# ecmwf/anemoi-models

Measured on AMD Instinct MI355X. Metric: mesh-node updates/sec (fwd step), higher is better.
Workload: dtype bf16

## Files before the change

### anemoi_models_amd/_lib.py

```python

from __future__ import annotations

import ctypes
import os
from ctypes import c_char_p
from ctypes import c_float
from ctypes import c_int
from ctypes import c_int64
from ctypes import c_uint32
from ctypes import c_void_p

import torch

_PKG_DIR = os.path.dirname(os.path.abspath(__file__))
LIB_PATH = os.path.join(_PKG_DIR, "lib", "libanemoi_amd.so")

ANEMOI_OK = 0
ANEMOI_ERR_INVALID = 1
ANEMOI_ERR_UNSUPPORTED = 2
ANEMOI_ERR_LAUNCH = 3

F32 = 0
BF16 = 1

ACT_NONE, ACT_GELU, ACT_SILU, ACT_RELU = 0, 1, 2, 3
ACT_CODES = {"Identity": ACT_NONE, "GELU": ACT_GELU, "SiLU": ACT_SILU, "ReLU": ACT_RELU}

ABI_VERSION = 41


class GtBlockArgs(ctypes.Structure):

    _fields_ = [
        ("struct_bytes", c_int64), ("n_dst", c_int64),
        ("dtype", ctypes.c_int32), ("C", ctypes.c_int32), ("H", ctypes.c_int32), ("up", ctypes.c_int32),
        ("hidden", ctypes.c_int32), ("act", ctypes.c_int32), ("k_proj", ctypes.c_int32), ("n_in", ctypes.c_int32),
        ("eps_mlp", c_float), ("eps_out", c_float),
        ("x", c_void_p), ("ldx", c_int64), ("x_stats", c_void_p),
        ("w_in", c_void_p), ("b_in", c_void_p), ("cs_in", c_void_p),
        ("sq", c_void_p), ("ld_sq", c_int64),
        ("q", c_void_p), ("k", c_void_p), ("v", c_void_p), ("x_r", c_void_p), ("u", c_void_p),
        ("ldq", c_int64), ("ldkv", c_int64), ("ldr", c_int64), ("ldu", c_int64),
        ("edge_attr", c_void_p), ("rowptr", c_void_p), ("col", c_void_p),
        ("att", c_void_p), ("ld_att", c_int64),
        ("w_proj", c_void_p), ("b_proj", c_void_p), ("res", c_void_p), ("ld_res", c_int64), ("y", c_void_p),
        ("y_stats", c_void_p),
        ("w_fc1", c_void_p), ("b_fc1", c_void_p), ("cs_fc1", c_void_p), ("h", c_void_p),
        ("w_fc2", c_void_p), ("b_fc2", c_void_p), ("out", c_void_p), ("out_stats", c_void_p),
        ("stats_ws", c_void_p), ("stats_ws_bytes", c_int64),
        ("run_ptr", c_void_p), ("run_perm", c_void_p), ("n_runs", c_int64),
        ("sched", c_void_p), ("sched_slots", ctypes.c_int32), ("sched_steps", ctypes.c_int32), ("n_src", c_int64),
        ("run_dst", c_void_p), ("n_edges", c_int64),
        ("tile_hdr", c_void_p), ("tile_dst", c_void_p), ("tile_src", c_void_p), ("tile_slot", c_void_p), ("tile_xcd", c_void_p),
        ("tile_max_per_xcd", ctypes.c_int32), ("tile_src_cap", ctypes.c_int32), ("tile_edge_cap", ctypes.c_int32),
        ("tile_pad", ctypes.c_int32),
    ]

class TfmBlockArgs(ctypes.Structure):

    _fields_ = [
        ("struct_bytes", c_int64), ("rows", c_int64),
        ("dtype", ctypes.c_int32), ("B", ctypes.c_int32), ("S", ctypes.c_int32), ("C", ctypes.c_int32), ("H", ctypes.c_int32),
        ("hidden", ctypes.c_int32), ("act", ctypes.c_int32), ("window", ctypes.c_int32),
        ("eps1", c_float), ("eps2", c_float),
        ("dropout_p", c_float), ("dropout_seed", c_uint32), ("dropout_seed_dev", c_void_p),
        ("dropout_h0", ctypes.c_int32), ("dropout_h_total", ctypes.c_int32),
        ("x", c_void_p), ("ldx", c_int64),
        ("ln1_w", c_void_p), ("ln1_b", c_void_p), ("ln2_w", c_void_p), ("ln2_b", c_void_p),
        ("w_qkv", c_void_p), ("b_qkv", c_void_p), ("w_proj", c_void_p), ("b_proj", c_void_p),
        ("w_fc1", c_void_p), ("b_fc1", c_void_p), ("w_fc2", c_void_p), ("b_fc2", c_void_p),
        ("h_ln", c_void_p), ("qkv", c_void_p), ("att", c_void_p), ("y", c_void_p), ("h", c_void_p),
        ("mhsa_ws", c_void_p), ("out", c_void_p),
    ]


SIGNATURES = {
    "anemoi_abi_version": (c_int, []),
    "anemoi_build_info": (ctypes.c_char_p, []),
    "anemoi_last_error": (c_char_p, []),
    "anemoi_layer_norm": (c_int, [c_int, c_void_p, c_int64, c_void_p, c_void_p, c_void_p, c_int64, c_int64, c_int,
                                  c_float, c_void_p]),
    "anemoi_layer_norm_residual": (c_int, [c_int, c_void_p, c_int64, c_void_p, c_void_p, c_void_p, c_int64, c_void_p, c_int64,
                                           c_int64, c_int, c_float, c_void_p]),
    "anemoi_layer_norm_stats": (c_int, [c_int, c_void_p, c_int64, c_void_p, c_void_p, c_void_p, c_int64, c_void_p, c_int64,
                                        c_int, c_float, c_void_p]),
    "anemoi_linear": (c_int, [c_int, c_int, c_void_p, c_int64, c_void_p, c_void_p, c_void_p, c_int64, c_void_p,
                              c_int64, c_int64, c_int, c_int, c_int, c_void_p]),
    "anemoi_linear_stats": (c_int, [c_int, c_void_p, c_int64, c_void_p, c_void_p, c_void_p, c_void_p, c_void_p, c_int64,
                                    c_void_p, c_int64, c_int64, c_int, c_int, c_void_p, c_int64, c_float, c_void_p,
                                    c_void_p]),
    "anemoi_row_stats": (c_int, [c_int, c_void_p, c_int64, c_void_p, c_int64, c_int, c_float, c_void_p]),
    "anemoi_linear_ln": (c_int, [c_int, c_int, c_void_p, c_int64, c_void_p, c_void_p, c_void_p, c_void_p, c_void_p,
                                 c_int64, c_void_p, c_int64, c_int64, c_int, c_int, c_int, c_void_p]),
    "anemoi_edge_attr_csr": (c_int, [c_void_p, c_int, c_void_p, c_int, c_int64, c_void_p, c_void_p, c_int, c_int,
                                     c_int64, c_void_p]),
    "anemoi_gt_edge_attention_folded": (c_int, [c_int, c_void_p, c_int64, c_void_p, c_void_p, c_int64, c_void_p,
                                                c_int64, c_void_p, c_int64, c_void_p, c_int, c_void_p, c_void_p,
                                                c_void_p, c_int64, c_void_p, c_int64, c_int, c_int, c_void_p]),
    "anemoi_gt_edge_attention_folded_runs": (c_int, [c_int, c_void_p, c_int64, c_void_p, c_void_p, c_int64, c_void_p,
                                                     c_int64, c_void_p, c_int64, c_void_p, c_int, c_void_p, c_void_p,
                                                     c_void_p, c_void_p, c_int64, c_void_p, c_int64, c_void_p, c_int64, c_int,
                                                     c_int, c_void_p]),
    "anemoi_gt_edge_attention_folded_groups": (c_int, [c_int, c_void_p, c_int64, c_void_p, c_void_p, c_int64, c_void_p,
                                                       c_int64, c_void_p, c_int64, c_void_p, c_int, c_void_p, c_void_p,
                                                       c_void_p, c_void_p, c_void_p, c_int64, c_int64, c_void_p, c_int64,
                                                       c_void_p, c_int64, c_int, c_int, c_void_p]),
    "anemoi_edge_schedule_shape": (c_int, [c_int, c_int64, c_int, c_void_p, c_void_p]),
    "anemoi_gt_edge_attention_folded_sched": (c_int, [c_int, c_void_p, c_int64, c_void_p, c_void_p, c_int64, c_void_p,
                                                      c_int64, c_void_p, c_int64, c_void_p, c_int, c_void_p, c_void_p,
                                                      c_void_p, c_int, c_int, c_int64, c_int64, c_void_p, c_int64, c_void_p,
                                                      c_int64, c_int, c_int, c_void_p]),
    "anemoi_gt_edge_attention_folded_tiles": (c_int, [c_int, c_void_p, c_int64, c_void_p, c_void_p, c_int64, c_void_p,
                                                      c_int64, c_void_p, c_int64, c_void_p, c_int, c_void_p, c_void_p,
                                                      c_void_p, c_void_p, c_void_p, c_void_p, c_void_p, c_int, c_int, c_int,
                                                      c_int64, c_int64, c_void_p, c_int64, c_void_p, c_int64, c_int, c_int,
                                                      c_void_p]),
    "anemoi_linear_dual": (c_int, [c_int, c_void_p, c_int64, c_void_p, c_void_p, c_void_p, c_int64, c_void_p, c_int64,
                                   c_int64, c_int, c_int, c_int, c_void_p]),
    "anemoi_linear_actgrad": (c_int, [c_int, c_void_p, c_int64, c_void_p, c_void_p, c_int64, c_void_p, c_int64, c_int64,
                                      c_int, c_int, c_int, c_void_p]),
    "anemoi_gt_conv": (c_int, [c_int, c_void_p, c_int64, c_void_p, c_void_p, c_int64, c_void_p, c_int64, c_void_p, c_int64,
                               c_void_p, c_void_p, c_void_p, c_int64, c_void_p, c_int64, c_int, c_int, c_float, c_uint32,
                               c_void_p, c_void_p]),
    "anemoi_gt_conv_backward_dst": (c_int, [c_int, c_void_p, c_int64, c_void_p, c_void_p, c_int64, c_void_p, c_int64,
                                            c_void_p, c_int64, c_void_p, c_void_p, c_void_p, c_void_p, c_void_p, c_void_p,
                                            c_void_p, c_int64, c_int64, c_int, c_int, c_float, c_uint32, c_void_p,
                                            c_void_p]),
    "anemoi_gt_conv_backward_src": (c_int, [c_int, c_void_p, c_int64, c_void_p, c_int64, c_void_p, c_void_p, c_void_p,
                                            c_void_p, c_void_p, c_void_p, c_void_p, c_void_p, c_int64, c_void_p, c_int64,
                                            c_int64, c_int, c_int, c_float, c_uint32, c_void_p, c_void_p]),
    "anemoi_gt_edge_attention": (c_int, [c_int, c_void_p, c_int64, c_void_p, c_void_p, c_int64, c_void_p, c_int64,
                                         c_void_p, c_int, c_int, c_void_p, c_void_p, c_void_p, c_void_p, c_void_p,
                                         c_int64, c_int64, c_int, c_int, c_void_p]),
    "anemoi_gather_add_act": (c_int, [c_int, c_void_p, c_int64, c_void_p, c_int64, c_void_p, c_int64, c_void_p, c_void_p,
                                      c_void_p, c_int64, c_int64, c_int, c_int, c_void_p]),
    "anemoi_segment_sum": (c_int, [c_int, c_void_p, c_int64, c_void_p, c_void_p, c_int64, c_int64, c_int, c_void_p]),
    "anemoi_segment_sum_cat": (c_int, [c_int, c_void_p, c_int64, c_void_p, c_void_p, c_int64, c_void_p, c_int64, c_int64,
                                       c_int, c_void_p]),
    "anemoi_mhsa_workspace_bytes": (c_int64, [c_int, c_int, c_int, c_int, c_int]),
    "anemoi_mhsa": (c_int, [c_int, c_void_p, c_int64, c_void_p, c_int64, c_void_p, c_void_p, c_int, c_int, c_int, c_int,
                            c_int, c_float, c_uint32, c_void_p, c_int, c_int, c_void_p]),
    "anemoi_mhsa_backward_workspace_bytes": (c_int64, [c_int, c_int, c_int, c_int, c_int]),
    "anemoi_mhsa_backward": (c_int, [c_int, c_void_p, c_int64, c_void_p, c_int64, c_void_p, c_int64, c_void_p, c_void_p,
                                     c_void_p, c_int64, c_void_p, c_int, c_int, c_int, c_int, c_int, c_float, c_uint32,
                                     c_void_p, c_int, c_int, c_void_p]),
    "anemoi_assemble_nodes": (c_int, [c_int, c_void_p, c_int, c_int, c_int, c_int64, c_int, c_void_p, c_int,
                                      c_void_p, c_int, c_void_p, c_int64, c_void_p, c_void_p, c_void_p]),
    "anemoi_finalize_output": (c_int, [c_void_p, c_int, c_void_p, c_int, c_int, c_int, c_int64, c_int, c_void_p,
                                       c_void_p, c_void_p, c_void_p, c_void_p, c_void_p]),
    "anemoi_assemble_node_rows": (c_int, [c_int, c_void_p, c_int, c_int64, c_int, c_void_p, c_int, c_void_p, c_int,
                                          c_void_p, c_int64, c_void_p, c_int64, c_void_p, c_void_p, c_void_p]),
    "anemoi_finalize_output_rows": (c_int, [c_void_p, c_int, c_void_p, c_int, c_int64, c_int, c_void_p, c_void_p, c_int64,
                                            c_void_p, c_void_p, c_void_p, c_void_p, c_void_p]),
    "anemoi_bound_output": (c_int, [c_void_p, c_int, c_int64, c_int, c_void_p, c_void_p, c_void_p, c_void_p, c_int,
                                    c_void_p, c_void_p, c_void_p, c_void_p]),
    "anemoi_prognostic_residual": (c_int, [c_void_p, c_int, c_void_p, c_int, c_int, c_int, c_int64, c_int, c_void_p,
                                           c_void_p, c_int, c_void_p]),
    "anemoi_advance_input": (c_int, [c_void_p, c_int, c_int, c_int, c_int64, c_int, c_void_p, c_int, c_void_p, c_int,
                                     c_void_p, c_void_p]),
    "anemoi_transpose": (c_int, [c_int, c_void_p, c_int64, c_void_p, c_int64, c_int64, c_int, c_void_p]),
    "anemoi_transpose_colsum_rows": (c_int64, [c_int64, c_int64]),
    "anemoi_transpose_chunked": (c_int, [c_int, c_void_p, c_int64, c_void_p, c_int64, c_int64, c_int, c_int64, c_void_p,
                                         c_void_p]),
    "anemoi_weight_grad_tn": (c_int, [c_void_p, c_int64, c_void_p, c_int64, c_void_p, c_int64, c_void_p, c_int64, c_int64,
                                      c_int, c_int, c_int, c_void_p]),
    "anemoi_linear_batched": (c_int, [c_int, c_int, c_void_p, c_int64, c_int64, c_void_p, c_int64, c_void_p, c_int64,
                                      c_int64, c_int, c_int64, c_int, c_int, c_void_p]),
    "anemoi_col_sum_workspace_floats": (c_int64, [c_int64, c_int]),
    "anemoi_col_sum": (c_int, [c_int, c_void_p, c_int64, c_int64, c_int, c_void_p, c_void_p, c_int64, c_void_p]),
    "anemoi_row_dot": (c_int, [c_int, c_void_p, c_int64, c_void_p, c_int64, c_void_p, c_void_p, c_int64, c_int, c_void_p]),
    "anemoi_row_scale": (c_int, [c_int, c_void_p, c_int64, c_void_p, c_float, c_void_p, c_int64, c_int64, c_int, c_void_p]),
    "anemoi_act_forward": (c_int, [c_int, c_int, c_void_p, c_int64, c_void_p, c_int64, c_void_p, c_int64, c_int64, c_int,
                                   c_void_p]),
    "anemoi_act_backward": (c_int, [c_int, c_int, c_void_p, c_int64, c_void_p, c_int64, c_void_p, c_int64, c_int64, c_int,
                                    c_void_p]),
    "anemoi_layer_norm_backward_workspace_floats": (c_int64, [c_int64, c_int]),
    "anemoi_layer_norm_backward": (c_int, [c_int, c_void_p, c_int64, c_void_p, c_void_p, c_void_p, c_int64, c_void_p,
                                           c_int64, c_void_p, c_int64, c_int64, c_int, c_void_p, c_void_p, c_void_p,
                                           c_int64, c_void_p]),
    "anemoi_gt_edge_attention_folded_backward_dst": (c_int, [c_int, c_void_p, c_int64, c_void_p, c_void_p, c_int64,
                                                             c_void_p, c_int64, c_void_p, c_int64, c_void_p, c_int64,
                                                             c_void_p, c_void_p, c_int, c_void_p, c_void_p, c_void_p,
                                                             c_void_p, c_void_p, c_void_p, c_int64, c_void_p, c_int64,
                                                             c_void_p, c_int64, c_int64, c_int, c_int, c_void_p]),
    "anemoi_gt_edge_attention_folded_backward_src": (c_int, [c_int, c_void_p, c_int64, c_void_p, c_int64, c_void_p,
                                                             c_void_p, c_void_p, c_void_p, c_void_p, c_void_p, c_void_p,
                                                             c_void_p, c_int64, c_int64, c_int, c_int, c_void_p]),
    "anemoi_gt_edge_attr_grad": (c_int, [c_int, c_void_p, c_void_p, c_void_p, c_void_p, c_int64, c_void_p, c_int64,
                                         c_void_p, c_void_p, c_int64, c_int, c_int, c_int, c_void_p]),
    "anemoi_convert_pad": (c_int, [c_int, c_void_p, c_int64, c_int, c_void_p, c_int64, c_int64, c_int, c_void_p]),
    "anemoi_add": (c_int, [c_int, c_void_p, c_int64, c_void_p, c_int64, c_void_p, c_int64, c_int64, c_int, c_void_p]),
    "anemoi_gt_block_tail": (c_int, [ctypes.POINTER(GtBlockArgs), c_void_p]),
    "anemoi_gt_processor_block_forward": (c_int, [ctypes.POINTER(GtBlockArgs), c_void_p]),
    "anemoi_transformer_block_forward": (c_int, [ctypes.POINTER(TfmBlockArgs), c_void_p]),
}

_lib = None


class KernelLibraryMissing(RuntimeError):
    pass


def load(build_if_missing: bool = False) -> ctypes.CDLL:
    global _lib
    if _lib is not None:
        return _lib
    if not os.path.exists(LIB_PATH):
        if build_if_missing:
            from ._build import build

            build()
        else:
            raise KernelLibraryMissing(
                f"{LIB_PATH} not found: the HIP kernel library has not been built "
                "(run `python -c 'import __graft_entry__ as g; g.build()'`). There is no CPU fallback."
            )
    lib = ctypes.CDLL(LIB_PATH)
    for name, (restype, argtypes) in SIGNATURES.items():
        fn = getattr(lib, name)
        fn.restype = restype
        fn.argtypes = argtypes
    got = lib.anemoi_abi_version()
    if got != ABI_VERSION:
        raise RuntimeError(f"libanemoi_amd.so ABI version {got} != expected {ABI_VERSION}; rebuild the library")
    _lib = lib
    return lib


def check(status: int, what: str) -> None:
    if status == ANEMOI_OK:
        return
    msg = load().anemoi_last_error()
    msg = msg.decode() if msg else what
    if status == ANEMOI_ERR_INVALID:
        raise ValueError(msg)
    if status == ANEMOI_ERR_UNSUPPORTED:
        raise NotImplementedError(msg)
    raise RuntimeError(msg)
```

### anemoi_models_amd/csrc/blocks.hip

```cpp
#include "common.hpp"

using namespace anemoi;

namespace {

int check_args(const anemoi_gt_block_args* a, const char* who, bool with_input) {
  ANEMOI_REQUIRE(a != nullptr, ANEMOI_ERR_INVALID, "%s: null argument block", who);
  ANEMOI_REQUIRE(a->struct_bytes == (int64_t)sizeof(anemoi_gt_block_args), ANEMOI_ERR_INVALID,
                 "%s: argument block of %lld bytes, this library expects %lld (header / binding out of sync)", who,
                 (long long)a->struct_bytes, (long long)sizeof(anemoi_gt_block_args));
  ANEMOI_REQUIRE(a->dtype == ANEMOI_BF16, ANEMOI_ERR_UNSUPPORTED,
                 "%s: the LayerNorm-folded block route is bf16 only (dtype %d)", who, a->dtype);
  ANEMOI_REQUIRE(a->n_dst >= 0 && a->C > 0 && a->H > 0 && a->C % a->H == 0 && a->up > 0 && a->hidden > 0,
                 ANEMOI_ERR_INVALID, "%s: bad shape (n_dst %lld, C %d, H %d, up %d, hidden %d)", who, (long long)a->n_dst,
                 a->C, a->H, a->up, a->hidden);
  ANEMOI_REQUIRE(a->k_proj >= a->C + a->H * a->up && a->ld_att >= a->k_proj, ANEMOI_ERR_INVALID,
                 "%s: projection K %d / ld_att %lld too small for C + H * up = %d", who, a->k_proj, (long long)a->ld_att,
                 a->C + a->H * a->up);
  ANEMOI_REQUIRE(a->edge_attr && a->rowptr && a->col && a->att && a->w_proj && a->y && a->y_stats && a->w_fc1 && a->cs_fc1 &&
                     a->h && a->w_fc2 && a->out && a->stats_ws,
                 ANEMOI_ERR_INVALID, "%s: null pointer", who);
  ANEMOI_REQUIRE(a->stats_ws_bytes >= a->n_dst * (int64_t)(a->C / 128 > 1 ? a->C / 128 : 1) * 8, ANEMOI_ERR_INVALID,
                 "%s: statistics workspace of %lld bytes too small", who, (long long)a->stats_ws_bytes);
  if (with_input) {
    ANEMOI_REQUIRE(a->x && a->x_stats && a->w_in && a->cs_in && a->sq, ANEMOI_ERR_INVALID, "%s: null pointer (input product)",
                   who);
    ANEMOI_REQUIRE(a->n_in >= 4 * a->C + a->H * a->up && a->ld_sq >= a->n_in && a->ldx >= a->C, ANEMOI_ERR_INVALID,
                   "%s: input product of %d columns (ld %lld) cannot hold x_r | q | k | v | u = %d", who, a->n_in,
                   (long long)a->ld_sq, 4 * a->C + a->H * a->up);
  } else {
    ANEMOI_REQUIRE(a->q && a->k && a->v && a->x_r && a->u && a->res, ANEMOI_ERR_INVALID,
                   "%s: null pointer (edge phase operands / residual)", who);
  }
  return ANEMOI_OK;
}

int run_tail(const anemoi_gt_block_args* a, anemoi_stream_t stream) {
  int st;
  if (a->tile_hdr != nullptr && a->run_ptr == nullptr)
    st = anemoi_gt_edge_attention_folded_tiles(a->dtype, a->q, a->ldq, a->k, a->v, a->ldkv, a->x_r, a->ldr, a->u, a->ldu,
                                               a->edge_attr, a->up, a->rowptr, a->col, a->tile_hdr, a->tile_dst, a->tile_src,
                                               a->tile_slot, a->tile_xcd, a->tile_max_per_xcd, a->tile_src_cap,
                                               a->tile_edge_cap, a->n_src, a->n_edges, a->att, a->ld_att, nullptr, a->n_dst,
                                               a->C, a->H, stream);
  else if (a->sched != nullptr && a->run_ptr == nullptr)
    st = anemoi_gt_edge_attention_folded_sched(a->dtype, a->q, a->ldq, a->k, a->v, a->ldkv, a->x_r, a->ldr, a->u, a->ldu,
                                               a->edge_attr, a->up, a->rowptr, a->col, a->sched, a->sched_slots, a->sched_steps,
                                               a->n_src, a->n_edges, a->att, a->ld_att, nullptr, a->n_dst, a->C, a->H, stream);
  else if (a->run_ptr != nullptr && a->run_dst != nullptr)
    st = anemoi_gt_edge_attention_folded_groups(a->dtype, a->q, a->ldq, a->k, a->v, a->ldkv, a->x_r, a->ldr, a->u, a->ldu,
                                                a->edge_attr, a->up, a->rowptr, a->col, a->run_ptr, a->run_dst, a->run_perm,
                                                a->n_runs, a->n_src, a->att, a->ld_att, nullptr, a->n_dst, a->C, a->H, stream);
  else
    st = anemoi_gt_edge_attention_folded_runs(a->dtype, a->q, a->ldq, a->k, a->v, a->ldkv, a->x_r, a->ldr, a->u, a->ldu,
                                              a->edge_attr, a->up, a->rowptr, a->col, a->run_ptr, a->run_perm, a->n_runs,
                                              a->att, a->ld_att, nullptr, a->n_dst, a->C, a->H, stream);
  if (st != ANEMOI_OK) return st;
  st = anemoi_linear_stats(a->dtype, a->att, a->ld_att, a->w_proj, a->b_proj, nullptr, nullptr, a->res, a->ld_res, a->y,
                           a->C, a->n_dst, a->C, a->k_proj, a->stats_ws, a->stats_ws_bytes, a->eps_mlp, a->y_stats, stream);
  if (st != ANEMOI_OK) return st;
  st = anemoi_linear_ln(a->dtype, a->dtype, a->y, a->C, a->w_fc1, a->b_fc1, a->cs_fc1, a->y_stats, nullptr, 0, a->h,
                        a->hidden, a->n_dst, a->hidden, a->C, a->act, stream);
  if (st != ANEMOI_OK) return st;
  if (a->out_stats != nullptr)
    return anemoi_linear_stats(a->dtype, a->h, a->hidden, a->w_fc2, a->b_fc2, nullptr, nullptr, a->y, a->C, a->out, a->C,
                               a->n_dst, a->C, a->hidden, a->stats_ws, a->stats_ws_bytes, a->eps_out, a->out_stats, stream);
  return anemoi_linear(a->dtype, a->dtype, a->h, a->hidden, a->w_fc2, a->b_fc2, a->y, a->C, a->out, a->C, a->n_dst, a->C,
                       a->hidden, ANEMOI_ACT_NONE, stream);
}

}

extern "C" int anemoi_gt_block_tail(const anemoi_gt_block_args* args, anemoi_stream_t stream) {
  const int st = check_args(args, "anemoi_gt_block_tail", false);
  if (st != ANEMOI_OK) return st;
  if (args->n_dst == 0) return ANEMOI_OK;
  return run_tail(args, stream);
}

extern "C" int anemoi_gt_processor_block_forward(const anemoi_gt_block_args* args, anemoi_stream_t stream) {
  int st = check_args(args, "anemoi_gt_processor_block_forward", true);
  if (st != ANEMOI_OK) return st;
  if (args->n_dst == 0) return ANEMOI_OK;
  st = anemoi_linear_ln(args->dtype, args->dtype, args->x, args->ldx, args->w_in, args->b_in, args->cs_in, args->x_stats,
                        nullptr, 0, args->sq, args->ld_sq, args->n_dst, args->n_in, args->C, ANEMOI_ACT_NONE, stream);
  if (st != ANEMOI_OK) return st;
  anemoi_gt_block_args a = *args;
  const char* sq = static_cast<const char*>(args->sq);
  const int64_t c2 = (int64_t)args->C * 2;
  a.x_r = sq;
  a.q = sq + c2;
  a.k = sq + 2 * c2;
  a.v = sq + 3 * c2;
  a.u = sq + 4 * c2;
  a.ldq = a.ldkv = a.ldr = a.ldu = args->ld_sq;
  a.res = args->x;
  a.ld_res = args->ldx;
  return run_tail(&a, stream);
}

extern "C" int anemoi_transformer_block_forward(const anemoi_tfm_block_args* a, anemoi_stream_t stream) {
  const char* who = "anemoi_transformer_block_forward";
  ANEMOI_REQUIRE(a != nullptr, ANEMOI_ERR_INVALID, "%s: null argument block", who);
  ANEMOI_REQUIRE(a->struct_bytes == (int64_t)sizeof(anemoi_tfm_block_args), ANEMOI_ERR_INVALID,
                 "%s: argument block of %lld bytes, this library expects %lld (header / binding out of sync)", who,
                 (long long)a->struct_bytes, (long long)sizeof(anemoi_tfm_block_args));
  ANEMOI_REQUIRE(a->dtype == ANEMOI_F32 || a->dtype == ANEMOI_BF16, ANEMOI_ERR_UNSUPPORTED, "%s: dtype %d", who, a->dtype);
  ANEMOI_REQUIRE(a->rows >= 0 && a->B > 0 && a->S >= 0 && a->rows == (int64_t)a->B * a->S && a->C > 0 && a->H > 0 &&
                     a->C % a->H == 0 && a->hidden > 0,
                 ANEMOI_ERR_INVALID, "%s: bad shape (rows %lld, B %d, S %d, C %d, H %d, hidden %d)", who, (long long)a->rows,
                 a->B, a->S, a->C, a->H, a->hidden);
  ANEMOI_REQUIRE(a->x && a->ln1_w && a->ln1_b && a->ln2_w && a->ln2_b && a->w_qkv && a->w_proj && a->w_fc1 && a->w_fc2 &&
                     a->h_ln && a->qkv && a->att && a->y && a->h && a->out,
                 ANEMOI_ERR_INVALID, "%s: null pointer", who);
  ANEMOI_REQUIRE(a->ldx >= a->C && a->out != a->x, ANEMOI_ERR_INVALID, "%s: ldx too small, or out aliases x", who);
  if (a->rows == 0) return ANEMOI_OK;
  const int C = a->C;
  int st = anemoi_layer_norm(a->dtype, a->x, a->ldx, a->ln1_w, a->ln1_b, a->h_ln, C, a->rows, C, a->eps1, stream);
  if (st != ANEMOI_OK) return st;
  st = anemoi_linear(a->dtype, a->dtype, a->h_ln, C, a->w_qkv, a->b_qkv, nullptr, 0, a->qkv, 3 * (int64_t)C, a->rows, 3 * C, C,
                     ANEMOI_ACT_NONE, stream);
  if (st != ANEMOI_OK) return st;
  st = anemoi_mhsa(a->dtype, a->qkv, 3 * (int64_t)C, a->att, C, a->mhsa_ws, nullptr, a->B, a->S, a->H, C / a->H, a->window,
                   a->dropout_p, a->dropout_seed, a->dropout_seed_dev, a->dropout_h0, a->dropout_h_total, stream);
  if (st != ANEMOI_OK) return st;
  st = anemoi_linear(a->dtype, a->dtype, a->att, C, a->w_proj, a->b_proj, a->x, a->ldx, a->y, C, a->rows, C, C, ANEMOI_ACT_NONE,
                     stream);
  if (st != ANEMOI_OK) return st;
  st = anemoi_layer_norm(a->dtype, a->y, C, a->ln2_w, a->ln2_b, a->h_ln, C, a->rows, C, a->eps2, stream);
  if (st != ANEMOI_OK) return st;
  st = anemoi_linear(a->dtype, a->dtype, a->h_ln, C, a->w_fc1, a->b_fc1, nullptr, 0, a->h, a->hidden, a->rows, a->hidden, C,
                     a->act, stream);
  if (st != ANEMOI_OK) return st;
  return anemoi_linear(a->dtype, a->dtype, a->h, a->hidden, a->w_fc2, a->b_fc2, a->y, C, a->out, C, a->rows, C, a->hidden,
                       ANEMOI_ACT_NONE, stream);
}
```

### anemoi_models_amd/csrc/elementwise.hip

```cpp
#include <cstdlib>

#include "common.hpp"

namespace anemoi {

template <typename T>
__device__ __forceinline__ float round_to(float v);
template <>
__device__ __forceinline__ float round_to<float>(float v) { return v; }
template <>
__device__ __forceinline__ float round_to<bf16_t>(float v) { return bf16_to_f32(f32_to_bf16(v)); }

template <typename T, int VEC, int ITEMS>
__global__ __launch_bounds__(256) void layer_norm_kernel(const T* __restrict__ x, int64_t ldx,
                                                         const float* __restrict__ gamma,
                                                         const float* __restrict__ beta, T* __restrict__ y,
                                                         int64_t ldy, int64_t rows, int C, float eps,
                                                         float2* __restrict__ stats, const T* __restrict__ res = nullptr,
                                                         int64_t ldr = 0) {
  const int lane = threadIdx.x & 63;
  const int64_t row = (int64_t)blockIdx.x * 4 + (threadIdx.x >> 6);
  if (row >= rows) return;
  const T* xr = x + row * ldx;
  float v[ITEMS][VEC];
// ... 497 lines not shown
      const int m = op_mul[i];
      if (m >= 0) v *= yr[m];
      yr[c] = v;
    }
    for (int j = 0; j < n_fin; ++j) {
      const int c = fin_col[j];
      yr[c] = (yr[c] - fin_add[j]) / fin_mul[j];
    }
  }
}

static bool force_idx64() {
  static const bool v = [] {
    const char* e = getenv("ANEMOI_AMD_IDX64");
    return e != nullptr && atoi(e) != 0;
  }();
  return v;
}

static inline unsigned flat_grid(int64_t total) {
  int64_t blocks = (total + 255) / 256;
  if (blocks > 256 * 16) blocks = 256 * 16;
  if (blocks < 1) blocks = 1;
  return (unsigned)blocks;
}

}

using namespace anemoi;

extern "C" {

int anemoi_layer_norm(int dtype, const void* x, int64_t ldx, const float* gamma, const float* beta, void* y,
                      int64_t ldy, int64_t rows, int C, float eps, anemoi_stream_t stream) {
  ANEMOI_REQUIRE(x && y && gamma && beta, ANEMOI_ERR_INVALID, "anemoi_layer_norm: null pointer");
  ANEMOI_REQUIRE(C > 0 && rows >= 0 && ldx >= C && ldy >= C, ANEMOI_ERR_INVALID,
                 "anemoi_layer_norm: bad shape rows=%lld C=%d ldx=%lld ldy=%lld", (long long)rows, C, (long long)ldx,
                 (long long)ldy);
  if (rows == 0) return ANEMOI_OK;
  if (dtype == ANEMOI_F32) return layer_norm_launch<float>(x, ldx, gamma, beta, y, ldy, rows, C, eps, as_stream(stream));
  if (dtype == ANEMOI_BF16) return layer_norm_launch<bf16_t>(x, ldx, gamma, beta, y, ldy, rows, C, eps, as_stream(stream));
  return fail(ANEMOI_ERR_UNSUPPORTED, "anemoi_layer_norm: dtype %d", dtype);
}

int anemoi_layer_norm_residual(int dtype, const void* x, int64_t ldx, const float* gamma, const float* beta,
                               const void* residual, int64_t ldr, void* y, int64_t ldy, int64_t rows, int C, float eps,
                               anemoi_stream_t stream) {
  ANEMOI_REQUIRE(x && y && gamma && beta && residual, ANEMOI_ERR_INVALID, "anemoi_layer_norm_residual: null pointer");
  ANEMOI_REQUIRE(C > 0 && rows >= 0 && ldx >= C && ldy >= C && ldr >= C, ANEMOI_ERR_INVALID,
                 "anemoi_layer_norm_residual: bad shape rows=%lld C=%d ldx=%lld ldr=%lld ldy=%lld", (long long)rows, C,
                 (long long)ldx, (long long)ldr, (long long)ldy);
  if (rows == 0) return ANEMOI_OK;
  if (dtype == ANEMOI_F32)
    return layer_norm_launch<float>(x, ldx, gamma, beta, y, ldy, rows, C, eps, as_stream(stream), nullptr, residual, ldr);
  if (dtype == ANEMOI_BF16)
    return layer_norm_launch<bf16_t>(x, ldx, gamma, beta, y, ldy, rows, C, eps, as_stream(stream), nullptr, residual, ldr);
  return fail(ANEMOI_ERR_UNSUPPORTED, "anemoi_layer_norm_residual: dtype %d", dtype);
}

int anemoi_layer_norm_stats(int dtype, const void* x, int64_t ldx, const float* gamma, const float* beta, void* y,
                            int64_t ldy, float* stats, int64_t rows, int C, float eps, anemoi_stream_t stream) {
  ANEMOI_REQUIRE(x && y && gamma && beta && stats, ANEMOI_ERR_INVALID, "anemoi_layer_norm_stats: null pointer");
  ANEMOI_REQUIRE(C > 0 && rows >= 0 && ldx >= C && ldy >= C && (uintptr_t)stats % 8 == 0, ANEMOI_ERR_INVALID,
                 "anemoi_layer_norm_stats: bad shape rows=%lld C=%d ldx=%lld ldy=%lld (stats 8-byte aligned)",
                 (long long)rows, C, (long long)ldx, (long long)ldy);
  if (rows == 0) return ANEMOI_OK;
  float2* sp = reinterpret_cast<float2*>(stats);
  if (dtype == ANEMOI_F32)
    return layer_norm_launch<float>(x, ldx, gamma, beta, y, ldy, rows, C, eps, as_stream(stream), sp);
  if (dtype == ANEMOI_BF16)
    return layer_norm_launch<bf16_t>(x, ldx, gamma, beta, y, ldy, rows, C, eps, as_stream(stream), sp);
  return fail(ANEMOI_ERR_UNSUPPORTED, "anemoi_layer_norm_stats: dtype %d", dtype);
}

int anemoi_row_stats(int dtype, const void* x, int64_t ldx, float* stats, int64_t rows, int C, float eps,
                     anemoi_stream_t stream) {
  ANEMOI_REQUIRE(x && stats, ANEMOI_ERR_INVALID, "anemoi_row_stats: null pointer");
  ANEMOI_REQUIRE(C > 0 && rows >= 0 && ldx >= C, ANEMOI_ERR_INVALID, "anemoi_row_stats: bad shape rows=%lld C=%d ldx=%lld",
                 (long long)rows, C, (long long)ldx);
  ANEMOI_REQUIRE((uintptr_t)stats % 8 == 0, ANEMOI_ERR_INVALID, "anemoi_row_stats: stats must be 8-byte aligned");
  if (rows == 0) return ANEMOI_OK;
  if (dtype == ANEMOI_F32) return row_stats_launch<float>(x, ldx, stats, rows, C, eps, as_stream(stream));
  if (dtype == ANEMOI_BF16) return row_stats_launch<bf16_t>(x, ldx, stats, rows, C, eps, as_stream(stream));
  return fail(ANEMOI_ERR_UNSUPPORTED, "anemoi_row_stats: dtype %d", dtype);
}

static int assemble_nodes_impl(int dtype, const float* x, int B, int T, int Ens, int64_t G, int V, const float* latlons,
                               int n_ll, const float* trainable, int n_tr, void* out, int64_t ldo, const float* in_mul,
                               const float* in_add, const int64_t* rows, int64_t n_rows, anemoi_stream_t stream) {
  ANEMOI_REQUIRE((in_mul == nullptr) == (in_add == nullptr), ANEMOI_ERR_INVALID,
                 "anemoi_assemble_nodes: in_mul and in_add come together");
  ANEMOI_REQUIRE(out && B > 0 && Ens > 0 && G >= 0 && T >= 0 && V >= 0 && n_ll >= 0 && n_tr >= 0, ANEMOI_ERR_INVALID,
                 "anemoi_assemble_nodes: bad argument");
  ANEMOI_REQUIRE((x != nullptr) || T * V == 0, ANEMOI_ERR_INVALID, "anemoi_assemble_nodes: x is null");
  ANEMOI_REQUIRE((latlons != nullptr) || n_ll == 0, ANEMOI_ERR_INVALID, "anemoi_assemble_nodes: latlons is null");
  ANEMOI_REQUIRE((trainable != nullptr) || n_tr == 0, ANEMOI_ERR_INVALID, "anemoi_assemble_nodes: trainable is null");
  ANEMOI_REQUIRE(ldo >= (int64_t)T * V + n_ll + n_tr, ANEMOI_ERR_INVALID, "anemoi_assemble_nodes: ldo too small");
  const int64_t total = (rows != nullptr ? n_rows : (int64_t)B * Ens * G) * ldo;
  if (total == 0) return ANEMOI_OK;
  hipStream_t st = as_stream(stream);
  if (ldo % 8 == 0 && ldo < ((int64_t)1 << 31) && (uintptr_t)out % 16 == 0 && (dtype == ANEMOI_F32 || dtype == ANEMOI_BF16)) {
    const int ldo8 = (int)(ldo / 8);
#define ANEMOI_ASM8(TT, I32)                                                                                          \
  hipLaunchKernelGGL((assemble_nodes8_kernel<TT, I32>), dim3(flat_grid(total / 8)), dim3(256), 0, st, x, B, T, Ens, G, V, \
                     latlons, n_ll, trainable, n_tr, static_cast<TT*>(out), ldo8, in_mul, in_add, rows, n_rows)
    const bool idx32 = !force_idx64() && total / 8 < ((int64_t)1 << 31) - ((int64_t)1 << 24);
    if (dtype == ANEMOI_F32) {
      if (idx32) ANEMOI_ASM8(float, true);
      else ANEMOI_ASM8(float, false);
    } else {
      if (idx32) ANEMOI_ASM8(bf16_t, true);
      else ANEMOI_ASM8(bf16_t, false);
    }
#undef ANEMOI_ASM8
    return check_launch("anemoi_assemble_nodes");
  }
  if (dtype == ANEMOI_F32)
    hipLaunchKernelGGL((assemble_nodes_kernel<float>), dim3(flat_grid(total)), dim3(256), 0, st, x, B, T, Ens, G, V,
                       latlons, n_ll, trainable, n_tr, static_cast<float*>(out), ldo, in_mul, in_add, rows, n_rows);
  else if (dtype == ANEMOI_BF16)
    hipLaunchKernelGGL((assemble_nodes_kernel<bf16_t>), dim3(flat_grid(total)), dim3(256), 0, st, x, B, T, Ens, G, V,
                       latlons, n_ll, trainable, n_tr, static_cast<bf16_t*>(out), ldo, in_mul, in_add, rows, n_rows);
  else
    return fail(ANEMOI_ERR_UNSUPPORTED, "anemoi_assemble_nodes: dtype %d", dtype);
  return check_launch("anemoi_assemble_nodes");
}

int anemoi_assemble_nodes(int dtype, const float* x, int B, int T, int Ens, int64_t G, int V, const float* latlons,
                          int n_ll, const float* trainable, int n_tr, void* out, int64_t ldo, const float* in_mul,
                          const float* in_add, anemoi_stream_t stream) {
  return assemble_nodes_impl(dtype, x, B, T, Ens, G, V, latlons, n_ll, trainable, n_tr, out, ldo, in_mul, in_add, nullptr, 0,
                             stream);
}

int anemoi_assemble_node_rows(int dtype, const float* x, int T, int64_t G, int V, const float* latlons, int n_ll,
                              const float* trainable, int n_tr, const int64_t* rows, int64_t n_rows, void* out,
                              int64_t ldo, const float* in_mul, const float* in_add, anemoi_stream_t stream) {
  ANEMOI_REQUIRE(n_rows >= 0 && (rows != nullptr || n_rows == 0), ANEMOI_ERR_INVALID,
                 "anemoi_assemble_node_rows: null row list");
  if (n_rows == 0) return ANEMOI_OK;
  return assemble_nodes_impl(dtype, x, 1, T, 1, G, V, latlons, n_ll, trainable, n_tr, out, ldo, in_mul, in_add, rows, n_rows,
                             stream);
}

int anemoi_edge_attr_csr(const float* a0, int d0, const float* a1, int d1, int64_t rows0, const int32_t* perm,
                         float* out, int ld_out, int one_col, int64_t n_edges, anemoi_stream_t stream) {
  ANEMOI_REQUIRE(a0 && perm && out && d0 > 0 && d1 >= 0 && rows0 > 0 && n_edges >= 0, ANEMOI_ERR_INVALID,
                 "anemoi_edge_attr_csr: bad argument");
  ANEMOI_REQUIRE((a1 != nullptr) || d1 == 0, ANEMOI_ERR_INVALID, "anemoi_edge_attr_csr: a1 is null but d1 > 0");
  ANEMOI_REQUIRE(ld_out >= d0 + d1, ANEMOI_ERR_INVALID, "anemoi_edge_attr_csr: ld_out %d < %d", ld_out, d0 + d1);
  ANEMOI_REQUIRE(one_col < ld_out && (one_col < 0 || one_col >= d0 + d1), ANEMOI_ERR_INVALID,
                 "anemoi_edge_attr_csr: one_col %d must be a padding column", one_col);
  if (n_edges == 0) return ANEMOI_OK;
  hipLaunchKernelGGL(edge_attr_csr_kernel, dim3(flat_grid(n_edges * ld_out)), dim3(256), 0, as_stream(stream), a0, d0,
                     a1, d1, rows0, perm, out, ld_out, one_col, n_edges);
  return check_launch("anemoi_edge_attr_csr");
}

int anemoi_convert_pad(int src_dtype, const void* src, int64_t ld_src, int dst_dtype, void* dst, int64_t ld_dst,
                       int64_t rows, int cols, anemoi_stream_t stream) {
  ANEMOI_REQUIRE(src && dst && rows >= 0 && cols >= 0 && ld_src >= cols && ld_dst >= cols, ANEMOI_ERR_INVALID,
                 "anemoi_convert_pad: bad argument");
  if (rows == 0 || ld_dst == 0) return ANEMOI_OK;
  hipStream_t st = as_stream(stream);
  dim3 grid(flat_grid(rows * ld_dst)), block(256);
#define CP(S, D)                                                                                           \
  hipLaunchKernelGGL((convert_pad_kernel<S, D>), grid, block, 0, st, static_cast<const S*>(src), ld_src, \
                     static_cast<D*>(dst), ld_dst, rows, cols)
  if (src_dtype == ANEMOI_F32 && dst_dtype == ANEMOI_F32) CP(float, float);
  else if (src_dtype == ANEMOI_F32 && dst_dtype == ANEMOI_BF16) CP(float, bf16_t);
  else if (src_dtype == ANEMOI_BF16 && dst_dtype == ANEMOI_F32) CP(bf16_t, float);
  else if (src_dtype == ANEMOI_BF16 && dst_dtype == ANEMOI_BF16) CP(bf16_t, bf16_t);
  else return fail(ANEMOI_ERR_UNSUPPORTED, "anemoi_convert_pad: dtypes %d -> %d", src_dtype, dst_dtype);
#undef CP
  return check_launch("anemoi_convert_pad");
}

int anemoi_row_scale(int dtype, const void* x, int64_t ldx, const float* s, float alpha, void* out, int64_t ldo,
                     int64_t rows, int cols, anemoi_stream_t stream) {
  ANEMOI_REQUIRE(x && s && out && rows >= 0 && cols >= 0 && ldx >= cols && ldo >= cols, ANEMOI_ERR_INVALID,
                 "anemoi_row_scale: bad argument");
  if (rows * cols == 0) return ANEMOI_OK;
  hipStream_t st = as_stream(stream);
  const int vec = dtype == ANEMOI_F32 ? 4 : 8;
  dim3 grid(flat_grid(rows * ((cols + vec - 1) / vec))), block(256);
  if (dtype == ANEMOI_F32)
    hipLaunchKernelGGL((row_scale_kernel<float>), grid, block, 0, st, static_cast<const float*>(x), ldx, s, alpha,
                       static_cast<float*>(out), ldo, rows, cols);
  else if (dtype == ANEMOI_BF16)
    hipLaunchKernelGGL((row_scale_kernel<bf16_t>), grid, block, 0, st, static_cast<const bf16_t*>(x), ldx, s, alpha,
                       static_cast<bf16_t*>(out), ldo, rows, cols);
  else
    return fail(ANEMOI_ERR_UNSUPPORTED, "anemoi_row_scale: dtype %d", dtype);
  return check_launch("anemoi_row_scale");
}

int anemoi_row_dot(int dtype, const void* a, int64_t lda, const void* b, int64_t ldb, const float* shift, float* out,
                   int64_t rows, int cols, anemoi_stream_t stream) {
  ANEMOI_REQUIRE(a && b && out && rows >= 0 && cols >= 0 && lda >= cols && ldb >= cols, ANEMOI_ERR_INVALID,
                 "anemoi_row_dot: bad argument");
  if (rows == 0) return ANEMOI_OK;
  hipStream_t st = as_stream(stream);
  dim3 grid((unsigned)((rows + 3) / 4)), block(256);
  ANEMOI_REQUIRE((rows + 3) / 4 < ((int64_t)1 << 31), ANEMOI_ERR_UNSUPPORTED, "anemoi_row_dot: grid too large");
  if (dtype == ANEMOI_F32)
    hipLaunchKernelGGL((row_dot_kernel<float>), grid, block, 0, st, static_cast<const float*>(a), lda,
                       static_cast<const float*>(b), ldb, shift, out, rows, cols);
  else if (dtype == ANEMOI_BF16)
    hipLaunchKernelGGL((row_dot_kernel<bf16_t>), grid, block, 0, st, static_cast<const bf16_t*>(a), lda,
                       static_cast<const bf16_t*>(b), ldb, shift, out, rows, cols);
  else
    return fail(ANEMOI_ERR_UNSUPPORTED, "anemoi_row_dot: dtype %d", dtype);
  return check_launch("anemoi_row_dot");
}

int anemoi_add(int dtype, const void* a, int64_t lda, const void* b, int64_t ldb, void* y, int64_t ldy, int64_t rows,
               int cols, anemoi_stream_t stream) {
  ANEMOI_REQUIRE(a && b && y && rows >= 0 && cols >= 0, ANEMOI_ERR_INVALID, "anemoi_add: bad argument");
  if (rows * cols == 0) return ANEMOI_OK;
  hipStream_t st = as_stream(stream);
  dim3 grid(flat_grid(rows * cols)), block(256);
  if (dtype == ANEMOI_F32)
    hipLaunchKernelGGL((add_kernel<float>), grid, block, 0, st, static_cast<const float*>(a), lda,
                       static_cast<const float*>(b), ldb, static_cast<float*>(y), ldy, rows, cols);
  else if (dtype == ANEMOI_BF16)
    hipLaunchKernelGGL((add_kernel<bf16_t>), grid, block, 0, st, static_cast<const bf16_t*>(a), lda,
                       static_cast<const bf16_t*>(b), ldb, static_cast<bf16_t*>(y), ldy, rows, cols);
  else
    return fail(ANEMOI_ERR_UNSUPPORTED, "anemoi_add: dtype %d", dtype);
  return check_launch("anemoi_add");
}

int anemoi_prognostic_residual(float* y, int V_out, const float* x, int B, int T, int Ens, int64_t G, int V_in,
                               const int32_t* out_idx, const int32_t* in_idx, int n_prog, anemoi_stream_t stream) {
  ANEMOI_REQUIRE(y && x && B > 0 && T > 0 && Ens > 0 && G >= 0 && n_prog >= 0, ANEMOI_ERR_INVALID,
                 "anemoi_prognostic_residual: bad argument");
  ANEMOI_REQUIRE(n_prog == 0 || (out_idx && in_idx), ANEMOI_ERR_INVALID, "anemoi_prognostic_residual: null index");
  const int64_t total = (int64_t)B * Ens * G * n_prog;
  if (total == 0) return ANEMOI_OK;
  hipLaunchKernelGGL(prognostic_residual_kernel, dim3(flat_grid(total)), dim3(256), 0, as_stream(stream), y, V_out, x,
                     B, T, Ens, G, V_in, out_idx, in_idx, n_prog);
  return check_launch("anemoi_prognostic_residual");
}

int anemoi_advance_input(float* x, int B, int T, int Ens, int64_t G, int V_in, const float* y, int V_out,
                         const float* forcing, int F, const int32_t* colmap, anemoi_stream_t stream) {
  ANEMOI_REQUIRE(x && y && colmap && B > 0 && T > 0 && Ens > 0 && G >= 0 && V_in > 0 && V_out > 0 && F >= 0,
                 ANEMOI_ERR_INVALID, "anemoi_advance_input: bad argument");
  const int64_t total = (int64_t)B * Ens * G * V_in;
  if (total == 0) return ANEMOI_OK;
  hipLaunchKernelGGL(advance_input_kernel, dim3(flat_grid(total)), dim3(256), 0, as_stream(stream), x, B, T, Ens, G,
                     V_in, y, V_out, forcing, F, colmap);
  return check_launch("anemoi_advance_input");
}

static int finalize_output_impl(float* y, int V_out, const float* x, int B, int T, int Ens, int64_t G, int V_in,
                                const int32_t* src, const float* in_mul, const float* in_add, const float* out_mul,
                                const float* out_add, const int64_t* rows, int64_t n_rows, anemoi_stream_t stream) {
  ANEMOI_REQUIRE(y && x && src && B > 0 && T > 0 && Ens > 0 && G >= 0 && V_in > 0 && V_out > 0, ANEMOI_ERR_INVALID,
                 "anemoi_finalize_output: bad argument");
  ANEMOI_REQUIRE((in_mul == nullptr) == (in_add == nullptr) && (out_mul == nullptr) == (out_add == nullptr),
                 ANEMOI_ERR_INVALID, "anemoi_finalize_output: mul and add come together");
  const int64_t total = (rows != nullptr ? n_rows : (int64_t)B * Ens * G) * V_out;
  if (total == 0) return ANEMOI_OK;
  if (!force_idx64() && total < ((int64_t)1 << 31) - ((int64_t)1 << 24))
    hipLaunchKernelGGL(finalize_output_kernel<true>, dim3(flat_grid(total)), dim3(256), 0, as_stream(stream), y, V_out, x, B,
                       T, Ens, G, V_in, src, in_mul, in_add, out_mul, out_add, rows, n_rows);
  else
    hipLaunchKernelGGL(finalize_output_kernel<false>, dim3(flat_grid(total)), dim3(256), 0, as_stream(stream), y, V_out, x, B,
                       T, Ens, G, V_in, src, in_mul, in_add, out_mul, out_add, rows, n_rows);
  return check_launch("anemoi_finalize_output");
}

int anemoi_finalize_output(float* y, int V_out, const float* x, int B, int T, int Ens, int64_t G, int V_in,
                           const int32_t* src, const float* in_mul, const float* in_add, const float* out_mul,
                           const float* out_add, anemoi_stream_t stream) {
  return finalize_output_impl(y, V_out, x, B, T, Ens, G, V_in, src, in_mul, in_add, out_mul, out_add, nullptr, 0, stream);
}

int anemoi_finalize_output_rows(float* y, int V_out, const float* x, int T, int64_t G, int V_in, const int32_t* src,
                                const int64_t* rows, int64_t n_rows, const float* in_mul, const float* in_add,
                                const float* out_mul, const float* out_add, anemoi_stream_t stream) {
  ANEMOI_REQUIRE(n_rows >= 0 && (rows != nullptr || n_rows == 0), ANEMOI_ERR_INVALID,
                 "anemoi_finalize_output_rows: null row list");
  if (n_rows == 0) return ANEMOI_OK;
  return finalize_output_impl(y, V_out, x, 1, T, 1, G, V_in, src, in_mul, in_add, out_mul, out_add, rows, n_rows, stream);
}

int anemoi_bound_output(float* y, int V_out, int64_t rows, int n_ops, const int32_t* op_col, const float* op_lo,
                        const float* op_hi, const int32_t* op_mul, int n_fin, const int32_t* fin_col,
                        const float* fin_mul, const float* fin_add, anemoi_stream_t stream) {
  ANEMOI_REQUIRE(y && V_out > 0 && rows >= 0 && n_ops >= 0 && n_fin >= 0, ANEMOI_ERR_INVALID,
                 "anemoi_bound_output: bad argument");
  ANEMOI_REQUIRE(n_ops == 0 || (op_col && op_lo && op_hi && op_mul), ANEMOI_ERR_INVALID,
                 "anemoi_bound_output: null op list");
  ANEMOI_REQUIRE(n_fin == 0 || (fin_col && fin_mul && fin_add), ANEMOI_ERR_INVALID,
                 "anemoi_bound_output: null de-normalisation list");
  if (rows == 0 || (n_ops == 0 && n_fin == 0)) return ANEMOI_OK;
  hipLaunchKernelGGL(bound_output_kernel, dim3(flat_grid(rows)), dim3(256), 0, as_stream(stream), y, V_out, rows, n_ops,
                     op_col, op_lo, op_hi, op_mul, n_fin, fin_col, fin_mul, fin_add);
  return check_launch("anemoi_bound_output");
}

int anemoi_abi_version(void) { return 41; }

#ifndef ANEMOI_HIPCC_VERSION
#define ANEMOI_HIPCC_VERSION "unknown (built without anemoi_models_amd/_build.py)"
#endif
const char* anemoi_build_info(void) { return "gfx950; " ANEMOI_HIPCC_VERSION; }

const char* anemoi_last_error(void) { return err_buf(); }

}
```

### anemoi_models_amd/layers/block.py

```python

from __future__ import annotations

import os
from abc import ABC
from abc import abstractmethod
from typing import Optional

import torch
from torch import Tensor
from torch import nn

from .. import ops
from .. import runtime
from .. import training
from ..runtime import EdgePlan
from .conv import GraphConv
from .conv import GraphTransformerConv
from .mlp import MLP
from .mlp import NativeSequential
from .mlp import activation_class
from .mlp import linear_native


def inference_num_chunks() -> int:
    return int(os.environ.get("ANEMOI_INFERENCE_NUM_CHUNKS", "1"))


def _group_size(group) -> int:
    return 1 if group is None else group.size()


def _as_compute(x: Tensor, dtype: torch.dtype) -> Tensor:
    x = x if x.dtype == dtype else x.to(dtype)
    return x if (x.dim() == 2 and x.stride(1) == 1) else x.contiguous()



def folded_edge_phase(q: Tensor, k: Tensor, v: Tensor, x_r: Optional[Tensor], u: Tensor, edge_attr_csr: Tensor, plan,
                      num_heads: int, up: int, ld_out: Optional[int] = None) -> Tensor:
    runs = edge_runs(plan, q.dtype)
    tiles = None if runs is not None else edge_tiles(plan, q, num_heads, up)
    return ops.gt_edge_attention_folded(q, k, v, x_r, u, edge_attr_csr, plan.rowptr, plan.col, num_heads, up,
                                        ld_out=ld_out, runs=runs, tiles=tiles,
                                        sched=None if runs is not None or tiles is not None else edge_schedule(plan, q))


TILES_DEFAULT = "0"


def edge_tiles(plan, q: Tensor, num_heads: int, up: int):
    if (q.dtype != torch.bfloat16 or not hasattr(plan, "tiles")
            or os.environ.get("ANEMOI_AMD_EDGE_TILES", TILES_DEFAULT) == "0"):
        return None
    return plan.tiles(q.dtype, q.shape[-1], num_heads, up)


def edge_schedule(plan, q: Tensor):
    if q.dtype != torch.bfloat16 or not hasattr(plan, "schedule") or os.environ.get("ANEMOI_AMD_EDGE_SCHED", "1") == "0":
        return None
    return plan.schedule(q.dtype, q.shape[-1])


def set_tile_args(a, tiles, n_src: int, n_edges: int) -> None:
    a.tile_hdr, a.tile_dst, a.tile_src = tiles.hdr.data_ptr(), tiles.dst.data_ptr(), tiles.src.data_ptr()
    a.tile_slot, a.tile_xcd = tiles.slot.data_ptr(), tiles.xcd.data_ptr()
    a.tile_max_per_xcd, a.tile_src_cap, a.tile_edge_cap = tiles.max_tiles_per_xcd, tiles.src_cap, tiles.edge_cap
    a.n_src, a.n_edges = n_src, n_edges


def edge_runs(plan, dtype):
    if dtype != torch.bfloat16 or not hasattr(plan, "runs3") or os.environ.get("ANEMOI_AMD_EDGE_RUNS", "1") == "0":
        return None
    return plan.runs3()


class EmbeddedRows:

    def __init__(self, x_aug: Tensor, one_col: int, emb: nn.Linear, h: Optional[Tensor], packed, tag: str) -> None:
        self.x_aug, self.one_col, self.emb, self.h, self._packed, self._tag = x_aug, one_col, emb, h, packed, tag

    @property
    def dtype(self) -> torch.dtype:
        return self.x_aug.dtype

    @property
    def device(self) -> torch.device:
        return self.x_aug.device

    @property
    def shape(self):
        return (self.x_aug.shape[0], self.emb.out_features)

    def stats(self, eps: float) -> Tensor:
        if self.h is not None:
            return ops.row_stats(self.h, eps)
        kp = self.x_aug.shape[1]
        t = self._packed.get((self._tag, "embstats", self.dtype, kp, self.one_col), [self.emb.weight, self.emb.bias],
                             lambda: runtime.embedding_stats_operator(self.emb.weight, self.emb.bias, kp, self.one_col,
                                                                      self.dtype))
        return ops.row_stats(ops.linear(self.x_aug, t, None, stats_eps=eps), eps)


class BaseBlock(nn.Module, ABC):

    @abstractmethod
    def forward(self, x, edge_attr, edge_index, shapes, batch_size, size=None, model_comm_group=None): ...


class GraphTransformerBaseBlock(BaseBlock, ABC):

    def __init__(
        self,
        in_channels: int,
        hidden_dim: int,
        out_channels: int,
        edge_dim: int,
        num_heads: int = 16,
        bias: bool = True,
        activation: str = "GELU",
        num_chunks: int = 1,
        update_src_nodes: bool = False,
        **kwargs,
    ) -> None:
        super().__init__(**kwargs)
        self.update_src_nodes = update_src_nodes
        self.out_channels_conv = out_channels // num_heads
        self.num_heads = num_heads
        self.num_chunks = num_chunks
        self.activation = activation
        self.edge_dim = edge_dim
        width = num_heads * self.out_channels_conv

        self.lin_key = nn.Linear(in_channels, width)
        self.lin_query = nn.Linear(in_channels, width)
        self.lin_value = nn.Linear(in_channels, width)
        self.lin_self = nn.Linear(in_channels, width, bias=bias)
        self.lin_edge = nn.Linear(edge_dim, width)
        self.conv = GraphTransformerConv(out_channels=self.out_channels_conv)
        self.projection = nn.Linear(out_channels, out_channels)

        act = activation_class(activation)
        self.node_dst_mlp = nn.Sequential(
            nn.LayerNorm(out_channels), nn.Linear(out_channels, hidden_dim), act(), nn.Linear(hidden_dim, out_channels)
        )
        self.layer_norm1 = nn.LayerNorm(in_channels)
        if self.update_src_nodes:
            self.node_src_mlp = nn.Sequential(
                nn.LayerNorm(out_channels), nn.Linear(out_channels, hidden_dim), act(),
                nn.Linear(hidden_dim, out_channels),
            )
        self._packed = runtime.PackedWeights()
        self._plans = runtime.PlanCache()
        self._dst_mlp: Optional[NativeSequential] = None
        self._src_mlp: Optional[NativeSequential] = None

    def shard_qkve_heads(self, query: Tensor, key: Tensor, value: Tensor, edges: Tensor, shapes: tuple, batch_size: int,
                         model_comm_group=None):
        h, d = self.num_heads, self.out_channels_conv
        if _group_size(model_comm_group) <= 1:
            return tuple(t.reshape(t.shape[0], h, d) for t in (query, key, value, edges))
        from ..distributed.transformer import shard_heads

        assert batch_size == 1, "Only batch size of 1 is supported when model is sharded across GPUs"
        shapes_src, shapes_dst, shapes_edges = shapes
        out = []
        for t, shp in ((query, shapes_dst), (key, shapes_src), (value, shapes_src), (edges, shapes_edges)):
            t = t.reshape(1, t.shape[0], h, d).permute(0, 2, 1, 3)
            t = shard_heads(t, shapes=shp, mgroup=model_comm_group)
            out.append(t[0].permute(1, 0, 2).contiguous())
        return tuple(out)

    def shard_output_seq(self, out: Tensor, shapes: tuple, batch_size: int, model_comm_group=None) -> Tensor:
        if _group_size(model_comm_group) <= 1:
            return out.reshape(out.shape[0], -1)
        from ..distributed.transformer import shard_sequence

        t = out.permute(1, 0, 2).unsqueeze(0)
        t = shard_sequence(t, shapes=shapes[1], mgroup=model_comm_group)
        return t[0].permute(1, 0, 2).reshape(t.shape[2], -1).contiguous()

    def _cat_linear(self, tag: str, layers, dtype):
        w = self._packed.get((tag, "w", dtype), [l.weight for l in layers],
                             lambda: runtime.pack_weight([l.weight for l in layers], dtype))
        b = self._packed.get((tag, "b"), [l.bias for l in layers],
                             lambda: runtime.pack_bias([l.bias for l in layers], [l.out_features for l in layers],
                                                       layers[0].weight.device))
        return w, b

    @staticmethod
    def _ln_begin(ln: nn.LayerNorm, x: Tensor):
        if isinstance(x, EmbeddedRows):
            return x, x.stats(ln.eps), ln
        if runtime.ln_fold_enabled(x.dtype):
            return x, ops.row_stats(x, ln.eps), ln
        return ops.layer_norm(x, runtime.f32c(ln.weight), runtime.f32c(ln.bias), ln.eps), None, None

    def _ln_linear(self, handle, tag: str, plain, rows, params, **kw) -> Tensor:
        xin, stats, ln = handle
        if isinstance(xin, EmbeddedRows):
            xa = xin.x_aug
            wf, bf, zero = self._packed.get(
                (tag, "embfold", xa.dtype, xa.shape[1], xin.one_col, xin._tag),
                list(params) + [ln.weight, ln.bias, xin.emb.weight, xin.emb.bias],
                lambda: runtime.fold_embedded_layer_norm(*rows(), ln.weight, ln.bias, xin.emb.weight, xin.emb.bias,
                                                         xa.shape[1], xin.one_col, xa.dtype))
            return ops.linear(xa, wf, bf, ln=(stats, zero), **kw)
        if stats is None:
            w, b = plain()
            return ops.linear(xin, w, b, **kw)
        wf, bf, cs = self._packed.get(
            (tag, "lnfold", xin.dtype), list(params) + [ln.weight, ln.bias],
            lambda: runtime.fold_layer_norm(*rows(), ln.weight, ln.bias, xin.dtype))
        return ops.linear(xin, wf, bf, ln=(stats, cs), **kw)

    def _cat_rows(self, layers):
        w = torch.cat([l.weight.detach().float() for l in layers], dim=0)
        b = runtime.pack_bias([l.bias for l in layers], [l.out_features for l in layers], w.device)
        return w, b

    def _folded_rows(self, lead_layers, up: int):
        w, b = self._cat_rows(lead_layers)
        wu, bu = self._query_fold(up)
        return torch.cat([w, wu], dim=0), torch.cat([b, bu], dim=0)

    def _edge_params(self):
        return runtime.f32c(self.lin_edge.weight), runtime.f32c(self.lin_edge.bias)

    def fold_width(self, dtype) -> Optional[int]:
        if os.environ.get("ANEMOI_AMD_EDGE_FOLD", "1") == "0":
            return None
        vec = 16 // torch.empty((), dtype=dtype).element_size()
        d, h = self.out_channels_conv, self.num_heads
        if d % vec != 0 or (d // vec) not in (1, 2, 4, 8, 16):
            return None
        up = ops.round_up(self.edge_dim + 1, 4)
        if up > 16 or (h * up) % vec != 0 or self.lin_self.in_features % vec != 0:
            return None
        return up

    def edge_layout(self, dtype):
        up = self.fold_width(dtype)
        return (ops.round_up(self.edge_dim, 4), -1) if up is None else (up, self.edge_dim)

    def _edge_fold(self, up: int) -> Tensor:
        h, d = self.num_heads, self.out_channels_conv
        we = torch.zeros((h * d, up), dtype=torch.float32, device=self.lin_edge.weight.device)
        we[:, : self.edge_dim] = self.lin_edge.weight.detach().float()
        we[:, self.edge_dim] = self.lin_edge.bias.detach().float()
        return we.view(h, d, up)

    def _query_fold(self, up: int):
        h, d = self.num_heads, self.out_channels_conv
        weh = self._edge_fold(up)
        wq = self.lin_query.weight.detach().float().view(h, d, -1)
        wu = torch.einsum("hda,hdc->hac", weh, wq).reshape(h * up, -1)
        bu = torch.einsum("hda,hd->ha", weh, self.lin_query.bias.detach().float().view(h, d)).reshape(h * up)
        return wu, bu

    def _projection_fold(self, up: int) -> Tensor:
        h, d = self.num_heads, self.out_channels_conv
        wp = self.projection.weight.detach().float()
        return torch.einsum("ohd,hda->oha", wp.view(wp.shape[0], h, d), self._edge_fold(up)).reshape(wp.shape[0],
                                                                                                       h * up)

    def _folded_in(self, tag: str, lead_layers, dtype, up: int):
        edge_q = [self.lin_edge.weight, self.lin_edge.bias, self.lin_query.weight, self.lin_query.bias]
        w_in = self._packed.get((tag, "w", dtype, up), [l.weight for l in lead_layers] + edge_q,
                                lambda: runtime.pack_weight([l.weight for l in lead_layers] + [self._query_fold(up)[0]],
                                                            dtype))
        b_in = self._packed.get((tag, "b", up), [l.bias for l in lead_layers] + edge_q,
                                lambda: torch.cat([runtime.pack_bias([l.bias for l in lead_layers],
                                                                     [l.out_features for l in lead_layers],
                                                                     self.lin_edge.weight.device),
                                                   self._query_fold(up)[1]]).contiguous())
        return w_in, b_in

    def _folded_out(self, dtype, up: int):
        edge_p = [self.lin_edge.weight, self.lin_edge.bias, self.projection.weight]
        w_out = self._packed.get(("projf", "w", dtype, up), edge_p,
                                 lambda: runtime.pack_weight_cols([self.projection.weight.detach().float(),
                                                                   self._projection_fold(up)], dtype))
        return w_out, runtime.f32c(self.projection.bias)

    def _fold_params(self, lead_layers):
        return ([l.weight for l in lead_layers] + [l.bias for l in lead_layers]
                + [self.lin_edge.weight, self.lin_edge.bias, self.lin_query.weight, self.lin_query.bias])

    def _mlp_ln_eps(self, which: str, dtype) -> Optional[float]:
        mlp = self.node_dst_mlp if which == "dst" else self.node_src_mlp
        first = mlp[0] if isinstance(mlp, nn.Sequential) else None
        return first.eps if isinstance(first, nn.LayerNorm) and runtime.ln_fold_enabled(dtype) else None

    def _next_ln_eps(self, dtype) -> Optional[float]:
        ln1 = getattr(self, "layer_norm1", None)
        return ln1.eps if isinstance(ln1, nn.LayerNorm) and runtime.ln_fold_enabled(dtype) else None

    def block_abi_operands(self, dtype: torch.dtype, lead_layers, tag: str):
        up = self.fold_width(dtype)
        if up is None or not runtime.ln_fold_enabled(dtype):
            return None
        if self._dst_mlp is None:
            self._dst_mlp = NativeSequential(self.node_dst_mlp)
        mlp = self._dst_mlp.folded_pair(dtype)
        if mlp is None:
            return None
        ln = self.layer_norm1
        w_in, b_in, cs_in = self._packed.get(
            (tag, "lnfold", dtype), list(self._fold_params(lead_layers)) + [ln.weight, ln.bias],
            lambda: runtime.fold_layer_norm(*self._folded_rows(lead_layers, up), ln.weight, ln.bias, dtype))
        w_proj, b_proj = self._folded_out(dtype, up)
        eps_mlp, act, w1, b1, cs1, w2, b2 = mlp
        return dict(up=up, w_in=w_in, b_in=b_in, cs_in=cs_in, w_proj=w_proj, b_proj=b_proj, eps_mlp=eps_mlp, act=act, w_fc1=w1,
                    b_fc1=b1, cs_fc1=cs1, w_fc2=w2, b_fc2=b2, eps_ln1=ln.eps)

    def _block_tail(self, q: Tensor, k: Tensor, v: Tensor, x_r: Tensor, u: Tensor, edge_attr_csr: Tensor, plan, res: Tensor,
                    up: int, out_stats_eps: Optional[float]) -> Optional[Tensor]:
        import ctypes

        from .. import _lib

        dtype = q.dtype
        if (ops.PROFILE is not None or dtype != torch.bfloat16 or not q.is_cuda or plan.num_edges == 0 or q.shape[0] == 0
                or not self.block_abi or self._mlp_ln_eps("dst", dtype) is None):
            return None
        if self._dst_mlp is None:
            self._dst_mlp = NativeSequential(self.node_dst_mlp)
        mlp = self._dst_mlp.folded_pair(dtype)
        if mlp is None or not (res.dim() == 2 and res.stride(1) == 1):
            return None
        eps_mlp, act, w1, b1, cs1, w2, b2 = mlp
        wp, bp = self._folded_out(dtype, up)
        n, c, h = q.shape[0], q.shape[1], self.num_heads
        dev = q.device
        att = torch.empty((n, wp.shape[1]), dtype=dtype, device=dev)
        if wp.shape[1] > c + h * up:
            att[:, c + h * up:].zero_()
        y, hid, out = (torch.empty((n, w), dtype=dtype, device=dev) for w in (c, w1.shape[0], c))
        stats = torch.empty((2 if out_stats_eps is not None else 1, n, 2), dtype=torch.float32, device=dev)
        ws = torch.empty((n * max(c // 128, 1), 2), dtype=torch.float32, device=dev)
        a = _lib.GtBlockArgs()
        a.struct_bytes, a.n_dst, a.dtype = ctypes.sizeof(_lib.GtBlockArgs), n, ops.dtype_code(dtype)
        a.C, a.H, a.up, a.hidden, a.act, a.k_proj = c, h, up, w1.shape[0], _lib.ACT_CODES[act], wp.shape[1]
        a.eps_mlp, a.eps_out = eps_mlp, (out_stats_eps if out_stats_eps is not None else 0.0)
        a.q, a.k, a.v, a.x_r, a.u = q.data_ptr(), k.data_ptr(), v.data_ptr(), x_r.data_ptr(), u.data_ptr()
        a.ldq, a.ldkv, a.ldr, a.ldu = ops._ld(q), ops._ld(k), ops._ld(x_r), ops._ld(u)
        a.edge_attr, a.rowptr, a.col = edge_attr_csr.data_ptr(), plan.rowptr.data_ptr(), plan.col.data_ptr()
        runs = edge_runs(plan, dtype)
        if runs is not None:
            a.run_ptr, a.run_perm, a.n_runs = runs[0].data_ptr(), runs[1].data_ptr(), runs[0].shape[0] - 1
            if len(runs) == 3:
                a.run_dst, a.n_src = runs[2].data_ptr(), k.shape[0]
        else:
            tiles = edge_tiles(plan, q, h, up)
            if tiles is not None:
                set_tile_args(a, tiles, k.shape[0], edge_attr_csr.shape[0])
            sched = None if tiles is not None else edge_schedule(plan, q)
            if sched is not None:
                a.sched, a.sched_slots, a.sched_steps, a.n_src = sched.data_ptr(), sched.shape[1], sched.shape[2], k.shape[0]
                a.n_edges = edge_attr_csr.shape[0]
        a.att, a.ld_att = att.data_ptr(), wp.shape[1]
        a.w_proj, a.b_proj = wp.data_ptr(), ops._ptr(bp)
        a.res, a.ld_res, a.y, a.y_stats = res.data_ptr(), ops._ld(res), y.data_ptr(), stats[0].data_ptr()
        a.w_fc1, a.b_fc1, a.cs_fc1, a.h = w1.data_ptr(), ops._ptr(b1), cs1.data_ptr(), hid.data_ptr()
        a.w_fc2, a.b_fc2, a.out = w2.data_ptr(), ops._ptr(b2), out.data_ptr()
        a.out_stats = stats[1].data_ptr() if out_stats_eps is not None else None
        a.stats_ws, a.stats_ws_bytes = ws.data_ptr(), ws.numel() * 4
        _lib.check(_lib.load().anemoi_gt_block_tail(ctypes.byref(a), ops._stream()), "anemoi_gt_block_tail")
        if out_stats_eps is not None:
            ops._carry_stats(out, out_stats_eps, stats[1])
        return out

    block_abi = True

    def _node_mlp(self, y: Tensor, which: str, num_chunks: int, out_stats_eps: Optional[float] = None) -> Tensor:
        if which == "dst":
            if self._dst_mlp is None:
                self._dst_mlp = NativeSequential(self.node_dst_mlp)
            run = self._dst_mlp
        else:
            if self._src_mlp is None:
                self._src_mlp = NativeSequential(self.node_src_mlp)
            run = self._src_mlp
        if num_chunks <= 1:
            return run(y, residual=y, out_stats_eps=out_stats_eps)
        return torch.cat([run(c, residual=c) for c in y.tensor_split(num_chunks, dim=0) if c.shape[0] > 0], dim=0)

    def _check_channels(self, dtype) -> None:
        mult = ops.k_multiple(dtype)
        width = self.num_heads * self.out_channels_conv
        if width % mult != 0:
            raise NotImplementedError(
                f"hidden width {width} must be a multiple of {mult} for {dtype} on the MI355X path"
            )

    def _edge_inputs(self, edge_attr: Tensor, edge_index: Tensor, n_src: int, n_dst: int, dtype):
        if edge_attr.shape[1] != self.edge_dim:
            raise ValueError(f"edge_attr has {edge_attr.shape[1]} features, lin_edge expects {self.edge_dim}")
        if edge_attr.shape[0] != edge_index.shape[1]:
            raise ValueError(f"edge_attr has {edge_attr.shape[0]} rows for {edge_index.shape[1]} edges")
        plan = self._plans.get(edge_index, n_src, n_dst)
        return plan, ops.edge_attr_csr(edge_attr, None, plan.perm, *self.edge_layout(dtype))

    @abstractmethod
    def forward(self, x, edge_attr, edge_index, shapes, batch_size, model_comm_group=None, size=None): ...


class GraphTransformerProcessorBlock(GraphTransformerBaseBlock):

    def native(self, x: Tensor, edge_attr_csr: Tensor, plan: EdgePlan, halo=None) -> Tensor:
        dtype = x.dtype
        self._check_channels(dtype)
        c = self.num_heads * self.out_channels_conv
        xh = self._ln_begin(self.layer_norm1, x)
        up = self.fold_width(dtype)
        if halo is not None:
            if up is None:
                raise NotImplementedError("node-partitioned blocks need the folded edge kernel")
            n_own = x.shape[0]
            kv_layers, sq_layers = [self.lin_key, self.lin_value], [self.lin_self, self.lin_query]
            kv = torch.empty((n_own + halo.n_recv, 2 * c), dtype=dtype, device=x.device)
            self._ln_linear(xh, "kv", lambda: self._cat_linear("kv", kv_layers, dtype),
                            lambda: self._cat_rows(kv_layers), [l.weight for l in kv_layers] + [l.bias for l in kv_layers],
                            out=kv[:n_own])
            pending = halo.start(kv, n_own)
            wpf, bp = self._folded_out(dtype, up)
            sq = self._ln_linear(xh, "squ", lambda: self._folded_in("squ", sq_layers, dtype, up),
                                 lambda: self._folded_rows(sq_layers, up),
                                 self._fold_params(sq_layers))
            halo.finish(pending)
            done = self._block_tail(sq[:, c:2 * c], kv[:, :c], kv[:, c:], sq[:, :c], sq[:, 2 * c:], edge_attr_csr, plan, x, up,
                                    self._next_ln_eps(dtype))
            if done is not None:
                return done
            att = folded_edge_phase(sq[:, c:2 * c], kv[:, :c], kv[:, c:], sq[:, :c], sq[:, 2 * c:], edge_attr_csr, plan,
                                    self.num_heads, up, ld_out=wpf.shape[1])
            y = ops.linear(att, wpf, bp, residual=x, stats_eps=self._mlp_ln_eps("dst", dtype))
            return self._node_mlp(y, "dst", 1, out_stats_eps=self._next_ln_eps(dtype))
        all4 = [self.lin_self, self.lin_query, self.lin_key, self.lin_value]
        if up is not None:
            wpf, bp = self._folded_out(dtype, up)
            sq = self._ln_linear(xh, "sqkvu", lambda: self._folded_in("sqkvu", all4, dtype, up),
                                 lambda: self._folded_rows(all4, up),
                                 self._fold_params(all4))
            done = self._block_tail(sq[:, c:2 * c], sq[:, 2 * c:3 * c], sq[:, 3 * c:4 * c], sq[:, :c], sq[:, 4 * c:],
                                    edge_attr_csr, plan, x, up, self._next_ln_eps(dtype))
            if done is not None:
                return done
            att = folded_edge_phase(sq[:, c:2 * c], sq[:, 2 * c:3 * c], sq[:, 3 * c:4 * c], sq[:, :c], sq[:, 4 * c:],
                                    edge_attr_csr, plan, self.num_heads, up, ld_out=wpf.shape[1])
            y = ops.linear(att, wpf, bp, residual=x, stats_eps=self._mlp_ln_eps("dst", dtype))
            return self._node_mlp(y, "dst", 1, out_stats_eps=self._next_ln_eps(dtype))
        wp, bp = self._cat_linear("proj", [self.projection], dtype)
        we, be = self._edge_params()
        sqkv = self._ln_linear(xh, "sqkv", lambda: self._cat_linear("sqkv", all4, dtype), lambda: self._cat_rows(all4),
                               [l.weight for l in all4] + [l.bias for l in all4])
        att = self.conv.fused(sqkv[:, c:2 * c], sqkv[:, 2 * c:3 * c], sqkv[:, 3 * c:], sqkv[:, :c], edge_attr_csr,
                              self.edge_dim, we, be, plan, self.num_heads)
        y = ops.linear(att, wp, bp, residual=x, stats_eps=self._mlp_ln_eps("dst", dtype))
        return self._node_mlp(y, "dst", 1, out_stats_eps=self._next_ln_eps(dtype))

    def _sharded(self, x: Tensor, edge_attr: Tensor, edge_index: Tensor, shapes: tuple, batch_size: int, model_comm_group,
                 size=None) -> Tensor:
        from .. import autograd

        dtype = runtime.compute_dtype(x)
        x = _as_compute(x, dtype)
        ln = self.layer_norm1
        h = autograd.layer_norm(x, ln.weight, ln.bias, ln.eps)
        x_r, q, k, v = (autograd.linear(h, lin.weight, lin.bias) for lin in (self.lin_self, self.lin_query, self.lin_key,
                                                                              self.lin_value))
        e = autograd.linear(_as_compute(edge_attr, dtype), self.lin_edge.weight, self.lin_edge.bias)
        q, k, v, e = self.shard_qkve_heads(q, k, v, e, shapes, batch_size, model_comm_group)
        out = self.conv(q, k, v, e, edge_index, size=size)
        out = self.shard_output_seq(out, shapes, batch_size, model_comm_group)
        out = autograd.linear(out + x_r, self.projection.weight, self.projection.bias, "Identity", x)
        return training.sequential(self.node_dst_mlp, out, residual=out)

    def forward(
        self,
        x: Tensor,
        edge_attr: Tensor,
        edge_index: Tensor,
        shapes: tuple,
        batch_size: int,
        model_comm_group=None,
        size=None,
    ):
        if _group_size(model_comm_group) > 1:
            assert batch_size == 1, "Only batch size of 1 is supported when model is sharded across GPUs"
            return self._sharded(x, edge_attr, edge_index, shapes, batch_size, model_comm_group, size), edge_attr
        if training.wants_grad(self, x, edge_attr):
            return training.gt_processor_block(self, x, edge_attr, edge_index, size)
        dtype = runtime.compute_dtype(x)
        n = x.shape[0]
        if size is not None and tuple(size) != (n, n):
            raise ValueError(f"Encountered tensor with size {n} in dimension 0, but expected size {tuple(size)}")
        plan, ea = self._edge_inputs(edge_attr, edge_index, n, n, dtype)
        return self.native(_as_compute(x, dtype), ea, plan), edge_attr


class GraphTransformerMapperBlock(GraphTransformerBaseBlock):

    def __init__(
        self,
        in_channels: int,
        hidden_dim: int,
        out_channels: int,
        edge_dim: int,
        num_heads: int = 16,
        bias: bool = True,
        activation: str = "GELU",
        num_chunks: int = 1,
        update_src_nodes: bool = False,
        **kwargs,
    ) -> None:
        super().__init__(
            in_channels=in_channels, hidden_dim=hidden_dim, out_channels=out_channels, edge_dim=edge_dim,
            num_heads=num_heads, bias=bias, activation=activation, num_chunks=num_chunks,
            update_src_nodes=update_src_nodes, **kwargs,
        )
        self.layer_norm2 = nn.LayerNorm(in_channels)

    def native(self, x_src: Tensor, x_dst: Tensor, edge_attr_csr: Tensor, plan: EdgePlan, num_chunks: int = 1,
               halo=None, out_stats_eps: Optional[float] = None):
        dtype = x_dst.dtype
        self._check_channels(dtype)
        c = self.num_heads * self.out_channels_conv
        h_dst = x_dst.h if isinstance(x_dst, EmbeddedRows) else x_dst
        if isinstance(x_src, EmbeddedRows) and x_src.h is None and self.update_src_nodes:
            raise ValueError("update_src_nodes needs the embedded source rows")
        kv_layers, sq_layers = [self.lin_key, self.lin_value], [self.lin_self, self.lin_query]
        kv_args = ("kv", lambda: self._cat_linear("kv", kv_layers, dtype), lambda: self._cat_rows(kv_layers),
                   [l.weight for l in kv_layers] + [l.bias for l in kv_layers])
        xs = self._ln_begin(self.layer_norm1, x_src)
        if halo is None:
            kv = self._ln_linear(xs, *kv_args)
        else:
            n_own = x_src.shape[0]
            kv = torch.empty((n_own + halo.n_recv, 2 * c), dtype=dtype, device=x_src.device)
            self._ln_linear(xs, *kv_args, out=kv[:n_own])
            pending = halo.start(kv, n_own)
        del xs
        xd = self._ln_begin(self.layer_norm2, x_dst)
        up = self.fold_width(dtype)
        if up is not None:
            wp, bp = self._folded_out(dtype, up)
            sq = self._ln_linear(xd, "squ", lambda: self._folded_in("squ", sq_layers, dtype, up),
                                 lambda: self._folded_rows(sq_layers, up),
                                 self._fold_params(sq_layers))
            del xd
            if halo is not None:
                halo.finish(pending)
            if num_chunks <= 1 and not self.update_src_nodes:
                done = self._block_tail(sq[:, c:2 * c], kv[:, :c], kv[:, c:], sq[:, :c], sq[:, 2 * c:], edge_attr_csr, plan,
                                        h_dst, up, out_stats_eps)
                if done is not None:
                    return (x_src.h if isinstance(x_src, EmbeddedRows) else x_src), done
            att = folded_edge_phase(sq[:, c:2 * c], kv[:, :c], kv[:, c:], sq[:, :c], sq[:, 2 * c:], edge_attr_csr, plan,
                                    self.num_heads, up, ld_out=wp.shape[1])
        else:
            if halo is not None:
                raise NotImplementedError("node-partitioned blocks need the folded edge kernel")
            wp, bp = self._cat_linear("proj", [self.projection], dtype)
            we, be = self._edge_params()
            sq = self._ln_linear(xd, "sq", lambda: self._cat_linear("sq", sq_layers, dtype),
                                 lambda: self._cat_rows(sq_layers),
                                 [l.weight for l in sq_layers] + [l.bias for l in sq_layers])
            del xd
            att = self.conv.fused(sq[:, c:], kv[:, :c], kv[:, c:], sq[:, :c], edge_attr_csr, self.edge_dim, we, be,
                                  plan, self.num_heads)
        del sq, kv
        y = ops.linear(att, wp, bp, residual=h_dst,
                       stats_eps=self._mlp_ln_eps("dst", dtype) if num_chunks <= 1 else None)
        del att
        new_dst = self._node_mlp(y, "dst", num_chunks, out_stats_eps=out_stats_eps)
        if isinstance(x_src, EmbeddedRows):
            x_src = x_src.h
        new_src = self._node_mlp(x_src, "src", num_chunks) if self.update_src_nodes else x_src
        return new_src, new_dst

    def _sharded(self, x, edge_attr: Tensor, edge_index: Tensor, shapes: tuple, batch_size: int, model_comm_group, size=None):
        from .. import autograd

        x_src, x_dst = x
        dtype = runtime.compute_dtype(x_dst)
        x_src, x_dst = _as_compute(x_src, dtype), _as_compute(x_dst, dtype)
        ln1, ln2 = self.layer_norm1, self.layer_norm2
        hs = autograd.layer_norm(x_src, ln1.weight, ln1.bias, ln1.eps)
        hd = autograd.layer_norm(x_dst, ln2.weight, ln2.bias, ln2.eps)
        x_r = autograd.linear(hd, self.lin_self.weight, self.lin_self.bias)
        q = autograd.linear(hd, self.lin_query.weight, self.lin_query.bias)
        k = autograd.linear(hs, self.lin_key.weight, self.lin_key.bias)
        v = autograd.linear(hs, self.lin_value.weight, self.lin_value.bias)
        e = autograd.linear(_as_compute(edge_attr, dtype), self.lin_edge.weight, self.lin_edge.bias)
        q, k, v, e = self.shard_qkve_heads(q, k, v, e, shapes, batch_size, model_comm_group)
        out = self.conv(q, k, v, e, edge_index, size=size)
        out = self.shard_output_seq(out, shapes, batch_size, model_comm_group)
        out = autograd.linear(out + x_r, self.projection.weight, self.projection.bias, "Identity", x_dst)
        new_src = training.sequential(self.node_src_mlp, x_src, residual=x_src) if self.update_src_nodes else x_src
        return new_src, training.sequential(self.node_dst_mlp, out, residual=out)

    def forward(
        self,
        x,
        edge_attr: Tensor,
        edge_index: Tensor,
        shapes: tuple,
        batch_size: int,
        model_comm_group=None,
        size=None,
    ):
        if _group_size(model_comm_group) > 1:
            assert batch_size == 1, "Only batch size of 1 is supported when model is sharded across GPUs"
            return self._sharded(x, edge_attr, edge_index, shapes, batch_size, model_comm_group, size), edge_attr
        if training.wants_grad(self, x[0], x[1], edge_attr):
            return training.gt_mapper_block(self, x, edge_attr, edge_index, size)
        x_src, x_dst = x
        dtype = runtime.compute_dtype(x_dst)
        n_src, n_dst = x_src.shape[0], x_dst.shape[0]
        if size is not None and tuple(size) != (n_src, n_dst):
            raise ValueError(f"Encountered tensors with sizes {(n_src, n_dst)}, but expected size {tuple(size)}")
        plan, ea = self._edge_inputs(edge_attr, edge_index, n_src, n_dst, dtype)
        num_chunks = self.num_chunks if self.training else inference_num_chunks()
        new_src, new_dst = self.native(_as_compute(x_src, dtype), _as_compute(x_dst, dtype), ea, plan, num_chunks)
        return (new_src if self.update_src_nodes else x[0], new_dst), edge_attr


class GraphConvBaseBlock(BaseBlock, ABC):
    def __init__(
        self,
        in_channels: int,
        out_channels: int,
        mlp_extra_layers: int = 0,
        activation: str = "SiLU",
        update_src_nodes: bool = True,
        num_chunks: int = 1,
        **kwargs,
    ) -> None:
        super().__init__(**kwargs)
        self.update_src_nodes = update_src_nodes
        self.num_chunks = num_chunks
        self.node_mlp = MLP(2 * in_channels, out_channels, out_channels, n_extra_layers=mlp_extra_layers,
                            activation=activation)
        self.conv = GraphConv(in_channels=in_channels, out_channels=out_channels, mlp_extra_layers=mlp_extra_layers,
                              activation=activation)
        self._packed = runtime.PackedWeights()
        self._plans = runtime.PlanCache()

    @abstractmethod
    def forward(self, x, edge_attr: Tensor, edge_index: Tensor, shapes: tuple, model_comm_group=None, size=None):
        """``(new nodes, new edge state)`` -- reference layers/block.py:157-167."""

    @staticmethod
    def _check_width(width: int, dtype) -> None:
        mult = ops.k_multiple(dtype)
        if width % mult != 0:
            raise NotImplementedError(f"hidden width {width} must be a multiple of {mult} for {dtype} on the MI355X path")


class GraphConvProcessorBlock(GraphConvBaseBlock):

    def native(self, x: Tensor, e_csr: Tensor, plan: EdgePlan, halo=None):
        dtype = x.dtype
        c = x.shape[1]
        self._check_width(c, dtype)
        edge_mlp, node_mlp = self.conv.edge_mlp.native(), self.node_mlp.native()
        lin1 = edge_mlp.steps[0][1]
        act1 = edge_mlp.steps[0][2]
        if lin1.in_features != 3 * c or e_csr.shape[1] != c:
            raise ValueError(f"GNN block expects node / edge width {lin1.in_features // 3}, got {c} / {e_csr.shape[1]}")
        if e_csr.shape[0] == 0 and halo is None:
            xcat = torch.zeros((x.shape[0], 2 * c), dtype=dtype, device=x.device)
            xcat[:, :c].copy_(x)
            return node_mlp(xcat, residual=x), e_csr
        w_nodes = self._packed.get(("w1_nodes", dtype), [lin1.weight],
                                   lambda: runtime.pack_weight([lin1.weight[:, :c], lin1.weight[:, c:2 * c]], dtype))
        w_edges = self._packed.get(("w1_edges", dtype), [lin1.weight],
                                   lambda: runtime.pack_weight([lin1.weight[:, 2 * c:]], dtype))
        b1 = None if lin1.bias is None else runtime.f32c(lin1.bias)
        if halo is None:
            p = ops.linear(x, w_nodes, None)
            p_dst, p_src = p[:, :c], p[:, c:]
            t = ops.linear(e_csr, w_edges, b1)
        else:
            n_own = x.shape[0]
            p_src = torch.empty((n_own + halo.n_recv, c), dtype=dtype, device=x.device)
            ops.linear(x, w_nodes[c:], None, out=p_src[:n_own])
            pending = halo.start(p_src, n_own)
            p_dst = ops.linear(x, w_nodes[:c], None)
            t = ops.linear(e_csr, w_edges, b1)
            halo.finish(pending)
            p = None
        h = ops.gather_add_act(t, p_dst, p_src, plan.dst, plan.col, act=act1, out=t)
        e_new = edge_mlp(h, residual=e_csr, start=1)
        del h, t, p, p_dst, p_src
        xcat = ops.segment_sum(e_new, plan.rowptr, cat_with=x)
        return node_mlp(xcat, residual=x), e_new

    def _sharded(self, x, edge_attr, edge_index, shapes, model_comm_group, size=None):
        from ..distributed.graph import shard_tensor, sync_tensor

        dtype = runtime.compute_dtype(x)
        x = _as_compute(x, dtype)
        x_in = sync_tensor(x, 0, shapes[1], model_comm_group)
        out, edges_new = self.conv(x_in, _as_compute(edge_attr, dtype), edge_index, size=size)
        out = shard_tensor(out, 0, shapes[1], model_comm_group, gather_in_backward=False)
        return training.mlp(self.node_mlp, torch.cat([x, out], dim=1), residual=x), edges_new

    def forward(self, x, edge_attr, edge_index, shapes, model_comm_group=None, size=None):
        if _group_size(model_comm_group) > 1:
            return self._sharded(x, edge_attr, edge_index, shapes, model_comm_group, size)
        if training.wants_grad(self, x, edge_attr):
            return training.gnn_processor_block(self, x, edge_attr, edge_index, size)
        dtype = runtime.compute_dtype(x)
        n = x.shape[0]
        plan = self._plans.get(edge_index, n, n)
        perm = plan.perm.long()
        e_csr = _as_compute(edge_attr, dtype).index_select(0, perm)
        x_new, e_new = self.native(_as_compute(x, dtype), e_csr, plan)
        edges_new = torch.empty_like(e_new)
        edges_new[perm] = e_new
        return x_new, edges_new


class GraphConvMapperBlock(GraphConvBaseBlock):

    def native(self, x_src: Tensor, x_dst: Tensor, e_csr: Tensor, plan: EdgePlan, halo=None):
        dtype = x_dst.dtype
        c = x_dst.shape[1]
        self._check_width(c, dtype)
        edge_mlp, node_mlp = self.conv.edge_mlp.native(), self.node_mlp.native()
        lin1, act1 = edge_mlp.steps[0][1], edge_mlp.steps[0][2]
        if e_csr.shape[0] == 0 and halo is None:
            def lone(x, second):
                xcat = torch.zeros((x.shape[0], 2 * c), dtype=dtype, device=x.device)
                xcat[:, :c].copy_(x)
                if second is not None:
                    xcat[:, c:].copy_(second)
                return node_mlp(xcat, residual=x)

            return (lone(x_src, x_src) if self.update_src_nodes else x_src, lone(x_dst, None)), e_csr
        w_dst = self._packed.get(("w1_dst", dtype), [lin1.weight], lambda: runtime.pack_weight([lin1.weight[:, :c]], dtype))
        w_src = self._packed.get(("w1_src", dtype), [lin1.weight],
                                 lambda: runtime.pack_weight([lin1.weight[:, c:2 * c]], dtype))
        w_edges = self._packed.get(("w1_edges", dtype), [lin1.weight],
                                   lambda: runtime.pack_weight([lin1.weight[:, 2 * c:]], dtype))
        if halo is None:
            p_src = ops.linear(x_src, w_src, None)
            pending = None
        else:
            n_own = x_src.shape[0]
            p_src = torch.empty((n_own + halo.n_recv, c), dtype=dtype, device=x_dst.device)
            ops.linear(x_src, w_src, None, out=p_src[:n_own])
            pending = halo.start(p_src, n_own)
        p_dst = ops.linear(x_dst, w_dst, None)
        t = ops.linear(e_csr, w_edges, None if lin1.bias is None else runtime.f32c(lin1.bias))
        if pending is not None:
            halo.finish(pending)
        h = ops.gather_add_act(t, p_dst, p_src, plan.dst, plan.col, act=act1, out=t)
        e_new = edge_mlp(h, residual=e_csr, start=1)
        del h, t, p_dst, p_src

        def update(x, agg):
            if agg is not None:
                return node_mlp(ops.segment_sum(agg, plan.rowptr, cat_with=x), residual=x)
            xcat = torch.empty((x.shape[0], 2 * c), dtype=dtype, device=x.device)
            xcat[:, :c].copy_(x)
            xcat[:, c:].copy_(x)
            return node_mlp(xcat, residual=x)

        new_dst = update(x_dst, e_new)
        new_src = update(x_src, None) if self.update_src_nodes else x_src
        return (new_src, new_dst), e_new

    def _sharded(self, x, edge_attr, edge_index, shapes, model_comm_group, size=None):
        from ..distributed.graph import shard_tensor, sync_tensor

        dtype = runtime.compute_dtype(x[1])
        x_src, x_dst = _as_compute(x[0], dtype), _as_compute(x[1], dtype)
        x_in = (sync_tensor(x_src, 0, shapes[0], model_comm_group), sync_tensor(x_dst, 0, shapes[1], model_comm_group))
        out, edges_new = self.conv(x_in, _as_compute(edge_attr, dtype), edge_index, size=size)
        out = shard_tensor(out, 0, shapes[1], model_comm_group, gather_in_backward=False)
        new_dst = training.mlp(self.node_mlp, torch.cat([x_dst, out], dim=1), residual=x_dst)
        new_src = x_src if not self.update_src_nodes else training.mlp(self.node_mlp, torch.cat([x_src, x_src], dim=1),
                                                                      residual=x_src)
        return (new_src, new_dst), edges_new

    def forward(self, x, edge_attr, edge_index, shapes, model_comm_group=None, size=None):
        if _group_size(model_comm_group) > 1:
            return self._sharded(x, edge_attr, edge_index, shapes, model_comm_group, size)
        if training.wants_grad(self, x[0], x[1], edge_attr):
            return training.gnn_mapper_block(self, x, edge_attr, edge_index, size)
        x_src, x_dst = x
        dtype = runtime.compute_dtype(x_dst)
        n_src, n_dst = x_src.shape[0], x_dst.shape[0]
        if size is not None and tuple(size) != (n_src, n_dst):
            raise ValueError(f"Encountered tensors with sizes {(n_src, n_dst)}, but expected size {tuple(size)}")
        plan = self._plans.get(edge_index, n_src, n_dst)
        perm = plan.perm.long()
        e_csr = _as_compute(edge_attr, dtype).index_select(0, perm)
        nodes, e_new = self.native(_as_compute(x_src, dtype), _as_compute(x_dst, dtype), e_csr, plan)
        edges_new = torch.empty_like(e_new)
        edges_new[perm] = e_new
        return nodes, edges_new


class TransformerProcessorBlock(BaseBlock):
    def __init__(self, num_channels: int, hidden_dim: int, num_heads: int, activation: str, window_size: int,
                 dropout_p: float = 0.0):
        super().__init__()
        from .attention import MultiHeadSelfAttention

        act = activation_class(activation)
        self.layer_norm1 = nn.LayerNorm(num_channels)
        self.attention = MultiHeadSelfAttention(num_heads=num_heads, embed_dim=num_channels, window_size=window_size,
                                                bias=False, is_causal=False, dropout_p=dropout_p)
        self.mlp = nn.Sequential(nn.Linear(num_channels, hidden_dim), act(), nn.Linear(hidden_dim, num_channels))
        self.layer_norm2 = nn.LayerNorm(num_channels)

        self._mlp: Optional[NativeSequential] = None

    def native(self, x: Tensor, batch_size: int, head_exchange=None) -> Tensor:
        ln1, ln2 = self.layer_norm1, self.layer_norm2
        att = self.attention
        if head_exchange is None:
            done = self._block_abi(x, batch_size)
            if done is not None:
                return done
        h = ops.layer_norm(x, runtime.f32c(ln1.weight), runtime.f32c(ln1.bias), ln1.eps)
        qkv = linear_native(att._packed, "lin_qkv", att.lin_qkv, h)
        drop_p, drop_seed, drop_dev = att.dropout(None if head_exchange is None else head_exchange.group)
        if head_exchange is not None:
            window = att.attention_window()
            qkv_heads = head_exchange.rows_to_heads(qkv, att.num_heads)
            if window >= 0:
                qkv_heads = qkv_heads.index_select(0, head_exchange.to_external)
            a_heads = ops.mhsa(qkv_heads, batch_size, head_exchange.local_heads(att.num_heads), window, dropout_p=drop_p,
                               dropout_seed=drop_seed, head_offset=head_exchange._head_bounds(att.num_heads)[head_exchange.rank],
                               heads_total=att.num_heads, seed_dev=drop_dev)
            if window >= 0:
                a_heads = a_heads.index_select(0, head_exchange.to_internal)
            a = head_exchange.heads_to_rows(a_heads, att.num_heads)
        else:
            a = ops.mhsa(qkv, batch_size, att.num_heads, att.attention_window(), dropout_p=drop_p, dropout_seed=drop_seed,
                         seed_dev=drop_dev)
        x = linear_native(att._packed, "projection", att.projection, a, residual=x)
        if self._mlp is None:
            self._mlp = NativeSequential(self.mlp)
        h = ops.layer_norm(x, runtime.f32c(ln2.weight), runtime.f32c(ln2.bias), ln2.eps)
        return self._mlp(h, residual=x)

    block_abi = True

    def _block_abi(self, x: Tensor, batch_size: int) -> Optional[Tensor]:
        import ctypes

        from .. import _lib

        dtype, att = x.dtype, self.attention
        c, rows = x.shape[1], x.shape[0]
        mult = ops.k_multiple(dtype)
        if (not self.block_abi or ops.PROFILE is not None or not x.is_cuda or rows == 0 or x.stride(1) != 1
                or c != att.embed_dim or c % mult != 0 or rows % batch_size != 0):
            return None
        if self._mlp is None:
            self._mlp = NativeSequential(self.mlp)
        steps = self._mlp.steps
        if [k for k, _, _ in steps] != ["linear", "linear"] or steps[0][2] not in _lib.ACT_CODES or steps[1][2] != "Identity":
            return None
        fc1, fc2 = steps[0][1], steps[1][1]
        hidden = fc1.out_features
        if hidden % mult != 0 or fc1.in_features != c or fc2.out_features != c:
            return None

        def packed(cache, tag, lin):
            w = cache.get((tag, "w", dtype), [lin.weight], lambda: runtime.pack_weight([lin.weight], dtype))
            return w, (None if lin.bias is None else runtime.f32c(lin.bias))

        w_qkv, b_qkv = packed(att._packed, "lin_qkv", att.lin_qkv)
        w_proj, b_proj = packed(att._packed, "projection", att.projection)
        w1 = self._mlp.cache.get(("w", 0, dtype), [fc1.weight], lambda: runtime.pack_weight([fc1.weight], dtype))
        w2 = self._mlp.cache.get(("w", 1, dtype), [fc2.weight], lambda: runtime.pack_weight([fc2.weight], dtype))
# ... 53 lines not shown
```

### anemoi_models_amd/ops.py

```python

from __future__ import annotations

from typing import Optional

import torch
from torch import Tensor

from . import _lib

_DT = {torch.float32: _lib.F32, torch.bfloat16: _lib.BF16}

PROFILE: Optional[list] = None


class _Timed:
    __slots__ = ("name", "work", "start")

    def __init__(self, name: str, **work) -> None:
        self.name, self.work, self.start = name, work, None

    def __enter__(self):
        if PROFILE is not None:
            self.start = torch.cuda.Event(enable_timing=True)
            self.start.record(torch.cuda.current_stream())
        return self

    def __exit__(self, *exc):
        if self.start is not None:
            end = torch.cuda.Event(enable_timing=True)
            end.record(torch.cuda.current_stream())
            PROFILE.append((self.name, self.start, end, self.work))
        return False


def dtype_code(dtype: torch.dtype) -> int:
    try:
        return _DT[dtype]
    except KeyError:
        raise NotImplementedError(f"compute dtype {dtype} is not supported (float32 or bfloat16)") from None


def k_multiple(dtype: torch.dtype) -> int:
    return 128 // torch.empty((), dtype=dtype).element_size()


def round_up(n: int, m: int) -> int:
    return (n + m - 1) // m * m


def _dev(*tensors: Optional[Tensor]) -> None:
    for t in tensors:
        if t is not None and not t.is_cuda:
            raise RuntimeError(
                "anemoi_models_amd kernels run on an MI355X only: got a CPU tensor (there is no CPU fallback)"
            )


_raw_stream = getattr(torch._C, "_cuda_getCurrentRawStream", None)


def _stream() -> int:
    if _raw_stream is not None:
        return _raw_stream(torch.cuda.current_device())
    return torch.cuda.current_stream().cuda_stream


def _rows(t: Tensor) -> Tensor:
    if t.dim() != 2 or (t.shape[1] > 1 and t.stride(1) != 1):
        raise ValueError(f"expected a row-major 2-D tensor (unit inner stride), got shape {tuple(t.shape)} "
                         f"strides {t.stride()}")
    return t


def _ld(t: Tensor) -> int:
    return t.stride(0) if t.shape[0] > 1 else max(t.stride(0), t.shape[1])


def _ptr(t: Optional[Tensor]) -> Optional[int]:
    return None if t is None else t.data_ptr()


def layer_norm(x: Tensor, weight: Tensor, bias: Tensor, eps: float = 1e-5, out: Optional[Tensor] = None,
               residual: Optional[Tensor] = None) -> Tensor:
    _dev(x, weight, bias, out, residual)
    _rows(x)
    if out is None:
        out = torch.empty((x.shape[0], x.shape[1]), dtype=x.dtype, device=x.device)
    if residual is not None:
        if residual.dtype != x.dtype or residual.shape != x.shape:
            raise ValueError("layer_norm: the residual must have the shape and dtype of x")
        with _Timed("layer_norm", bytes=3 * x.shape[0] * x.shape[1] * x.element_size()):
            st = _lib.load().anemoi_layer_norm_residual(dtype_code(x.dtype), x.data_ptr(), _ld(x), weight.data_ptr(),
                                                        bias.data_ptr(), residual.data_ptr(), _ld(_rows(residual)),
                                                        out.data_ptr(), _ld(_rows(out)), x.shape[0], x.shape[1], eps, _stream())
        _lib.check(st, "anemoi_layer_norm_residual")
        return out
    with _Timed("layer_norm", bytes=2 * x.shape[0] * x.shape[1] * x.element_size()):
        st = _lib.load().anemoi_layer_norm(dtype_code(x.dtype), x.data_ptr(), _ld(x), weight.data_ptr(),
                                           bias.data_ptr(), out.data_ptr(), _ld(_rows(out)), x.shape[0], x.shape[1],
                                           eps, _stream())
    _lib.check(st, "anemoi_layer_norm")
    return out


def layer_norm_with_stats(x: Tensor, weight: Tensor, bias: Tensor, eps: float = 1e-5):
    _dev(x, weight, bias)
    _rows(x)
    out = torch.empty((x.shape[0], x.shape[1]), dtype=x.dtype, device=x.device)
    stats = torch.empty((x.shape[0], 2), dtype=torch.float32, device=x.device)
    st = _lib.load().anemoi_layer_norm_stats(dtype_code(x.dtype), x.data_ptr(), _ld(x), weight.data_ptr(), bias.data_ptr(),
                                             out.data_ptr(), _ld(out), stats.data_ptr(), x.shape[0], x.shape[1], eps,
                                             _stream())
    _lib.check(st, "anemoi_layer_norm_stats")
    return out, stats


def _carry_stats(y: Tensor, eps: float, stats: Tensor) -> None:
    y._anemoi_row_stats = (eps, stats, y.data_ptr(), y._version)


def _carried_stats(x: Tensor, eps: float) -> Optional[Tensor]:
    rec = getattr(x, "_anemoi_row_stats", None)
    if rec is None:
        return None
    r_eps, stats, ptr, version = rec
    if r_eps != eps or stats.shape[0] != x.shape[0] or ptr != x.data_ptr() or version != x._version:
        return None
    return stats


def row_stats(x: Tensor, eps: float = 1e-5) -> Tensor:
    _dev(x)
    _rows(x)
    carried = _carried_stats(x, eps)
    if carried is not None:
        return carried
    out = torch.empty((x.shape[0], 2), dtype=torch.float32, device=x.device)
    with _Timed("row_stats", bytes=x.shape[0] * x.shape[1] * x.element_size()):
        st = _lib.load().anemoi_row_stats(dtype_code(x.dtype), x.data_ptr(), _ld(x), out.data_ptr(), x.shape[0],
                                          x.shape[1], eps, _stream())
    _lib.check(st, "anemoi_row_stats")
    return out


def linear(x: Tensor, w: Tensor, bias: Optional[Tensor] = None, *, act: str = "Identity",
           residual: Optional[Tensor] = None, out: Optional[Tensor] = None, out_dtype: Optional[torch.dtype] = None,
           n_out: Optional[int] = None, ln=None, stats_eps: Optional[float] = None) -> Tensor:
    _dev(x, w, bias, residual, out)
    _rows(x)
    if w.dtype != x.dtype or not w.is_contiguous():
        raise ValueError("linear: weight must be contiguous and in the activation dtype")
    n = w.shape[0] if n_out is None else n_out
    k = w.shape[1]
    if x.shape[1] != k:
        raise ValueError(f"linear: x has {x.shape[1]} columns, weight expects {k}")
    if out is None:
        out = torch.empty((x.shape[0], n), dtype=out_dtype or x.dtype, device=x.device)
    if act not in _lib.ACT_CODES:
        raise RuntimeError(f"activation {act} is not supported by the fused Linear kernel")
    if x.shape[0] == 0:
        return out
    alg = (x.shape[0] * k + n * k) * x.element_size() + x.shape[0] * n * (out.element_size() + (
        0 if residual is None else residual.element_size()))
    fuse_stats = stats_eps is not None and act == "Identity" and out.dtype == x.dtype and _rows(out).shape[1] == n
    with _Timed("linear", flops=2 * x.shape[0] * n * k, bytes=alg, m=x.shape[0], n=n, k=k):
        if fuse_stats:
            stats_in = colsum = None
            if ln is not None:
                stats_in, colsum = ln
                _dev(stats_in, colsum)
            m_rows = x.shape[0]
            ws = torch.empty((m_rows * max(n // 128, 1), 2), dtype=torch.float32, device=x.device)
            stats_out = torch.empty((m_rows, 2), dtype=torch.float32, device=x.device)
            st = _lib.load().anemoi_linear_stats(
                dtype_code(x.dtype), x.data_ptr(), _ld(x), w.data_ptr(), _ptr(bias), _ptr(colsum), _ptr(stats_in),
                _ptr(residual), 0 if residual is None else _ld(_rows(residual)), out.data_ptr(), _ld(_rows(out)), m_rows,
                n, k, ws.data_ptr(), ws.numel() * 4, stats_eps, stats_out.data_ptr(), _stream())
            _carry_stats(out, stats_eps, stats_out)
        elif ln is None:
            st = _lib.load().anemoi_linear(
                dtype_code(x.dtype), dtype_code(out.dtype), x.data_ptr(), _ld(x), w.data_ptr(), _ptr(bias),
                _ptr(residual), 0 if residual is None else _ld(_rows(residual)), out.data_ptr(), _ld(_rows(out)),
                x.shape[0], n, k, _lib.ACT_CODES[act], _stream())
        else:
            stats, colsum = ln
            _dev(stats, colsum)
            if stats.shape != (x.shape[0], 2) or stats.dtype != torch.float32 or not stats.is_contiguous():
                raise ValueError("linear: ln stats must be the contiguous [M, 2] f32 result of row_stats(x)")
            if colsum.numel() < n or colsum.dtype != torch.float32 or not colsum.is_contiguous():
                raise ValueError("linear: ln colsum must be a contiguous f32 vector with one entry per output column")
            st = _lib.load().anemoi_linear_ln(
                dtype_code(x.dtype), dtype_code(out.dtype), x.data_ptr(), _ld(x), w.data_ptr(), _ptr(bias),
                colsum.data_ptr(), stats.data_ptr(), _ptr(residual),
                0 if residual is None else _ld(_rows(residual)), out.data_ptr(), _ld(_rows(out)), x.shape[0], n, k,
                _lib.ACT_CODES[act], _stream())
    _lib.check(st, "anemoi_linear" if ln is None else "anemoi_linear_ln")
    return out


def edge_attr_csr(a0: Tensor, a1: Optional[Tensor], perm: Tensor, ld_out: Optional[int] = None,
                  one_col: int = -1) -> Tensor:
    _dev(a0, a1, perm)
    d0 = a0.shape[1]
    d1 = 0 if a1 is None else a1.shape[1]
    ld = round_up(d0 + d1, 4) if ld_out is None else ld_out
    a0 = a0.contiguous().float()
    a1 = None if a1 is None else a1.contiguous().float()
    out = torch.empty((perm.shape[0], ld), dtype=torch.float32, device=a0.device)
    if perm.shape[0] == 0:
        return out
    st = _lib.load().anemoi_edge_attr_csr(a0.data_ptr(), d0, _ptr(a1), d1, a0.shape[0], perm.data_ptr(),
                                          out.data_ptr(), ld, one_col, perm.shape[0], _stream())
    _lib.check(st, "anemoi_edge_attr_csr")
    return out


def gt_edge_attention(q: Tensor, k: Tensor, v: Tensor, x_r: Optional[Tensor], edge_attr: Tensor, edge_dim: int,
                      w_edge: Tensor, b_edge: Tensor, rowptr: Tensor, col: Tensor, num_heads: int,
                      out: Optional[Tensor] = None) -> Tensor:
    _dev(q, k, v, x_r, edge_attr, w_edge, b_edge, rowptr, col, out)
    n_dst, c = _rows(q).shape
    if _ld(_rows(k)) != _ld(_rows(v)):
        raise ValueError("gt_edge_attention: k and v must share their leading dimension")
    if out is None:
        out = torch.empty((n_dst, c), dtype=q.dtype, device=q.device)
    if rowptr.dtype != torch.int32 or col.dtype != torch.int32 or rowptr.shape[0] != n_dst + 1:
        raise ValueError("gt_edge_attention: rowptr/col must be int32 with rowptr of length n_dst + 1")
    if col.shape[0] == 0:
        col = torch.zeros(1, dtype=torch.int32, device=q.device)
        edge_attr = torch.zeros((1, max(4, round_up(edge_dim, 4))), dtype=torch.float32, device=q.device)
    alg_bytes = (2 * n_dst + 2 * k.shape[0]) * c * q.element_size() + col.shape[0] * 52 + (n_dst + 1) * 4
    with _Timed("gt_edge_attention", bytes=alg_bytes, n_dst=n_dst, n_src=k.shape[0], edges=col.shape[0]):
        st = _lib.load().anemoi_gt_edge_attention(
            dtype_code(q.dtype), q.data_ptr(), _ld(q), k.data_ptr(), v.data_ptr(), _ld(k), _ptr(x_r),
            0 if x_r is None else _ld(_rows(x_r)), edge_attr.data_ptr(),
            edge_attr.stride(0) if edge_attr.shape[0] > 1 else edge_attr.shape[1], edge_dim, w_edge.data_ptr(),
            b_edge.data_ptr(), rowptr.data_ptr(), col.data_ptr(), out.data_ptr(), _ld(_rows(out)), n_dst, c,
            num_heads, _stream())
    _lib.check(st, "anemoi_gt_edge_attention")
    return out


def gt_edge_attention_folded(q: Tensor, k: Tensor, v: Tensor, x_r: Optional[Tensor], u: Tensor, edge_attr: Tensor,
                             rowptr: Tensor, col: Tensor, num_heads: int, up: int, out: Optional[Tensor] = None,
                             ld_out: Optional[int] = None, lse: Optional[Tensor] = None, runs=None, sched=None,
                             tiles=None) -> Tensor:
    _dev(q, k, v, x_r, u, edge_attr, rowptr, col, out, lse)
    if lse is not None and (lse.dtype != torch.float32 or not lse.is_contiguous()
                            or tuple(lse.shape) != (_rows(q).shape[0], num_heads)):
        raise ValueError("gt_edge_attention_folded: lse must be a contiguous f32 [n_dst, H] tensor")
    n_dst, c = _rows(q).shape
    if _ld(_rows(k)) != _ld(_rows(v)):
        raise ValueError("gt_edge_attention_folded: k and v must share their leading dimension")
    width = c + num_heads * up
    ld = width if ld_out is None else ld_out
    if out is None:
        out = torch.empty((n_dst, ld), dtype=q.dtype, device=q.device)
        if ld > width:
            out[:, width:].zero_()
    if rowptr.dtype != torch.int32 or col.dtype != torch.int32 or rowptr.shape[0] != n_dst + 1:
        raise ValueError("gt_edge_attention_folded: rowptr/col must be int32 with rowptr of length n_dst + 1")
    if edge_attr.shape[0] != col.shape[0] or (col.shape[0] > 0 and (edge_attr.shape[1] != up or
                                                                      not edge_attr.is_contiguous())):
        raise ValueError("gt_edge_attention_folded: edge_attr must be contiguous [E, up]")
    if col.shape[0] == 0:
        col = torch.zeros(1, dtype=torch.int32, device=q.device)
        edge_attr = torch.zeros((1, up), dtype=torch.float32, device=q.device)
    alg_bytes = (2 * n_dst + 2 * k.shape[0]) * c * q.element_size() + col.shape[0] * 52 + (n_dst + 1) * 4
    fused_bytes = alg_bytes + n_dst * ((0 if x_r is None else c) + 2 * num_heads * up) * q.element_size()
    with _Timed("gt_edge_attention", bytes=alg_bytes, fused_bytes=fused_bytes, n_dst=n_dst, n_src=k.shape[0], edges=col.shape[0]):
        if runs is not None and len(runs) == 3:
            grp_ptr, grp_perm, grp_dst = runs
            _dev(grp_ptr, grp_perm, grp_dst)
            if (grp_ptr.dtype != torch.int32 or grp_perm.dtype != torch.int32 or grp_dst.dtype != torch.int32
                    or grp_perm.shape[0] != n_dst or grp_dst.shape[0] != n_dst):
                raise ValueError("gt_edge_attention_folded: runs = (int32 grp_ptr [n_groups + 1], int32 grp_perm [n_dst], "
                                 "int32 grp_dst [n_dst])")
            st = _lib.load().anemoi_gt_edge_attention_folded_groups(
                dtype_code(q.dtype), q.data_ptr(), _ld(q), k.data_ptr(), v.data_ptr(), _ld(_rows(k)), _ptr(x_r),
                0 if x_r is None else _ld(_rows(x_r)), u.data_ptr(), _ld(_rows(u)), edge_attr.data_ptr(), up,
                rowptr.data_ptr(), col.data_ptr(), grp_ptr.data_ptr(), grp_dst.data_ptr(), grp_perm.data_ptr(),
                grp_ptr.shape[0] - 1, _rows(k).shape[0], out.data_ptr(), _ld(_rows(out)), _ptr(lse), n_dst, c, num_heads,
                _stream())
        elif runs is not None:
            run_ptr, perm = runs
            _dev(run_ptr, perm)
            if run_ptr.dtype != torch.int32 or perm.dtype != torch.int32 or perm.shape[0] != run_ptr.shape[0] - 1:
                raise ValueError("gt_edge_attention_folded: runs = (int32 run_ptr [n_runs + 1], int32 perm [n_runs])")
            st = _lib.load().anemoi_gt_edge_attention_folded_runs(
                dtype_code(q.dtype), q.data_ptr(), _ld(q), k.data_ptr(), v.data_ptr(), _ld(_rows(k)), _ptr(x_r),
                0 if x_r is None else _ld(_rows(x_r)), u.data_ptr(), _ld(_rows(u)), edge_attr.data_ptr(), up,
                rowptr.data_ptr(), col.data_ptr(), run_ptr.data_ptr(), perm.data_ptr(), run_ptr.shape[0] - 1,
                out.data_ptr(), _ld(_rows(out)), _ptr(lse), n_dst, c, num_heads, _stream())
        elif tiles is not None:
            _dev(tiles.hdr, tiles.dst, tiles.src, tiles.slot, tiles.xcd)
            st = _lib.load().anemoi_gt_edge_attention_folded_tiles(
                dtype_code(q.dtype), q.data_ptr(), _ld(q), k.data_ptr(), v.data_ptr(), _ld(_rows(k)), _ptr(x_r),
                0 if x_r is None else _ld(_rows(x_r)), u.data_ptr(), _ld(_rows(u)), edge_attr.data_ptr(), up,
                rowptr.data_ptr(), col.data_ptr(), tiles.hdr.data_ptr(), tiles.dst.data_ptr(), tiles.src.data_ptr(),
                tiles.slot.data_ptr(), tiles.xcd.data_ptr(), tiles.max_tiles_per_xcd, tiles.src_cap, tiles.edge_cap,
                _rows(k).shape[0], col.shape[0], out.data_ptr(), _ld(_rows(out)), _ptr(lse), n_dst, c, num_heads, _stream())
        elif sched is not None:
            _dev(sched)
            if sched.dtype != torch.int32 or sched.dim() != 3 or sched.shape[0] != 8 or not sched.is_contiguous():
                raise ValueError("gt_edge_attention_folded: sched = contiguous int32 [8, slots, steps]")
            st = _lib.load().anemoi_gt_edge_attention_folded_sched(
                dtype_code(q.dtype), q.data_ptr(), _ld(q), k.data_ptr(), v.data_ptr(), _ld(_rows(k)), _ptr(x_r),
                0 if x_r is None else _ld(_rows(x_r)), u.data_ptr(), _ld(_rows(u)), edge_attr.data_ptr(), up,
                rowptr.data_ptr(), col.data_ptr(), sched.data_ptr(), sched.shape[1], sched.shape[2], _rows(k).shape[0],
                col.shape[0], out.data_ptr(), _ld(_rows(out)), _ptr(lse), n_dst, c, num_heads, _stream())
        else:
            st = _lib.load().anemoi_gt_edge_attention_folded(
                dtype_code(q.dtype), q.data_ptr(), _ld(q), k.data_ptr(), v.data_ptr(), _ld(_rows(k)), _ptr(x_r),
                0 if x_r is None else _ld(_rows(x_r)), u.data_ptr(), _ld(_rows(u)), edge_attr.data_ptr(), up,
                rowptr.data_ptr(), col.data_ptr(), out.data_ptr(), _ld(_rows(out)), _ptr(lse), n_dst, c, num_heads, _stream())
    _lib.check(st, "anemoi_gt_edge_attention_folded")
    return out


def gt_conv(q: Tensor, k: Tensor, v: Tensor, edges_csr: Tensor, rowptr: Tensor, col: Tensor, num_heads: int,
            x_r: Optional[Tensor] = None, lse: Optional[Tensor] = None, dropout_p: float = 0.0, dropout_seed: int = 0,
            seed_dev: Optional[Tensor] = None) -> Tensor:
    if not 0.0 <= dropout_p <= 1.0:
        raise ValueError(f"dropout probability has to be between 0 and 1, but got {dropout_p}")
    _dev(q, k, v, edges_csr, rowptr, col, x_r, lse)
    n_dst, c = _rows(q).shape
    if _ld(_rows(k)) != _ld(_rows(v)):
        raise ValueError("gt_conv: k and v must share their leading dimension")
    if rowptr.dtype != torch.int32 or col.dtype != torch.int32 or rowptr.shape[0] != n_dst + 1:
        raise ValueError("gt_conv: rowptr/col must be int32 with rowptr of length n_dst + 1")
    if edges_csr.shape[0] != col.shape[0] or edges_csr.dtype != q.dtype:
        raise ValueError("gt_conv: edges must be [E, C] in the activation dtype")
    out = torch.empty((n_dst, c), dtype=q.dtype, device=q.device)
    if col.shape[0] == 0:
        if lse is not None:
            lse.fill_(float("-inf"))
        return out.zero_() if x_r is None else out.copy_(x_r)
    alg_bytes = (2 * n_dst + 2 * k.shape[0] + col.shape[0]) * c * q.element_size() + col.shape[0] * 4 + (n_dst + 1) * 4
    with _Timed("gt_conv", bytes=alg_bytes, n_dst=n_dst, n_src=k.shape[0], edges=col.shape[0]):
        st = _lib.load().anemoi_gt_conv(dtype_code(q.dtype), q.data_ptr(), _ld(q), k.data_ptr(), v.data_ptr(), _ld(_rows(k)),
                                        edges_csr.data_ptr(), _ld(_rows(edges_csr)), _ptr(x_r),
                                        0 if x_r is None else _ld(_rows(x_r)), rowptr.data_ptr(), col.data_ptr(),
                                        out.data_ptr(), _ld(out), _ptr(lse), n_dst, c, num_heads, float(dropout_p),
                                        int(dropout_seed) & 0xFFFFFFFF, _seed_dev_ptr(seed_dev, q), _stream())
    _lib.check(st, "anemoi_gt_conv")
    return out


def gather_add_act(t: Tensor, p_dst: Tensor, p_src: Tensor, dst: Tensor, src: Tensor, act: str = "Identity",
                   out: Optional[Tensor] = None) -> Tensor:
    _dev(t, p_dst, p_src, dst, src, out)
    e, c = _rows(t).shape
    if out is None:
        out = torch.empty((e, c), dtype=t.dtype, device=t.device)
    if e == 0:
        return out
    if dst.dtype != torch.int32 or src.dtype != torch.int32 or dst.shape[0] != e or src.shape[0] != e:
        raise ValueError("gather_add_act: dst / src must be int32 [E]")
    with _Timed("gather_add_act", bytes=(2 * e + p_dst.shape[0] + p_src.shape[0]) * c * t.element_size() + 8 * e):
        st = _lib.load().anemoi_gather_add_act(dtype_code(t.dtype), t.data_ptr(), _ld(t), p_dst.data_ptr(),
                                               _ld(_rows(p_dst)), p_src.data_ptr(), _ld(_rows(p_src)), dst.data_ptr(),
                                               src.data_ptr(), out.data_ptr(), _ld(_rows(out)), e, c,
                                               _lib.ACT_CODES[act], _stream())
    _lib.check(st, "anemoi_gather_add_act")
    return out


def segment_sum(v: Tensor, rowptr: Tensor, out: Optional[Tensor] = None, cat_with: Optional[Tensor] = None) -> Tensor:
    _dev(v, rowptr, out, cat_with)
    n_dst = rowptr.shape[0] - 1
    c = _rows(v).shape[1]
    if cat_with is not None:
        x = _rows(cat_with)
        if x.shape != (n_dst, c) or x.dtype != v.dtype or out is not None:
            raise ValueError("segment_sum: cat_with must be [n_dst, C] of v's dtype (and no out=)")
        out = torch.empty((n_dst, 2 * c), dtype=v.dtype, device=v.device)
        if v.shape[0] == 0:
            out[:, :c].copy_(x)
            out[:, c:].zero_()
            return out
        with _Timed("segment_sum", bytes=(v.shape[0] + 3 * n_dst) * c * v.element_size()):
            st = _lib.load().anemoi_segment_sum_cat(dtype_code(v.dtype), v.data_ptr(), _ld(v), rowptr.data_ptr(),
                                                    x.data_ptr(), _ld(x), out.data_ptr(), 2 * c, n_dst, c, _stream())
        _lib.check(st, "anemoi_segment_sum_cat")
        return out
    if out is None:
        out = torch.empty((n_dst, c), dtype=v.dtype, device=v.device)
    if v.shape[0] == 0:
        return out.zero_()
    with _Timed("segment_sum", bytes=(v.shape[0] + n_dst) * c * v.element_size()):
        st = _lib.load().anemoi_segment_sum(dtype_code(v.dtype), v.data_ptr(), _ld(v), rowptr.data_ptr(),
                                            out.data_ptr(), _ld(_rows(out)), n_dst, c, _stream())
    _lib.check(st, "anemoi_segment_sum")
    return out


def _seed_dev_ptr(seed_dev: Optional[Tensor], like: Tensor):
    if seed_dev is None:
        return None
    if not seed_dev.is_cuda or seed_dev.device != like.device or seed_dev.numel() < 1 or seed_dev.element_size() < 4:
        raise ValueError("dropout seed_dev must be an integer tensor (>= 32 bits per element) on the input's device")
    return seed_dev.data_ptr()


def mhsa(qkv: Tensor, batch_size: int, num_heads: int, window: int = -1, out: Optional[Tensor] = None,
         return_lse: bool = False, dropout_p: float = 0.0, dropout_seed: int = 0, head_offset: int = 0,
         heads_total: int = 0, seed_dev: Optional[Tensor] = None):
    _dev(qkv, out)
    rows, c3 = _rows(qkv).shape
    c = c3 // 3
    s_len = rows // batch_size
    d = c // num_heads
    if out is None:
        out = torch.empty((rows, c), dtype=qkv.dtype, device=qkv.device)
    lib = _lib.load()
    code = dtype_code(qkv.dtype)
    ws_bytes = lib.anemoi_mhsa_workspace_bytes(code, batch_size, s_len, num_heads, d)
    ws = torch.empty(ws_bytes, dtype=torch.uint8, device=qkv.device) if ws_bytes > 0 else None
    lse = torch.empty((batch_size, num_heads, s_len), dtype=torch.float32, device=qkv.device) if return_lse else None
    with _Timed("mhsa", flops=4 * batch_size * num_heads * s_len * s_len * d, s=s_len, h=num_heads, d=d):
        st = lib.anemoi_mhsa(code, qkv.data_ptr(), _ld(qkv), out.data_ptr(), _ld(_rows(out)), _ptr(ws), _ptr(lse),
                             batch_size, s_len, num_heads, d, window, float(dropout_p), int(dropout_seed) & 0xFFFFFFFF,
                             _seed_dev_ptr(seed_dev, qkv), int(head_offset), int(heads_total), _stream())
    _lib.check(st, "anemoi_mhsa")
    return (out, lse) if return_lse else out


def mhsa_backward(qkv: Tensor, out: Tensor, dout: Tensor, lse: Tensor, batch_size: int, num_heads: int,
                  window: int = -1, dropout_p: float = 0.0, dropout_seed: int = 0, head_offset: int = 0,
                  heads_total: int = 0, use_mfma: bool = True, seed_dev: Optional[Tensor] = None) -> Tensor:
    _dev(qkv, out, dout, lse)
    rows, c3 = _rows(qkv).shape
    c = c3 // 3
    s_len = rows // batch_size
    dqkv = torch.empty((rows, c3), dtype=qkv.dtype, device=qkv.device)
    delta = torch.empty((batch_size, num_heads, s_len), dtype=torch.float32, device=qkv.device)
    if lse.dtype != torch.float32 or not lse.is_contiguous() or lse.numel() != delta.numel():
        raise ValueError("mhsa_backward: lse must be the contiguous f32 [B, H, S] output of mhsa(return_lse=True)")
    lib = _lib.load()
    ws_bytes = lib.anemoi_mhsa_backward_workspace_bytes(dtype_code(qkv.dtype), batch_size, s_len, num_heads, c // num_heads)
    ws = torch.empty(ws_bytes, dtype=torch.uint8, device=qkv.device) if ws_bytes > 0 and use_mfma else None
    st = lib.anemoi_mhsa_backward(dtype_code(qkv.dtype), qkv.data_ptr(), _ld(qkv), out.data_ptr(), _ld(_rows(out)),
                                  dout.data_ptr(), _ld(_rows(dout)), lse.data_ptr(), delta.data_ptr(), dqkv.data_ptr(), c3,
                                  _ptr(ws), batch_size, s_len, num_heads, c // num_heads, window, float(dropout_p),
                                  int(dropout_seed) & 0xFFFFFFFF, _seed_dev_ptr(seed_dev, qkv), int(head_offset),
                                  int(heads_total), _stream())
    _lib.check(st, "anemoi_mhsa_backward")
    return dqkv


def assemble_nodes(x: Optional[Tensor], latlons: Tensor, trainable: Optional[Tensor], batch_size: int,
                   dtype: torch.dtype, ld_out: Optional[int] = None, ensemble: int = 1, in_affine=None,
                   rows: Optional[Tensor] = None) -> Tensor:
    _dev(x, latlons, trainable, rows)
    mul = add = None
    if in_affine is not None and x is not None:
        mul, add = (t.contiguous().float() for t in in_affine)
        _dev(mul, add)
        if mul.numel() != x.shape[-1] or add.numel() != x.shape[-1]:
            raise ValueError("assemble_nodes: in_affine needs one (mul, add) pair per input variable")
    g = latlons.shape[0]
    n_ll = latlons.shape[1]
    n_tr = 0 if trainable is None else trainable.shape[1]
    if x is not None:
        b, t, ens, gx, v = x.shape
        if gx != g or b != batch_size:
            raise ValueError(f"assemble_nodes: x has shape {tuple(x.shape)} but the graph has {g} nodes")
        x = x.contiguous().float()
    else:
        b, t, ens, v = batch_size, 0, ensemble, 0
    width = t * v + n_ll + n_tr
    ld = width if ld_out is None else ld_out
    latlons = latlons.contiguous().float()
    trainable = None if trainable is None else trainable.contiguous().float()
    if rows is not None:
        if b != 1 or ens != 1 or rows.dtype != torch.int64 or rows.dim() != 1:
            raise ValueError("assemble_nodes: rows needs batch 1, ensemble 1 and a 1-d int64 id list")
        rows = rows.contiguous()
        out = torch.empty((rows.shape[0], ld), dtype=dtype, device=latlons.device)
        st = _lib.load().anemoi_assemble_node_rows(dtype_code(dtype), _ptr(x), t, g, v, latlons.data_ptr(), n_ll,
                                                   _ptr(trainable), n_tr, rows.data_ptr(), rows.shape[0], out.data_ptr(),
                                                   ld, _ptr(mul), _ptr(add), _stream())
        _lib.check(st, "anemoi_assemble_node_rows")
        return out
    out = torch.empty((b * ens * g, ld), dtype=dtype, device=latlons.device)
    st = _lib.load().anemoi_assemble_nodes(dtype_code(dtype), _ptr(x), b, t, ens, g, v, latlons.data_ptr(), n_ll,
                                           _ptr(trainable), n_tr, out.data_ptr(), ld, _ptr(mul), _ptr(add), _stream())
    _lib.check(st, "anemoi_assemble_nodes")
    return out


def finalize_output(y: Tensor, x: Tensor, src: Tensor, in_affine=None, out_affine=None,
                    rows: Optional[Tensor] = None) -> Tensor:
    _dev(y, x, src, rows)
    if y.dtype != torch.float32 or not y.is_contiguous():
        raise ValueError("finalize_output: y must be contiguous float32")
    x = x.contiguous().float()
    b, t, ens, g, v_in = x.shape
    if src.dtype != torch.int32 or src.numel() != y.shape[-1]:
        raise ValueError("finalize_output: src must be int32 with one entry per output column")
    im = ia = om = oa = None
    if in_affine is not None:
        im, ia = (t_.contiguous().float() for t_ in in_affine)
    if out_affine is not None:
        om, oa = (t_.contiguous().float() for t_ in out_affine)
    _dev(im, ia, om, oa)
    if rows is not None:
        if b != 1 or ens != 1 or rows.dtype != torch.int64 or rows.dim() != 1 or y.numel() != rows.shape[0] * y.shape[-1]:
            raise ValueError("finalize_output: rows needs batch 1, ensemble 1, a 1-d int64 id list and one y row per id")
        rows = rows.contiguous()
        st = _lib.load().anemoi_finalize_output_rows(y.data_ptr(), y.shape[-1], x.data_ptr(), t, g, v_in, src.data_ptr(),
                                                     rows.data_ptr(), rows.shape[0], _ptr(im), _ptr(ia), _ptr(om), _ptr(oa),
                                                     _stream())
        _lib.check(st, "anemoi_finalize_output_rows")
        return y
    st = _lib.load().anemoi_finalize_output(y.data_ptr(), y.shape[-1], x.data_ptr(), b, t, ens, g, v_in, src.data_ptr(),
                                            _ptr(im), _ptr(ia), _ptr(om), _ptr(oa), _stream())
    _lib.check(st, "anemoi_finalize_output")
    return y


def bound_output(y: Tensor, op_col: Tensor, op_lo: Tensor, op_hi: Tensor, op_mul: Tensor,
                 fin: Optional[tuple] = None) -> Tensor:
    _dev(y, op_col, op_lo, op_hi, op_mul)
    if y.dtype != torch.float32 or not y.is_contiguous():
        raise ValueError("bound_output: y must be contiguous float32")
    n_ops = op_col.numel()
    if op_col.dtype != torch.int32 or op_mul.dtype != torch.int32 or op_lo.dtype != torch.float32 or \
            op_hi.dtype != torch.float32 or op_lo.numel() != n_ops or op_hi.numel() != n_ops or op_mul.numel() != n_ops:
        raise ValueError("bound_output: op lists must be int32 / float32 vectors of one length")
    fc = fm = fa = None
    if fin is not None:
        fc, fm, fa = fin
        _dev(fc, fm, fa)
        if fc.dtype != torch.int32 or fm.dtype != torch.float32 or fa.dtype != torch.float32 or \
                fm.numel() != fc.numel() or fa.numel() != fc.numel():
            raise ValueError("bound_output: fin = (int32 columns, f32 mul, f32 add) of one length")
    v_out = y.shape[-1]
    st = _lib.load().anemoi_bound_output(y.data_ptr(), v_out, y.numel() // max(v_out, 1), n_ops, _ptr(op_col),
                                         _ptr(op_lo), _ptr(op_hi), _ptr(op_mul), 0 if fc is None else fc.numel(),
                                         _ptr(fc), _ptr(fm), _ptr(fa), _stream())
    _lib.check(st, "anemoi_bound_output")
    return y


def advance_input(x: Tensor, y: Tensor, colmap: Tensor, forcing: Optional[Tensor] = None) -> Tensor:
    _dev(x, y, colmap, forcing)
    if x.dtype != torch.float32 or y.dtype != torch.float32 or not x.is_contiguous() or not y.is_contiguous():
        raise ValueError("advance_input: x and y must be contiguous float32")
    b, t, ens, g, v_in = x.shape
    if tuple(y.shape[:3]) != (b, ens, g) or colmap.dtype != torch.int32 or colmap.numel() != v_in:
        raise ValueError(f"advance_input: y {tuple(y.shape)} / colmap do not match x {tuple(x.shape)}")
    f = 0
    if forcing is not None:
        if forcing.dtype != torch.float32 or not forcing.is_contiguous() or tuple(forcing.shape[:3]) != (b, ens, g):
            raise ValueError("advance_input: forcing must be contiguous float32 [B, Ens, G, F]")
        f = forcing.shape[-1]
    st = _lib.load().anemoi_advance_input(x.data_ptr(), b, t, ens, g, v_in, y.data_ptr(), y.shape[-1], _ptr(forcing), f,
                                          colmap.data_ptr(), _stream())
    _lib.check(st, "anemoi_advance_input")
    return x


def prognostic_residual(y: Tensor, x: Tensor, out_idx: Tensor, in_idx: Tensor) -> Tensor:
    _dev(y, x, out_idx, in_idx)
    if y.dtype != torch.float32 or not y.is_contiguous():
        raise ValueError("prognostic_residual: y must be contiguous float32")
    b, t, ens, g, v_in = x.shape
    x = x.contiguous().float()
    st = _lib.load().anemoi_prognostic_residual(y.data_ptr(), y.shape[-1], x.data_ptr(), b, t, ens, g, v_in,
                                                out_idx.data_ptr(), in_idx.data_ptr(), out_idx.shape[0], _stream())
    _lib.check(st, "anemoi_prognostic_residual")
    return y


def convert_pad(src: Tensor, dtype: torch.dtype, ld_out: Optional[int] = None) -> Tensor:
    _dev(src)
    _rows(src)
    rows, cols = src.shape
    ld = cols if ld_out is None else ld_out
    out = torch.empty((rows, ld), dtype=dtype, device=src.device)
    if rows == 0:
        return out
    st = _lib.load().anemoi_convert_pad(dtype_code(src.dtype), src.data_ptr(), _ld(src), dtype_code(dtype),
                                        out.data_ptr(), ld, rows, cols, _stream())
    _lib.check(st, "anemoi_convert_pad")
    return out


def add(a: Tensor, b: Tensor, out: Optional[Tensor] = None) -> Tensor:
    _dev(a, b, out)
    if a.shape != b.shape or a.dtype != b.dtype:
        raise ValueError("add: shape / dtype mismatch")
    if out is None:
        out = torch.empty(a.shape, dtype=a.dtype, device=a.device)
    st = _lib.load().anemoi_add(dtype_code(a.dtype), a.data_ptr(), _ld(_rows(a)), b.data_ptr(), _ld(_rows(b)),
                                out.data_ptr(), _ld(_rows(out)), a.shape[0], a.shape[1], _stream())
    _lib.check(st, "anemoi_add")
    return out


def transpose(x: Tensor, ld_out: Optional[int] = None) -> Tensor:
    _dev(x)
    rows, cols = _rows(x).shape
    ld = rows if ld_out is None else ld_out
    out = torch.empty((cols, ld), dtype=x.dtype, device=x.device)
    st = _lib.load().anemoi_transpose(dtype_code(x.dtype), x.data_ptr(), _ld(x), out.data_ptr(), ld, rows, cols, _stream())
    _lib.check(st, "anemoi_transpose")
    return out


def col_sum(x: Tensor, out: Optional[Tensor] = None) -> Tensor:
    _dev(x)
    rows, cols = _rows(x).shape
    lib = _lib.load()
    if out is None:
        out = torch.empty(cols, dtype=torch.float32, device=x.device)
    elif out.dtype != torch.float32 or out.numel() != cols or not out.is_contiguous():
        raise ValueError("col_sum: out must be a contiguous f32 vector of the column count")
    n_ws = lib.anemoi_col_sum_workspace_floats(rows, cols)
    ws = torch.empty(max(n_ws, 1), dtype=torch.float32, device=x.device)
    st = lib.anemoi_col_sum(dtype_code(x.dtype), x.data_ptr(), _ld(x), rows, cols, out.data_ptr(), ws.data_ptr(), n_ws,
# ... 188 lines not shown
```

### include/anemoi_amd.h

```cpp
#ifndef ANEMOI_AMD_H
#define ANEMOI_AMD_H

#include <stdint.h>

#ifdef __cplusplus
extern "C" {
#endif

#define ANEMOI_OK 0
#define ANEMOI_ERR_INVALID 1
#define ANEMOI_ERR_UNSUPPORTED 2
#define ANEMOI_ERR_LAUNCH 3

#define ANEMOI_F32 0
#define ANEMOI_BF16 1

#define ANEMOI_ACT_NONE 0
#define ANEMOI_ACT_GELU 1
#define ANEMOI_ACT_SILU 2
#define ANEMOI_ACT_RELU 3

typedef void* anemoi_stream_t;

int anemoi_abi_version(void);
const char* anemoi_build_info(void);
const char* anemoi_last_error(void);

int anemoi_layer_norm(int dtype, const void* x, int64_t ldx, const float* gamma, const float* beta, void* y,
                      int64_t ldy, int64_t rows, int C, float eps, anemoi_stream_t stream);

int anemoi_layer_norm_residual(int dtype, const void* x, int64_t ldx, const float* gamma, const float* beta,
                               const void* residual, int64_t ldr, void* y, int64_t ldy, int64_t rows, int C, float eps,
                               anemoi_stream_t stream);

int anemoi_layer_norm_stats(int dtype, const void* x, int64_t ldx, const float* gamma, const float* beta, void* y,
                            int64_t ldy, float* stats, int64_t rows, int C, float eps, anemoi_stream_t stream);

int anemoi_linear(int dtype, int out_dtype, const void* x, int64_t ldx, const void* w, const float* bias,
                  const void* residual, int64_t ldr, void* y, int64_t ldy, int64_t M, int N, int K, int act,
                  anemoi_stream_t stream);

int anemoi_row_stats(int dtype, const void* x, int64_t ldx, float* stats, int64_t rows, int C, float eps,
                     anemoi_stream_t stream);

int anemoi_linear_ln(int dtype, int out_dtype, const void* x, int64_t ldx, const void* w, const float* bias,
                     const float* colsum, const float* stats, const void* residual, int64_t ldr, void* y, int64_t ldy,
                     int64_t M, int N, int K, int act, anemoi_stream_t stream);

int anemoi_linear_stats(int dtype, const void* x, int64_t ldx, const void* w, const float* bias, const float* colsum,
                        const float* stats_in, const void* residual, int64_t ldr, void* y, int64_t ldy, int64_t M, int N,
                        int K, void* workspace, int64_t workspace_bytes, float eps, float* stats_out,
                        anemoi_stream_t stream);

int anemoi_edge_attr_csr(const float* a0, int d0, const float* a1, int d1, int64_t rows0, const int32_t* perm,
                         float* out, int ld_out, int one_col, int64_t n_edges, anemoi_stream_t stream);

int anemoi_gt_edge_attention(int dtype, const void* q, int64_t ldq, const void* k, const void* v, int64_t ldkv,
                             const void* x_r, int64_t ldr, const float* edge_attr, int ea_ld, int edge_dim,
                             const float* w_edge, const float* b_edge, const int32_t* rowptr, const int32_t* col,
                             void* out, int64_t ldo, int64_t n_dst, int C, int H, anemoi_stream_t stream);

int anemoi_gt_edge_attention_folded(int dtype, const void* q, int64_t ldq, const void* k, const void* v, int64_t ldkv,
                                    const void* x_r, int64_t ldr, const void* u, int64_t ldu, const float* edge_attr,
                                    int up, const int32_t* rowptr, const int32_t* col, void* out, int64_t ldo, float* lse,
                                    int64_t n_dst, int C, int H, anemoi_stream_t stream);

int anemoi_gt_edge_attention_folded_runs(int dtype, const void* q, int64_t ldq, const void* k, const void* v, int64_t ldkv,
                                         const void* x_r, int64_t ldr, const void* u, int64_t ldu, const float* edge_attr,
                                         int up, const int32_t* rowptr, const int32_t* col, const int32_t* run_ptr,
                                         const int32_t* run_perm, int64_t n_runs, void* out, int64_t ldo, float* lse,
                                         int64_t n_dst, int C, int H, anemoi_stream_t stream);

int anemoi_gt_edge_attention_folded_groups(int dtype, const void* q, int64_t ldq, const void* k, const void* v, int64_t ldkv,
                                           const void* x_r, int64_t ldr, const void* u, int64_t ldu, const float* edge_attr,
                                           int up, const int32_t* rowptr, const int32_t* col, const int32_t* grp_ptr,
                                           const int32_t* grp_dst, const int32_t* grp_perm, int64_t n_groups, int64_t n_src,
                                           void* out, int64_t ldo, float* lse, int64_t n_dst, int C, int H,
                                           anemoi_stream_t stream);

int anemoi_edge_schedule_shape(int dtype, int64_t n_dst, int C, int* slots, int* steps);
int anemoi_gt_edge_attention_folded_sched(int dtype, const void* q, int64_t ldq, const void* k, const void* v, int64_t ldkv,
                                          const void* x_r, int64_t ldr, const void* u, int64_t ldu, const float* edge_attr,
                                          int up, const int32_t* rowptr, const int32_t* col, const int32_t* sched, int slots,
                                          int steps, int64_t n_src, int64_t n_edges, void* out, int64_t ldo, float* lse,
                                          int64_t n_dst, int C, int H, anemoi_stream_t stream);

int anemoi_gt_edge_attention_folded_tiles(int dtype, const void* q, int64_t ldq, const void* k, const void* v, int64_t ldkv,
                                          const void* x_r, int64_t ldr, const void* u, int64_t ldu, const float* edge_attr,
                                          int up, const int32_t* rowptr, const int32_t* col, const int32_t* tile_hdr,
                                          const int32_t* tile_dst, const int32_t* tile_src, const uint8_t* tile_slot,
                                          const int32_t* tile_xcd, int max_tiles_per_xcd, int src_cap, int edge_cap,
                                          int64_t n_src, int64_t n_edges, void* out, int64_t ldo, float* lse, int64_t n_dst,
                                          int C, int H, anemoi_stream_t stream);

int anemoi_gt_conv(int dtype, const void* q, int64_t ldq, const void* k, const void* v, int64_t ldkv, const void* edges,
                   int64_t lde, const void* x_r, int64_t ldr, const int32_t* rowptr, const int32_t* col, void* out,
                   int64_t ldo, float* lse, int64_t n_dst, int C, int H, float dropout_p, uint32_t dropout_seed,
                   const void* dropout_seed_dev, anemoi_stream_t stream);
int anemoi_gt_conv_backward_dst(int dtype, const void* q, int64_t ldq, const void* k, const void* v, int64_t ldkv,
                                const void* edges, int64_t lde, const void* dout, int64_t ldd, const float* lse,
                                const int32_t* rowptr, const int32_t* col, float* alpha, float* w, float* dsum, void* dq,
                                int64_t lddq, int64_t n_dst, int C, int H, float dropout_p, uint32_t dropout_seed,
                                const void* dropout_seed_dev, anemoi_stream_t stream);
int anemoi_gt_conv_backward_src(int dtype, const void* q, int64_t ldq, const void* dout, int64_t ldd, const float* alpha,
                                const float* w, const float* dsum, const int32_t* rowptr_t, const int32_t* eid_t,
                                const int32_t* dst_t, void* dk, void* dv, int64_t ldg, void* dedges, int64_t ldde,
                                int64_t n_src, int C, int H, float dropout_p, uint32_t dropout_seed,
                                const void* dropout_seed_dev, anemoi_stream_t stream);

int anemoi_assemble_nodes(int dtype, const float* x, int B, int T, int Ens, int64_t G, int V, const float* latlons,
                          int n_ll, const float* trainable, int n_tr, void* out, int64_t ldo, const float* in_mul,
                          const float* in_add, anemoi_stream_t stream);

int anemoi_assemble_node_rows(int dtype, const float* x, int T, int64_t G, int V, const float* latlons, int n_ll,
                              const float* trainable, int n_tr, const int64_t* rows, int64_t n_rows, void* out,
                              int64_t ldo, const float* in_mul, const float* in_add, anemoi_stream_t stream);

int anemoi_finalize_output(float* y, int V_out, const float* x, int B, int T, int Ens, int64_t G, int V_in,
                           const int32_t* src, const float* in_mul, const float* in_add, const float* out_mul,
                           const float* out_add, anemoi_stream_t stream);

int anemoi_finalize_output_rows(float* y, int V_out, const float* x, int T, int64_t G, int V_in, const int32_t* src,
                                const int64_t* rows, int64_t n_rows, const float* in_mul, const float* in_add,
                                const float* out_mul, const float* out_add, anemoi_stream_t stream);

int anemoi_bound_output(float* y, int V_out, int64_t rows, int n_ops, const int32_t* op_col, const float* op_lo,
                        const float* op_hi, const int32_t* op_mul, int n_fin, const int32_t* fin_col,
                        const float* fin_mul, const float* fin_add, anemoi_stream_t stream);

int anemoi_prognostic_residual(float* y, int V_out, const float* x, int B, int T, int Ens, int64_t G, int V_in,
                               const int32_t* out_idx, const int32_t* in_idx, int n_prog, anemoi_stream_t stream);

int anemoi_advance_input(float* x, int B, int T, int Ens, int64_t G, int V_in, const float* y, int V_out,
                         const float* forcing, int F, const int32_t* colmap, anemoi_stream_t stream);

int anemoi_convert_pad(int src_dtype, const void* src, int64_t ld_src, int dst_dtype, void* dst, int64_t ld_dst,
                       int64_t rows, int cols, anemoi_stream_t stream);

int anemoi_add(int dtype, const void* a, int64_t lda, const void* b, int64_t ldb, void* y, int64_t ldy, int64_t rows,
               int cols, anemoi_stream_t stream);

int anemoi_gather_add_act(int dtype, const void* t, int64_t ldt, const void* p_dst, int64_t ldpd, const void* p_src,
                          int64_t ldps, const int32_t* dst, const int32_t* src, void* out, int64_t ldo,
                          int64_t n_edges, int C, int act, anemoi_stream_t stream);

int anemoi_segment_sum(int dtype, const void* v, int64_t ldv, const int32_t* rowptr, void* out, int64_t ldo,
                       int64_t n_dst, int C, anemoi_stream_t stream);

int anemoi_segment_sum_cat(int dtype, const void* v, int64_t ldv, const int32_t* rowptr, const void* x, int64_t ldx,
                           void* out, int64_t ldo, int64_t n_dst, int C, anemoi_stream_t stream);

int64_t anemoi_mhsa_workspace_bytes(int dtype, int B, int S, int H, int D);
int anemoi_mhsa(int dtype, const void* qkv, int64_t ld, void* out, int64_t ldo, void* workspace, float* lse, int B, int S,
                int H, int D, int window, float dropout_p, uint32_t dropout_seed, const void* dropout_seed_dev,
                int dropout_h0, int dropout_h_total, anemoi_stream_t stream);

int64_t anemoi_mhsa_backward_workspace_bytes(int dtype, int B, int S, int H, int D);
int anemoi_mhsa_backward(int dtype, const void* qkv, int64_t ld, const void* out, int64_t ldo, const void* dout,
                         int64_t lddo, const float* lse, float* delta, void* dqkv, int64_t lddq, void* workspace, int B,
                         int S, int H, int D, int window, float dropout_p, uint32_t dropout_seed,
                         const void* dropout_seed_dev, int dropout_h0, int dropout_h_total, anemoi_stream_t stream);


int anemoi_transpose(int dtype, const void* src, int64_t ld_src, void* dst, int64_t ld_dst, int64_t rows, int cols,
                     anemoi_stream_t stream);

int64_t anemoi_transpose_colsum_rows(int64_t rows, int64_t chunk_rows);
int anemoi_transpose_chunked(int dtype, const void* src, int64_t ld_src, void* dst, int64_t ld_dst, int64_t rows, int cols,
                             int64_t chunk_rows, float* colsum_partial, anemoi_stream_t stream);

int anemoi_weight_grad_tn(const void* dy, int64_t ldy, const void* x, int64_t ldx, void* partial, int64_t partial_stride,
                          void* bias_partial, int64_t bias_stride, int64_t M, int N, int K, int chunk_rows,
                          anemoi_stream_t stream);

int anemoi_linear_batched(int dtype, int out_dtype, const void* x, int64_t ldx, int64_t stride_x, const void* w,
                          int64_t stride_w, void* y, int64_t ldy, int64_t stride_y, int batch, int64_t M, int N, int K,
                          anemoi_stream_t stream);

int64_t anemoi_col_sum_workspace_floats(int64_t rows, int cols);
int anemoi_col_sum(int dtype, const void* x, int64_t ldx, int64_t rows, int cols, float* out, float* workspace,
                   int64_t workspace_floats, anemoi_stream_t stream);

int anemoi_row_dot(int dtype, const void* a, int64_t lda, const void* b, int64_t ldb, const float* shift, float* out,
                   int64_t rows, int cols, anemoi_stream_t stream);

int anemoi_row_scale(int dtype, const void* x, int64_t ldx, const float* s, float alpha, void* out, int64_t ldo,
                     int64_t rows, int cols, anemoi_stream_t stream);

int anemoi_act_forward(int dtype, int act, const void* pre, int64_t ldp, const void* residual, int64_t ldr, void* out,
                       int64_t ldo, int64_t rows, int cols, anemoi_stream_t stream);

int anemoi_act_backward(int dtype, int act, const void* pre, int64_t ldp, const void* dy, int64_t ldd, void* out,
                        int64_t ldo, int64_t rows, int cols, anemoi_stream_t stream);

int anemoi_linear_dual(int dtype, const void* x, int64_t ldx, const void* w, const float* bias, void* pre, int64_t ldp,
                       void* y, int64_t ldy, int64_t M, int N, int K, int act, anemoi_stream_t stream);

int anemoi_linear_actgrad(int dtype, const void* x, int64_t ldx, const void* w, const void* pre, int64_t ldp, void* y,
                          int64_t ldy, int64_t M, int N, int K, int act, anemoi_stream_t stream);

int64_t anemoi_layer_norm_backward_workspace_floats(int64_t rows, int C);
int anemoi_layer_norm_backward(int dtype, const void* x, int64_t ldx, const float* stats, const float* gamma,
                               const void* dy, int64_t ldd, const void* dres, int64_t ldr, void* dx, int64_t ldo,
                               int64_t rows, int C, float* dgamma, float* dbeta, float* workspace,
                               int64_t workspace_floats, anemoi_stream_t stream);

int anemoi_gt_edge_attention_folded_backward_dst(int dtype, const void* q, int64_t ldq, const void* k, const void* v,
                                                 int64_t ldkv, const void* dout, int64_t ldd, const void* u, int64_t ldu,
                                                 const void* dt, int64_t lddt, const float* lse, const float* edge_attr,
                                                 int up, const int32_t* rowptr, const int32_t* col, float* alpha,
                                                 float* w, float* dsum, void* dq, int64_t lddq, void* du, int64_t lddu,
                                                 void* dxr, int64_t lddxr, int64_t n_dst, int C, int H,
                                                 anemoi_stream_t stream);
int anemoi_gt_edge_attention_folded_backward_src(int dtype, const void* q, int64_t ldq, const void* dout, int64_t ldd,
                                                 const float* alpha, const float* w, const float* dsum,
                                                 const int32_t* rowptr_t, const int32_t* eid_t, const int32_t* dst_t,
                                                 void* dk, void* dv, int64_t ldg, int64_t n_src, int C, int H,
                                                 anemoi_stream_t stream);
int anemoi_gt_edge_attr_grad(int dtype, const float* alpha, const float* w, const float* dsum, const void* u, int64_t ldu,
                             const void* dt, int64_t lddt, const int32_t* dst_of_edge, float* dattr, int64_t n_edges,
                             int H, int up, int D, anemoi_stream_t stream);

typedef struct anemoi_gt_block_args {
  int64_t struct_bytes;
  int64_t n_dst;
  int32_t dtype;
  int32_t C, H, up;
  int32_t hidden, act;
  int32_t k_proj, n_in;
  float eps_mlp, eps_out;
  const void* x; int64_t ldx; const float* x_stats;
  const void* w_in; const float* b_in; const float* cs_in;
  void* sq; int64_t ld_sq;
  const void* q; const void* k; const void* v; const void* x_r; const void* u;
  int64_t ldq, ldkv, ldr, ldu;
  const float* edge_attr; const int32_t* rowptr; const int32_t* col;
  void* att; int64_t ld_att;
  const void* w_proj; const float* b_proj; const void* res; int64_t ld_res; void* y; float* y_stats;
  const void* w_fc1; const float* b_fc1; const float* cs_fc1; void* h;
  const void* w_fc2; const float* b_fc2; void* out; float* out_stats;
  void* stats_ws; int64_t stats_ws_bytes;
  const int32_t* run_ptr; const int32_t* run_perm; int64_t n_runs;
  const int32_t* sched; int32_t sched_slots, sched_steps; int64_t n_src;
  const int32_t* run_dst;
  int64_t n_edges;
  const int32_t* tile_hdr; const int32_t* tile_dst; const int32_t* tile_src; const uint8_t* tile_slot; const int32_t* tile_xcd;
  int32_t tile_max_per_xcd, tile_src_cap, tile_edge_cap, tile_pad;
} anemoi_gt_block_args;
int anemoi_gt_block_tail(const anemoi_gt_block_args* args, anemoi_stream_t stream);
int anemoi_gt_processor_block_forward(const anemoi_gt_block_args* args, anemoi_stream_t stream);

typedef struct anemoi_tfm_block_args {
  int64_t struct_bytes;
  int64_t rows;
  int32_t dtype;
  int32_t B, S, C, H;
  int32_t hidden, act;
  int32_t window;
  float eps1, eps2;
  float dropout_p; uint32_t dropout_seed; const void* dropout_seed_dev; int32_t dropout_h0, dropout_h_total;
  const void* x; int64_t ldx;
  const float* ln1_w; const float* ln1_b; const float* ln2_w; const float* ln2_b;
  const void* w_qkv; const float* b_qkv;
  const void* w_proj; const float* b_proj;
  const void* w_fc1; const float* b_fc1;
  const void* w_fc2; const float* b_fc2;
  void* h_ln;
  void* qkv;
  void* att;
  void* y;
  void* h;
  void* mhsa_ws;
  void* out;
} anemoi_tfm_block_args;
int anemoi_transformer_block_forward(const anemoi_tfm_block_args* args, anemoi_stream_t stream);

#ifdef __cplusplus
}
#endif
#endif
```

Baseline: 19.13 million.

## Fuse decoder LN-linear projection with degree-3 edge attention in one kernel

Adds a fused decoder kernel that computes the folded q/x_r/u projection of the layer-normed destination rows with MFMA on LDS tiles and immediately runs the degree-3 edge attention in the same block. A new mapper block entry point runs this kernel and then the existing projection/MLP tail. The goal is to avoid writing and re-reading the intermediate squ product and to save a launch. It only applies to bf16, K=256, uniform degree-3 plans without halo or chunking, and it adds complex double-buffered DMA logic.

```diff
diff --git a/anemoi_models_amd/_lib.py b/anemoi_models_amd/_lib.py
--- a/anemoi_models_amd/_lib.py
+++ b/anemoi_models_amd/_lib.py
@@ -26,7 +26,7 @@
 ACT_NONE, ACT_GELU, ACT_SILU, ACT_RELU = 0, 1, 2, 3
 ACT_CODES = {"Identity": ACT_NONE, "GELU": ACT_GELU, "SiLU": ACT_SILU, "ReLU": ACT_RELU}
 
-ABI_VERSION = 41
+ABI_VERSION = 42
 
 
 class GtBlockArgs(ctypes.Structure):
@@ -105,6 +105,9 @@
                                                        c_int64, c_void_p, c_int64, c_void_p, c_int, c_void_p, c_void_p,
                                                        c_void_p, c_void_p, c_void_p, c_int64, c_int64, c_void_p, c_int64,
                                                        c_void_p, c_int64, c_int, c_int, c_void_p]),
+    "anemoi_gt_decoder_fused": (c_int, [c_void_p, c_int64, c_int64, c_void_p, c_void_p, c_void_p, c_void_p, c_void_p,
+                                        c_void_p, c_int64, c_void_p, c_int, c_void_p, c_void_p, c_void_p, c_int64, c_void_p,
+                                        c_int64, c_void_p, c_int64, c_int, c_int, c_void_p]),
     "anemoi_edge_schedule_shape": (c_int, [c_int, c_int64, c_int, c_void_p, c_void_p]),
     "anemoi_gt_edge_attention_folded_sched": (c_int, [c_int, c_void_p, c_int64, c_void_p, c_void_p, c_int64, c_void_p,
                                                       c_int64, c_void_p, c_int64, c_void_p, c_int, c_void_p, c_void_p,
@@ -192,6 +195,7 @@
     "anemoi_add": (c_int, [c_int, c_void_p, c_int64, c_void_p, c_int64, c_void_p, c_int64, c_int64, c_int, c_void_p]),
     "anemoi_gt_block_tail": (c_int, [ctypes.POINTER(GtBlockArgs), c_void_p]),
     "anemoi_gt_processor_block_forward": (c_int, [ctypes.POINTER(GtBlockArgs), c_void_p]),
+    "anemoi_gt_mapper_block_forward": (c_int, [ctypes.POINTER(GtBlockArgs), c_void_p]),
     "anemoi_transformer_block_forward": (c_int, [ctypes.POINTER(TfmBlockArgs), c_void_p]),
 }
 
diff --git a/anemoi_models_amd/csrc/blocks.hip b/anemoi_models_amd/csrc/blocks.hip
--- a/anemoi_models_amd/csrc/blocks.hip
+++ b/anemoi_models_amd/csrc/blocks.hip
@@ -4,7 +4,7 @@
 
 namespace {
 
-int check_args(const anemoi_gt_block_args* a, const char* who, bool with_input) {
+int check_args(const anemoi_gt_block_args* a, const char* who, bool with_input, bool mapper = false) {
   ANEMOI_REQUIRE(a != nullptr, ANEMOI_ERR_INVALID, "%s: null argument block", who);
   ANEMOI_REQUIRE(a->struct_bytes == (int64_t)sizeof(anemoi_gt_block_args), ANEMOI_ERR_INVALID,
                  "%s: argument block of %lld bytes, this library expects %lld (header / binding out of sync)", who,
@@ -28,12 +28,18 @@
     ANEMOI_REQUIRE(a->n_in >= 4 * a->C + a->H * a->up && a->ld_sq >= a->n_in && a->ldx >= a->C, ANEMOI_ERR_INVALID,
                    "%s: input product of %d columns (ld %lld) cannot hold x_r | q | k | v | u = %d", who, a->n_in,
                    (long long)a->ld_sq, 4 * a->C + a->H * a->up);
+  } else if (mapper) {
+    ANEMOI_REQUIRE(a->x && a->x_stats && a->w_in && a->b_in && a->cs_in && a->k && a->v && a->res && a->run_dst && a->run_perm &&
+                       a->n_src > 0,
+                   ANEMOI_ERR_INVALID, "%s: null pointer (input product, k / v, residual or group lists)", who);
   } else {
     ANEMOI_REQUIRE(a->q && a->k && a->v && a->x_r && a->u && a->res, ANEMOI_ERR_INVALID,
                    "%s: null pointer (edge phase operands / residual)", who);
   }
   return ANEMOI_OK;
 }
+
+int run_proj_mlp(const anemoi_gt_block_args* a, anemoi_stream_t stream);
 
 int run_tail(const anemoi_gt_block_args* a, anemoi_stream_t stream) {
   int st;
@@ -56,6 +62,11 @@
                                               a->edge_attr, a->up, a->rowptr, a->col, a->run_ptr, a->run_perm, a->n_runs,
                                               a->att, a->ld_att, nullptr, a->n_dst, a->C, a->H, stream);
   if (st != ANEMOI_OK) return st;
+  return run_proj_mlp(a, stream);
+}
+
+int run_proj_mlp(const anemoi_gt_block_args* a, anemoi_stream_t stream) {
+  int st;
   st = anemoi_linear_stats(a->dtype, a->att, a->ld_att, a->w_proj, a->b_proj, nullptr, nullptr, a->res, a->ld_res, a->y,
                            a->C, a->n_dst, a->C, a->k_proj, a->stats_ws, a->stats_ws_bytes, a->eps_mlp, a->y_stats, stream);
   if (st != ANEMOI_OK) return st;
@@ -99,6 +110,18 @@
   return run_tail(&a, stream);
 }
 
+extern "C" int anemoi_gt_mapper_block_forward(const anemoi_gt_block_args* args, anemoi_stream_t stream) {
+  const char* who = "anemoi_gt_mapper_block_forward";
+  int st = check_args(args, who, false, true);
+  if (st != ANEMOI_OK) return st;
+  if (args->n_dst == 0) return ANEMOI_OK;
+  st = anemoi_gt_decoder_fused(args->x, args->ldx, args->ldx, args->x_stats, args->w_in, args->b_in, args->cs_in, args->k,
+                               args->v, args->ldkv, args->edge_attr, args->up, args->col, args->run_dst, args->run_perm,
+                               args->n_src, args->att, args->ld_att, nullptr, args->n_dst, args->C, args->H, stream);
+  if (st != ANEMOI_OK) return st;
+  return run_proj_mlp(args, stream);
+}
+
 extern "C" int anemoi_transformer_block_forward(const anemoi_tfm_block_args* a, anemoi_stream_t stream) {
   const char* who = "anemoi_transformer_block_forward";
   ANEMOI_REQUIRE(a != nullptr, ANEMOI_ERR_INVALID, "%s: null argument block", who);
diff --git a/anemoi_models_amd/csrc/decoder_fused.hip b/anemoi_models_amd/csrc/decoder_fused.hip
--- /dev/null
+++ b/anemoi_models_amd/csrc/decoder_fused.hip
@@ -0,0 +1,376 @@
+#include <cstdlib>
+
+#include "common.hpp"
+#include "edge_common.hpp"
+
+namespace anemoi {
+
+namespace {
+
+typedef __attribute__((ext_vector_type(8))) __bf16 dfbf16x8_t;
+typedef __attribute__((ext_vector_type(4))) float dff32x4_t;
+typedef __attribute__((ext_vector_type(2))) float dff32x2_t;
+typedef uint32_t dfu32x4_t __attribute__((ext_vector_type(4)));
+typedef uint32_t dfu32x2_t __attribute__((ext_vector_type(2)));
+
+constexpr int DF_TR = 32;
+constexpr int DF_K = 256;
+constexpr int DF_KS = DF_K / 32;
+constexpr int DF_ROW_BYTES = DF_K * 2;
+constexpr int DF_A_BYTES = DF_TR * DF_ROW_BYTES;
+constexpr int DF_OCOLS = 144;
+constexpr int DF_O_STRIDE = DF_OCOLS * 2;
+constexpr int DF_LDS = 2 * DF_A_BYTES + DF_TR * DF_O_STRIDE;
+
+struct DecoderFusedParams {
+  const bf16_t* x;
+  const float2* stats;
+  const bf16_t* w;
+  const float* b;
+  const float* cs;
+  const bf16_t* k;
+  const bf16_t* v;
+  const float* attr;
+  const int32_t* col;
+  const int32_t* grp_dst;
+  const int32_t* grp_perm;
+  bf16_t* out;
+  float* lse;
+  int64_t ldx, ldkv, ldo, n_dst, n_tiles;
+  int C, H;
+  float scale;
+};
+
+__device__ __forceinline__ int df_load_idx(const DecoderFusedParams& p, int64_t t, int lane) {
+  const int64_t e = t * DF_TR + (lane & 31);
+  if (t < 0 || e >= p.n_dst) return -1;
+  return lane < 32 ? p.grp_dst[e] : p.grp_perm[e];
+}
+
+}
+
+template <int UP>
+__global__ __launch_bounds__(256) void gt_decoder_fused_kernel(const DecoderFusedParams p) {
+  constexpr int VEC = 8, LPH = 8;
+  constexpr int APL = attrs_per_lane(UP, LPH);
+  static_assert(UP % APL == 0 && APL * LPH >= UP && APL == 2, "a lane owns two attributes or none");
+  extern __shared__ __attribute__((aligned(16))) char smem[];
+  char* const otile = smem + 2 * DF_A_BYTES;
+  const int lane = threadIdx.x & 63;
+  const int wid = __builtin_amdgcn_readfirstlane((int)(threadIdx.x >> 6));
+  const int xcd = blockIdx.x & 7;
+  const int bix = blockIdx.x >> 3, bpx = gridDim.x >> 3;
+  const int head = bix % p.H;
+  const int part = bix / p.H, nparts = bpx / p.H;
+  const int64_t t0 = p.n_tiles * xcd / 8, t1 = p.n_tiles * (xcd + 1) / 8;
+  if (t0 + part >= t1) return;
+  const int C = p.C;
+
+  const int fr = lane & 15, fq = lane >> 4;
+  int wrow[3];
+  bool wok[3];
+#pragma unroll
+  for (int cb = 0; cb < 2; ++cb) {
+    const int lc = (2 * wid + cb) * 16 + fr;
+    wrow[cb] = lc < 64 ? head * 64 + lc : C + head * 64 + (lc - 64);
+    wok[cb] = true;
+  }
+  wrow[2] = 2 * C + head * UP + (fr < UP ? fr : 0);
+  wok[2] = fr < UP;
+  dfbf16x8_t wf[3][DF_KS];
+#pragma unroll
+  for (int cb = 0; cb < 3; ++cb)
+#pragma unroll
+    for (int ks = 0; ks < DF_KS; ++ks) {
+      const dfu32x4_t raw = wok[cb] ? *reinterpret_cast<const dfu32x4_t*>(p.w + (int64_t)wrow[cb] * DF_K + ks * 32 + fq * 8)
+                                    : dfu32x4_t{0u, 0u, 0u, 0u};
+      wf[cb][ks] = __builtin_bit_cast(dfbf16x8_t, raw);
+    }
+  float bv[3][4], sv[3][4];
+#pragma unroll
+  for (int cb = 0; cb < 3; ++cb)
+#pragma unroll
+    for (int i = 0; i < 4; ++i) {
+      const int lc = 4 * fq + i;
+      int n;
+      bool ok = true;
+      if (cb < 2) {
+        const int c = (2 * wid + cb) * 16 + lc;
+        n = c < 64 ? head * 64 + c : C + head * 64 + (c - 64);
+      } else {
+        ok = lc < UP;
+        n = 2 * C + head * UP + (ok ? lc : 0);
+      }
+      bv[cb][i] = ok ? p.b[n] : 0.f;
+      sv[cb][i] = ok ? p.cs[n] : 0.f;
+    }
+
+  const uint32_t x_bytes = (uint32_t)(p.n_dst * p.ldx * 2);
+  const __amdgpu_buffer_rsrc_t xrs = __builtin_amdgcn_make_buffer_rsrc(const_cast<bf16_t*>(p.x), 0, (int)x_bytes, 0x00020000);
+  const __amdgpu_buffer_rsrc_t krs = __builtin_amdgcn_make_buffer_rsrc(const_cast<bf16_t*>(p.k), 0, -1, 0x00020000);
+  const __amdgpu_buffer_rsrc_t vrs = __builtin_amdgcn_make_buffer_rsrc(const_cast<bf16_t*>(p.v), 0, -1, 0x00020000);
+  const __amdgpu_buffer_rsrc_t ars = __builtin_amdgcn_make_buffer_rsrc(const_cast<float*>(p.attr), 0, -1, 0x00020000);
+  const __amdgpu_buffer_rsrc_t ors = __builtin_amdgcn_make_buffer_rsrc(p.out, 0, -1, 0x00020000);
+  const uint32_t kv_row_bytes = (uint32_t)(p.ldkv * 2), o_row_bytes = (uint32_t)(p.ldo * 2), x_row_bytes = (uint32_t)(p.ldx * 2);
+
+  const int j = lane & 7;
+  const int m_att = wid * 8 + (lane >> 3);
+  const int a0 = j * APL;
+  const bool a_own = a0 < UP;
+  const int a_ld = a_own ? a0 : 0;
+  const float amask = a_own ? 1.f : 0.f;
+  const int kv_lane_off = (head * 64 + j * VEC) * 2;
+
+  auto dma_tile = [&](int idx, int buf) {
+#pragma unroll
+    for (int i = 0; i < 4; ++i) {
+      const int rr = wid * 8 + 2 * i + (lane >> 5);
+      const int node = __shfl(idx, rr, 64);
+      const int chunk = (lane & 31) ^ (rr & 7);
+      const int voff = node >= 0 ? (int)((uint32_t)node * x_row_bytes + (uint32_t)chunk * 16) : (int)x_bytes;
+      __builtin_amdgcn_raw_ptr_buffer_load_lds(
+          xrs, (__attribute__((address_space(3))) void*)(smem + buf * DF_A_BYTES + (wid * 8 + 2 * i) * DF_ROW_BYTES), 16, voff,
+          0, 0, 0);
+    }
+  };
+  auto load_src = [&](int idx) -> int {
+    const int node = __shfl(idx, m_att, 64), pm = __shfl(idx, 32 + m_att, 64);
+    const int s = j < 3 ? j : 0;
+    return node >= 0 ? p.col[3 * node + ((pm >> (2 * s)) & 3)] : 0;
+  };
+
+  struct Gather {
+    dfu32x4_t kr[3], vr[3];
+    float at[3][APL];
+  };
+  auto gather = [&](int idx, int srcw, Gather& g) {
+    const int node = __shfl(idx, m_att, 64), pm = __shfl(idx, 32 + m_att, 64);
+    const int nd = node >= 0 ? node : 0;
+#pragma unroll
+    for (int s = 0; s < 3; ++s) {
+      const int src = __shfl(srcw, (lane & ~7) + s, 64);
+      const int row = (int)((uint32_t)src * kv_row_bytes);
+      g.kr[s] = __builtin_amdgcn_raw_buffer_load_b128(krs, kv_lane_off + row, 0, 0);
+      g.vr[s] = __builtin_amdgcn_raw_buffer_load_b128(vrs, kv_lane_off + row, 0, 0);
+    }
+#pragma unroll
+    for (int s = 0; s < 3; ++s) {
+      const int erow = 3 * nd + ((node >= 0 ? pm : 0) >> (2 * s) & 3);
+      const dfu32x2_t t = __builtin_amdgcn_raw_buffer_load_b64(ars, (int)((uint32_t)erow * (uint32_t)(UP * 4) + a_ld * 4), 0, 0);
+      g.at[s][0] = __uint_as_float(t.x);
+      g.at[s][1] = __uint_as_float(t.y);
+    }
+  };
+
+  int64_t t = t0 + part;
+  int idx_cur = df_load_idx(p, t, lane);
+  int idx_nxt = df_load_idx(p, t + nparts < t1 ? t + nparts : -1, lane);
+  int src_cur = load_src(idx_cur);
+  dma_tile(idx_cur, 0);
+  int buf = 0;
+
+  for (; t < t1; t += nparts) {
+    const bool has_next = t + nparts < t1;
+    asm volatile("s_waitcnt vmcnt(0)" ::: "memory");
+    __builtin_amdgcn_sched_barrier(0);
+    __builtin_amdgcn_s_barrier();
+    __builtin_amdgcn_sched_barrier(0);
+
+    float2 st[2];
+#pragma unroll
+    for (int rb = 0; rb < 2; ++rb) {
+      const int node = __shfl(idx_cur, rb * 16 + fr, 64);
+      float2 s = p.stats[node >= 0 ? node : 0];
+      asm volatile("" : "+v"(s.x), "+v"(s.y));
+      st[rb] = s;
+    }
+    Gather g;
+    gather(idx_cur, src_cur, g);
+    if (has_next) dma_tile(idx_nxt, buf ^ 1);
+    const int src_nxt = has_next ? load_src(idx_nxt) : 0;
+    const int idx_nn = df_load_idx(p, t + 2 * nparts < t1 ? t + 2 * nparts : -1, lane);
+
+    dff32x4_t acc[2][2], accu;
+#pragma unroll
+    for (int cb = 0; cb < 2; ++cb)
+#pragma unroll
+      for (int rb = 0; rb < 2; ++rb) acc[cb][rb] = dff32x4_t{0.f, 0.f, 0.f, 0.f};
+    accu = dff32x4_t{0.f, 0.f, 0.f, 0.f};
+    const char* abuf = smem + buf * DF_A_BYTES;
+#pragma unroll
+    for (int ks = 0; ks < DF_KS; ++ks) {
+      dfbf16x8_t bx[2];
+#pragma unroll
+      for (int rb = 0; rb < 2; ++rb) {
+        const int row = rb * 16 + fr;
+        const int slot = (ks * 4 + fq) ^ (row & 7);
+        bx[rb] = *reinterpret_cast<const dfbf16x8_t*>(abuf + row * DF_ROW_BYTES + slot * 16);
+      }
+#pragma unroll
+      for (int cb = 0; cb < 2; ++cb)
+#pragma unroll
+        for (int rb = 0; rb < 2; ++rb)
+          acc[cb][rb] = __builtin_amdgcn_mfma_f32_16x16x32_bf16(wf[cb][ks], bx[rb], acc[cb][rb], 0, 0, 0);
+      if (wid < 2) accu = __builtin_amdgcn_mfma_f32_16x16x32_bf16(wf[2][ks], wid == 0 ? bx[0] : bx[1], accu, 0, 0, 0);
+    }
+    auto epi = [&](const dff32x4_t& a, const float2& s, const float (&bb)[4], const float (&ss)[4], int row, int col) {
+      const dff32x2_t r2 = dff32x2_t{s.x, s.x}, t2 = dff32x2_t{s.y, s.y};
+      dff32x2_t p0 = dff32x2_t{a[0], a[1]}, p1 = dff32x2_t{a[2], a[3]};
+      p0 = p0 * r2 + (t2 * dff32x2_t{ss[0], ss[1]} + dff32x2_t{bb[0], bb[1]});
+      p1 = p1 * r2 + (t2 * dff32x2_t{ss[2], ss[3]} + dff32x2_t{bb[2], bb[3]});
+      *reinterpret_cast<dfu32x2_t*>(otile + row * DF_O_STRIDE + col * 2) =
+          dfu32x2_t{pack_bf16x2(p0.x, p0.y), pack_bf16x2(p1.x, p1.y)};
+    };
+#pragma unroll
+    for (int cb = 0; cb < 2; ++cb)
+#pragma unroll
+      for (int rb = 0; rb < 2; ++rb) epi(acc[cb][rb], st[rb], bv[cb], sv[cb], rb * 16 + fr, (2 * wid + cb) * 16 + 4 * fq);
+    if (wid < 2) epi(accu, wid == 0 ? st[0] : st[1], bv[2], sv[2], wid * 16 + fr, 128 + 4 * fq);
+    asm volatile("s_waitcnt lgkmcnt(0)" ::: "memory");
+    __builtin_amdgcn_sched_barrier(0);
+    __builtin_amdgcn_s_barrier();
+    __builtin_amdgcn_sched_barrier(0);
+
+    {
+      const int node = __shfl(idx_cur, m_att, 64);
+      const char* orow = otile + m_att * DF_O_STRIDE;
+      const dfu32x4_t qv = *reinterpret_cast<const dfu32x4_t*>(orow + (64 + j * VEC) * 2);
+      const dfu32x4_t xv = *reinterpret_cast<const dfu32x4_t*>(orow + (j * VEC) * 2);
+      RawWords<bf16_t, APL> uw;
+      uw.w[0] = *reinterpret_cast<const uint32_t*>(orow + (128 + a_ld) * 2);
+      QK<bf16_t, VEC> qk;
+      {
+        const uint32_t qw[4] = {qv.x, qv.y, qv.z, qv.w};
+        qk.set_raw(qw);
+      }
+      float u[APL];
+      uw.get(u);
+      float sc[3];
+#pragma unroll
+      for (int sl = 0; sl < 3; ++sl) {
+        float tt = qk.dot(__builtin_bit_cast(uint4, g.kr[sl]));
+#pragma unroll
+        for (int a = 0; a < APL; ++a) tt = fmaf(u[a] * amask, g.at[sl][a], tt);
+        sc[sl] = group_sum<LPH>(tt) * p.scale;
+      }
+      const float m = fmaxf(fmaxf(sc[0], sc[1]), sc[2]);
+      float l = 0.f;
+      dff32x2_t accv[VEC / 2];
+      float tacc[APL];
+#pragma unroll
+      for (int i = 0; i < VEC / 2; ++i) accv[i] = dff32x2_t{0.f, 0.f};
+#pragma unroll
+      for (int a = 0; a < APL; ++a) tacc[a] = 0.f;
+#pragma unroll
+      for (int sl = 0; sl < 3; ++sl) {
+        const float pe = __expf(sc[sl] - m);
+        l += pe;
+        float vv[VEC];
+        unpack<bf16_t, VEC>(__builtin_bit_cast(uint4, g.vr[sl]), vv);
+#pragma unroll
+        for (int i = 0; i < VEC / 2; ++i)
+          accv[i] = __builtin_elementwise_fma(dff32x2_t{pe, pe}, dff32x2_t{vv[2 * i], vv[2 * i + 1]}, accv[i]);
+#pragma unroll
+        for (int a = 0; a < APL; ++a) tacc[a] = fmaf(pe, g.at[sl][a], tacc[a]);
+      }
+      const float inv = 1.0f / (l + 1e-16f);
+      float o[VEC];
+      {
+#pragma clang fp contract(off)
+        RawWords<bf16_t, VEC> xw;
+        xw.w[0] = xv.x; xw.w[1] = xv.y; xw.w[2] = xv.z; xw.w[3] = xv.w;
+        float r[VEC];
+        xw.get(r);
+#pragma unroll
+        for (int i = 0; i < VEC; ++i) {
+          const float scaled = accv[i >> 1][i & 1] * inv;
+          o[i] = scaled + r[i];
+        }
+      }
+      if (node >= 0) {
+        const int out_off = (int)((uint32_t)node * o_row_bytes);
+        uint32_t ow[4];
+        pack_words<bf16_t, VEC>(o, ow);
+        __builtin_amdgcn_raw_buffer_store_b128(dfu32x4_t{ow[0], ow[1], ow[2], ow[3]}, ors, out_off + kv_lane_off, 0, 2);
+        __builtin_amdgcn_sched_barrier(0);
+        asm volatile("s_nop 1" ::: "memory");
+        __builtin_amdgcn_sched_barrier(0);
+        if (a_own) {
+          float t4[APL];
+#pragma unroll
+          for (int a = 0; a < APL; ++a) t4[a] = tacc[a] * inv;
+          uint32_t tw[RawWords<bf16_t, APL>::W];
+          pack_words<bf16_t, APL>(t4, tw);
+          __builtin_amdgcn_raw_buffer_store_b32(tw[0], ors, out_off + (C + head * UP + a0) * 2, 0, 0);
+        }
+        if (p.lse != nullptr && j == 0) p.lse[(int64_t)node * p.H + head] = m + __logf(l + 1e-16f);
+      }
+    }
+    idx_cur = idx_nxt;
+    idx_nxt = idx_nn;
+    src_cur = src_nxt;
+    buf ^= 1;
+  }
+}
+
+}
+
+using namespace anemoi;
+
+extern "C" int anemoi_gt_decoder_fused(const void* x_aug, int64_t ldx, int64_t k_in, const float* x_stats, const void* w_in,
+                                       const float* b_in, const float* cs_in, const void* k, const void* v, int64_t ldkv,
+                                       const float* edge_attr, int up, const int32_t* col, const int32_t* grp_dst,
+                                       const int32_t* grp_perm, int64_t n_src, void* att, int64_t ld_att, float* lse,
+                                       int64_t n_dst, int C, int H, anemoi_stream_t stream) {
+  const char* who = "anemoi_gt_decoder_fused";
+  ANEMOI_REQUIRE(x_aug && x_stats && w_in && b_in && cs_in && k && v && edge_attr && col && grp_dst && grp_perm && att,
+                 ANEMOI_ERR_INVALID, "%s: null pointer", who);
+  ANEMOI_REQUIRE(H > 0 && C == 64 * H && k_in == DF_K && (up == 4 || up == 8 || up == 12 || up == 16), ANEMOI_ERR_UNSUPPORTED,
+                 "%s: takes 64-channel heads, K = %d and up in {4, 8, 12, 16} (C %d, H %d, K %lld, up %d)", who, DF_K, C, H,
+                 (long long)k_in, up);
+  ANEMOI_REQUIRE(ldx >= k_in && ldkv >= C && ld_att >= (int64_t)C + (int64_t)H * up && n_src > 0 && n_dst >= 0,
+                 ANEMOI_ERR_INVALID, "%s: leading dimension too small", who);
+  const int64_t gib4 = (int64_t)1 << 32;
+  ANEMOI_REQUIRE(n_dst * ldx * 2 < gib4 / 2 && n_dst * ld_att * 2 < gib4 / 2 && n_src * ldkv * 2 < gib4 / 2 &&
+                     3 * n_dst * (int64_t)up * 4 < gib4 / 2,
+                 ANEMOI_ERR_UNSUPPORTED, "%s: operands beyond 31-bit byte offsets", who);
+  const bool aligned = (uintptr_t)x_aug % 16 == 0 && (uintptr_t)w_in % 16 == 0 && (uintptr_t)k % 16 == 0 &&
+                       (uintptr_t)v % 16 == 0 && (uintptr_t)att % 16 == 0 && (uintptr_t)edge_attr % 8 == 0 && ldx % 8 == 0 &&
+                       ldkv % 8 == 0 && ld_att % 8 == 0;
+  ANEMOI_REQUIRE(aligned, ANEMOI_ERR_UNSUPPORTED, "%s: operands must be 16-byte aligned", who);
+  if (n_dst == 0) return ANEMOI_OK;
+  DecoderFusedParams p;
+  p.x = static_cast<const bf16_t*>(x_aug);
+  p.stats = reinterpret_cast<const float2*>(x_stats);
+  p.w = static_cast<const bf16_t*>(w_in);
+  p.b = b_in;
+  p.cs = cs_in;
+  p.k = static_cast<const bf16_t*>(k);
+  p.v = static_cast<const bf16_t*>(v);
+  p.attr = edge_attr;
+  p.col = col;
+  p.grp_dst = grp_dst;
+  p.grp_perm = grp_perm;
+  p.out = static_cast<bf16_t*>(att);
+  p.lse = lse;
+  p.ldx = ldx;
+  p.ldkv = ldkv;
+  p.ldo = ld_att;
+  p.n_dst = n_dst;
+  p.n_tiles = (n_dst + DF_TR - 1) / DF_TR;
+  p.C = C;
+  p.H = H;
+  p.scale = 1.0f / sqrtf(64.0f);
+  int parts = (64 + H - 1) / H;
+  const int64_t tiles_per_xcd = (p.n_tiles + 7) / 8;
+  if (parts > tiles_per_xcd) parts = (int)(tiles_per_xcd > 0 ? tiles_per_xcd : 1);
+  const unsigned grid = (unsigned)(8 * H * parts);
+  hipStream_t st = as_stream(stream);
+  switch (up) {
+    case 4: hipLaunchKernelGGL((gt_decoder_fused_kernel<4>), dim3(grid), dim3(256), DF_LDS, st, p); break;
+    case 8: hipLaunchKernelGGL((gt_decoder_fused_kernel<8>), dim3(grid), dim3(256), DF_LDS, st, p); break;
+    case 12: hipLaunchKernelGGL((gt_decoder_fused_kernel<12>), dim3(grid), dim3(256), DF_LDS, st, p); break;
+    default: hipLaunchKernelGGL((gt_decoder_fused_kernel<16>), dim3(grid), dim3(256), DF_LDS, st, p); break;
+  }
+  return check_launch(who);
+}
diff --git a/anemoi_models_amd/csrc/elementwise.hip b/anemoi_models_amd/csrc/elementwise.hip
--- a/anemoi_models_amd/csrc/elementwise.hip
+++ b/anemoi_models_amd/csrc/elementwise.hip
@@ -823,7 +823,7 @@
   return check_launch("anemoi_bound_output");
 }
 
-int anemoi_abi_version(void) { return 41; }
+int anemoi_abi_version(void) { return 42; }
 
 #ifndef ANEMOI_HIPCC_VERSION
 #define ANEMOI_HIPCC_VERSION "unknown (built without anemoi_models_amd/_build.py)"
diff --git a/anemoi_models_amd/layers/block.py b/anemoi_models_amd/layers/block.py
--- a/anemoi_models_amd/layers/block.py
+++ b/anemoi_models_amd/layers/block.py
@@ -198,13 +198,8 @@
     def _ln_linear(self, handle, tag: str, plain, rows, params, **kw) -> Tensor:
         xin, stats, ln = handle
         if isinstance(xin, EmbeddedRows):
-            xa = xin.x_aug
-            wf, bf, zero = self._packed.get(
-                (tag, "embfold", xa.dtype, xa.shape[1], xin.one_col, xin._tag),
-                list(params) + [ln.weight, ln.bias, xin.emb.weight, xin.emb.bias],
-                lambda: runtime.fold_embedded_layer_norm(*rows(), ln.weight, ln.bias, xin.emb.weight, xin.emb.bias,
-                                                         xa.shape[1], xin.one_col, xa.dtype))
-            return ops.linear(xa, wf, bf, ln=(stats, zero), **kw)
+            wf, bf, zero = self._embedded_fold(handle, tag, rows, params)
+            return ops.linear(xin.x_aug, wf, bf, ln=(stats, zero), **kw)
         if stats is None:
             w, b = plain()
             return ops.linear(xin, w, b, **kw)
@@ -212,6 +207,15 @@
             (tag, "lnfold", xin.dtype), list(params) + [ln.weight, ln.bias],
             lambda: runtime.fold_layer_norm(*rows(), ln.weight, ln.bias, xin.dtype))
         return ops.linear(xin, wf, bf, ln=(stats, cs), **kw)
+
+    def _embedded_fold(self, handle, tag: str, rows, params):
+        xin, _, ln = handle
+        xa = xin.x_aug
+        return self._packed.get(
+            (tag, "embfold", xa.dtype, xa.shape[1], xin.one_col, xin._tag),
+            list(params) + [ln.weight, ln.bias, xin.emb.weight, xin.emb.bias],
+            lambda: runtime.fold_embedded_layer_norm(*rows(), ln.weight, ln.bias, xin.emb.weight, xin.emb.bias,
+                                                     xa.shape[1], xin.one_col, xa.dtype))
 
     def _cat_rows(self, layers):
         w = torch.cat([l.weight.detach().float() for l in layers], dim=0)
@@ -313,14 +317,16 @@
         return dict(up=up, w_in=w_in, b_in=b_in, cs_in=cs_in, w_proj=w_proj, b_proj=b_proj, eps_mlp=eps_mlp, act=act, w_fc1=w1,
                     b_fc1=b1, cs_fc1=cs1, w_fc2=w2, b_fc2=b2, eps_ln1=ln.eps)
 
-    def _block_tail(self, q: Tensor, k: Tensor, v: Tensor, x_r: Tensor, u: Tensor, edge_attr_csr: Tensor, plan, res: Tensor,
-                    up: int, out_stats_eps: Optional[float]) -> Optional[Tensor]:
+    def _block_tail(self, q: Optional[Tensor], k: Tensor, v: Tensor, x_r: Optional[Tensor], u: Optional[Tensor],
+                    edge_attr_csr: Tensor, plan, res: Tensor, up: int, out_stats_eps: Optional[float],
+                    fused=None) -> Optional[Tensor]:
         import ctypes
 
         from .. import _lib
 
-        dtype = q.dtype
-        if (ops.PROFILE is not None or dtype != torch.bfloat16 or not q.is_cuda or plan.num_edges == 0 or q.shape[0] == 0
+        dtype = k.dtype
+        n_rows = res.shape[0]
+        if (ops.PROFILE is not None or dtype != torch.bfloat16 or not k.is_cuda or plan.num_edges == 0 or n_rows == 0
                 or not self.block_abi or self._mlp_ln_eps("dst", dtype) is None):
             return None
         if self._dst_mlp is None:
@@ -330,8 +336,8 @@
             return None
         eps_mlp, act, w1, b1, cs1, w2, b2 = mlp
         wp, bp = self._folded_out(dtype, up)
-        n, c, h = q.shape[0], q.shape[1], self.num_heads
-        dev = q.device
+        n, c, h = n_rows, k.shape[1], self.num_heads
+        dev = k.device
         att = torch.empty((n, wp.shape[1]), dtype=dtype, device=dev)
         if wp.shape[1] > c + h * up:
             att[:, c + h * up:].zero_()
@@ -342,11 +348,19 @@
         a.struct_bytes, a.n_dst, a.dtype = ctypes.sizeof(_lib.GtBlockArgs), n, ops.dtype_code(dtype)
         a.C, a.H, a.up, a.hidden, a.act, a.k_proj = c, h, up, w1.shape[0], _lib.ACT_CODES[act], wp.shape[1]
         a.eps_mlp, a.eps_out = eps_mlp, (out_stats_eps if out_stats_eps is not None else 0.0)
-        a.q, a.k, a.v, a.x_r, a.u = q.data_ptr(), k.data_ptr(), v.data_ptr(), x_r.data_ptr(), u.data_ptr()
-        a.ldq, a.ldkv, a.ldr, a.ldu = ops._ld(q), ops._ld(k), ops._ld(x_r), ops._ld(u)
+        a.k, a.v, a.ldkv = k.data_ptr(), v.data_ptr(), ops._ld(k)
+        if fused is None:
+            a.q, a.x_r, a.u = q.data_ptr(), x_r.data_ptr(), u.data_ptr()
+            a.ldq, a.ldr, a.ldu = ops._ld(q), ops._ld(x_r), ops._ld(u)
         a.edge_attr, a.rowptr, a.col = edge_attr_csr.data_ptr(), plan.rowptr.data_ptr(), plan.col.data_ptr()
         runs = edge_runs(plan, dtype)
-        if runs is not None:
+        if fused is not None:
+            x_aug, x_stats, w_in, b_in, cs_in = fused
+            a.x, a.ldx, a.x_stats = x_aug.data_ptr(), ops._ld(x_aug), x_stats.data_ptr()
+            a.w_in, a.b_in, a.cs_in = w_in.data_ptr(), b_in.data_ptr(), cs_in.data_ptr()
+            a.run_ptr, a.run_perm, a.n_runs = runs[0].data_ptr(), runs[1].data_ptr(), runs[0].shape[0] - 1
+            a.run_dst, a.n_src = runs[2].data_ptr(), k.shape[0]
+        elif runs is not None:
             a.run_ptr, a.run_perm, a.n_runs = runs[0].data_ptr(), runs[1].data_ptr(), runs[0].shape[0] - 1
             if len(runs) == 3:
                 a.run_dst, a.n_src = runs[2].data_ptr(), k.shape[0]
@@ -365,7 +379,11 @@
         a.w_fc2, a.b_fc2, a.out = w2.data_ptr(), ops._ptr(b2), out.data_ptr()
         a.out_stats = stats[1].data_ptr() if out_stats_eps is not None else None
         a.stats_ws, a.stats_ws_bytes = ws.data_ptr(), ws.numel() * 4
-        _lib.check(_lib.load().anemoi_gt_block_tail(ctypes.byref(a), ops._stream()), "anemoi_gt_block_tail")
+        if fused is not None:
+            _lib.check(_lib.load().anemoi_gt_mapper_block_forward(ctypes.byref(a), ops._stream()),
+                       "anemoi_gt_mapper_block_forward")
+        else:
+            _lib.check(_lib.load().anemoi_gt_block_tail(ctypes.byref(a), ops._stream()), "anemoi_gt_block_tail")
         if out_stats_eps is not None:
             ops._carry_stats(out, out_stats_eps, stats[1])
         return out
@@ -543,7 +561,21 @@
         del xs
         xd = self._ln_begin(self.layer_norm2, x_dst)
         up = self.fold_width(dtype)
-        if up is not None:
+        runs = self._decoder_fused_runs(x_dst, plan, up, halo, num_chunks)
+        if runs is not None:
+            wp, bp = self._folded_out(dtype, up)
+            fold = self._embedded_fold(xd, "squ", lambda: self._folded_rows(sq_layers, up), self._fold_params(sq_layers))
+            fused = (x_dst.x_aug, xd[1]) + tuple(fold)
+            del xd
+            if not self.update_src_nodes:
+                done = self._block_tail(None, kv[:, :c], kv[:, c:], None, None, edge_attr_csr, plan, h_dst, up, out_stats_eps,
+                                        fused=fused)
+                if done is not None:
+                    return (x_src.h if isinstance(x_src, EmbeddedRows) else x_src), done
+            att = ops.gt_decoder_fused(*fused, kv[:, :c], kv[:, c:], edge_attr_csr, plan.col, runs, self.num_heads, up,
+                                       ld_out=wp.shape[1])
+            sq = None
+        elif up is not None:
             wp, bp = self._folded_out(dtype, up)
             sq = self._ln_linear(xd, "squ", lambda: self._folded_in("squ", sq_layers, dtype, up),
                                  lambda: self._folded_rows(sq_layers, up),
@@ -578,6 +610,19 @@
             x_src = x_src.h
         new_src = self._node_mlp(x_src, "src", num_chunks) if self.update_src_nodes else x_src
         return new_src, new_dst
+
+    def _decoder_fused_runs(self, x_dst, plan, up: Optional[int], halo, num_chunks: int):
+        if (up is None or halo is not None or num_chunks > 1 or not isinstance(x_dst, EmbeddedRows)
+                or x_dst.dtype != torch.bfloat16 or not x_dst.x_aug.is_cuda
+                or os.environ.get("ANEMOI_AMD_DECODER_FUSED", "1") == "0"):
+            return None
+        if plan.num_edges != 3 * x_dst.x_aug.shape[0]:
+            return None
+        c = self.num_heads * self.out_channels_conv
+        if not ops.decoder_fused_supported(x_dst.x_aug, c, self.num_heads, up):
+            return None
+        runs = edge_runs(plan, torch.bfloat16)
+        return runs if runs is not None and len(runs) == 3 else None
 
     def _sharded(self, x, edge_attr: Tensor, edge_index: Tensor, shapes: tuple, batch_size: int, model_comm_group, size=None):
         from .. import autograd
diff --git a/anemoi_models_amd/ops.py b/anemoi_models_amd/ops.py
--- a/anemoi_models_amd/ops.py
+++ b/anemoi_models_amd/ops.py
@@ -318,6 +318,52 @@
     return out
 
 
+DECODER_FUSED_K = 256
+
+
+def decoder_fused_supported(x_aug: Tensor, c: int, num_heads: int, up: int) -> bool:
+    n = x_aug.shape[0]
+    return (x_aug.dtype == torch.bfloat16 and x_aug.dim() == 2 and x_aug.shape[1] == DECODER_FUSED_K and x_aug.is_contiguous()
+            and c == 64 * num_heads and up in (4, 8, 12, 16) and n >= 1024 and not (1 <= n % 256 <= 8)
+            and n * (c + num_heads * up + 64) * 2 < (1 << 31))
+
+
+def gt_decoder_fused(x_aug: Tensor, stats: Tensor, w_in: Tensor, b_in: Tensor, cs_in: Tensor, k: Tensor, v: Tensor,
+                     edge_attr: Tensor, col: Tensor, runs, num_heads: int, up: int, ld_out: Optional[int] = None) -> Tensor:
+    _dev(x_aug, stats, w_in, b_in, cs_in, k, v, edge_attr, col)
+    n_dst = x_aug.shape[0]
+    c = _rows(k).shape[1]
+    width = c + num_heads * up
+    n_in = 2 * c + num_heads * up
+    if not decoder_fused_supported(x_aug, c, num_heads, up):
+        raise NotImplementedError(f"gt_decoder_fused: no kernel for this shape (rows {n_dst}, K {x_aug.shape[1]}, C {c}, "
+                                  f"H {num_heads}, up {up}, {x_aug.dtype})")
+    if runs is None or len(runs) != 3:
+        raise ValueError("gt_decoder_fused: needs the group lists (grp_ptr, grp_perm, grp_dst) of EdgePlan.runs3")
+    _, grp_perm, grp_dst = runs
+    if (stats.dtype != torch.float32 or not stats.is_contiguous() or stats.shape[0] != n_dst
+            or w_in.shape[0] < n_in or w_in.shape[1] != x_aug.shape[1] or not w_in.is_contiguous()
+            or _ld(_rows(k)) != _ld(_rows(v)) or col.shape[0] != 3 * n_dst or edge_attr.shape != (3 * n_dst, up)
+            or grp_dst.shape[0] != n_dst or grp_perm.shape[0] != n_dst):
+        raise ValueError("gt_decoder_fused: operand shapes do not match a uniform-degree-3 plan of this block")
+    ld = width if ld_out is None else ld_out
+    out = torch.empty((n_dst, ld), dtype=x_aug.dtype, device=x_aug.device)
+    if ld > width:
+        out[:, width:].zero_()
+    kk = x_aug.shape[1]
+    flops = 2 * n_dst * kk * n_in
+    esz = x_aug.element_size()
+    alg_bytes = (n_dst * kk * esz + n_dst * 8 + 2 * k.shape[0] * c * esz + col.shape[0] * 52 + 2 * n_dst * 4
+                 + n_dst * width * esz)
+    with _Timed("gt_decoder_fused", flops=flops, bytes=alg_bytes, n_dst=n_dst, n_src=k.shape[0], edges=col.shape[0]):
+        st = _lib.load().anemoi_gt_decoder_fused(
+            x_aug.data_ptr(), _ld(x_aug), kk, stats.data_ptr(), w_in.data_ptr(), b_in.data_ptr(), cs_in.data_ptr(),
+            k.data_ptr(), v.data_ptr(), _ld(_rows(k)), edge_attr.data_ptr(), up, col.data_ptr(), grp_dst.data_ptr(),
+            grp_perm.data_ptr(), _rows(k).shape[0], out.data_ptr(), _ld(out), None, n_dst, c, num_heads, _stream())
+    _lib.check(st, "anemoi_gt_decoder_fused")
+    return out
+
+
 def gt_conv(q: Tensor, k: Tensor, v: Tensor, edges_csr: Tensor, rowptr: Tensor, col: Tensor, num_heads: int,
             x_r: Optional[Tensor] = None, lse: Optional[Tensor] = None, dropout_p: float = 0.0, dropout_seed: int = 0,
             seed_dev: Optional[Tensor] = None) -> Tensor:
diff --git a/include/anemoi_amd.h b/include/anemoi_amd.h
--- a/include/anemoi_amd.h
+++ b/include/anemoi_amd.h
@@ -77,6 +77,12 @@
                                            const int32_t* grp_dst, const int32_t* grp_perm, int64_t n_groups, int64_t n_src,
                                            void* out, int64_t ldo, float* lse, int64_t n_dst, int C, int H,
                                            anemoi_stream_t stream);
+
+int anemoi_gt_decoder_fused(const void* x_aug, int64_t ldx, int64_t k_in, const float* x_stats, const void* w_in,
+                            const float* b_in, const float* cs_in, const void* k, const void* v, int64_t ldkv,
+                            const float* edge_attr, int up, const int32_t* col, const int32_t* grp_dst,
+                            const int32_t* grp_perm, int64_t n_src, void* att, int64_t ld_att, float* lse, int64_t n_dst,
+                            int C, int H, anemoi_stream_t stream);
 
 int anemoi_edge_schedule_shape(int dtype, int64_t n_dst, int C, int* slots, int* steps);
 int anemoi_gt_edge_attention_folded_sched(int dtype, const void* q, int64_t ldq, const void* k, const void* v, int64_t ldkv,
@@ -249,6 +255,7 @@
 } anemoi_gt_block_args;
 int anemoi_gt_block_tail(const anemoi_gt_block_args* args, anemoi_stream_t stream);
 int anemoi_gt_processor_block_forward(const anemoi_gt_block_args* args, anemoi_stream_t stream);
+int anemoi_gt_mapper_block_forward(const anemoi_gt_block_args* args, anemoi_stream_t stream);
 
 typedef struct anemoi_tfm_block_args {
   int64_t struct_bytes;
```

After: 19.26 million (median of 6 runs). No clear change (+0.7%).
